# matvogel/P2P-Bridge

Measured on AMD Instinct MI355X. Metric: denoised points/sec (8192-pt patches, T=30), higher is better.
Workload: dtype f32; 1 GPU; PVDS_PUNet xyz-only, 8192-pt patches, T=30 bridge steps, batch 32 per GPU (BASELINE configs[1]); patches_per_gpu=32, points_per_patch=8192, bridge_steps=30, parallelism=patch-shard x1, process_group_world_size=1, hipgraph=True, weights=seeded random init (26.44 M params)

## Files before the change

include/p2pb_hip.h:

```cpp
#ifndef P2PB_HIP_H
#define P2PB_HIP_H

#include <stddef.h>

#ifdef __cplusplus
extern "C" {
#endif

#define P2PB_EINVAL (-22)

#define P2PB_ABI_VERSION 9

int p2pb_version(void);
const char *p2pb_target_arch(void);
int p2pb_set_split_terms(int terms);
int p2pb_set_split_terms_thread(int terms);
int p2pb_get_split_terms(void);
int p2pb_set_deterministic(int on);
int p2pb_get_deterministic(void);
int p2pb_debug_pointwise_form(int cin, int cout, int npos, unsigned long long *launches);

int p2pb_gn_finisher_arm(int groups, double count_per_channel, const float *gamma, const float *beta, const float *style,
                         int style_stride, float eps, float *scale, float *shift, float *chmean);
int p2pb_gn_finisher_armed(void);
void p2pb_gn_finisher_disarm(void);

int p2pb_voxel_coords(int b, int n, int r, int normalize, float eps, const float *coords, float *norm,
                      int *vox, void *stream);

size_t p2pb_avg_voxelize_ws_bytes(int b, int n, int r);
int p2pb_avg_voxelize_forward(int b, int c, int n, int r, const int *coords, const float *feat, int *ind,
                              int *cnt, float *out, void *ws, void *stream);
int p2pb_avg_voxelize_backward(int b, int c, int n, int r3, const int *ind, const int *cnt,
                               const float *grad_y, float *grad_x, void *stream);

int p2pb_trilinear_devoxelize_forward(int b, int c, int n, int r, int is_training, const float *coords,
                                      const float *feat, int *inds, float *wgts, float *outs, void *stream);
int p2pb_trilinear_devoxelize_backward(int b, int c, int n, int r3, const int *inds, const float *wgts,
                                       const float *grad_y, float *grad_x, void *stream);

int p2pb_ball_query(int b, int n, int m, float r2, int u, const float *centers, const float *points, int *idx,
                    void *stream);

int p2pb_grouping_forward(int b, int c, int n, int m, int u, const float *feat, const int *idx, float *out,
                          void *stream);
int p2pb_grouping_backward(int b, int c, int n, int m, int u, const float *grad_y, const int *idx,
                           float *grad_x, void *stream);
int p2pb_grouping_backward_pitched(int b, int c, int n, int m, int u, const float *grad_y, long gy_pitch, const int *idx,
                                   float *grad_x, void *stream);

int p2pb_group_concat(int b, int c, int n, int m, int u, const float *coords, const float *centers,
                      const float *feat, const int *idx, float *out, void *stream);

int p2pb_gather_features_forward(int b, int c, int n, int m, const float *feat, const int *idx, float *out,
                                 void *stream);
int p2pb_gather_features_backward(int b, int c, int n, int m, const float *grad_y, const int *idx,
                                  float *grad_x, void *stream);

int p2pb_furthest_point_sampling(int b, int n, int m, const float *coords, float *dist_ws, int *idx,
                                 void *stream);

size_t p2pb_fps_coop_ws_bytes(int b, int n);
int p2pb_furthest_point_sampling_coop(int b, int n, int m, const float *coords, void *ws, int *idx, void *stream);
size_t p2pb_fps_grid_ws_bytes(int b, int n);
int p2pb_furthest_point_sampling_grid(int b, int n, int m, const float *coords, void *ws, int *idx, void *stream);

int p2pb_point_face_dist(int np, int nt, const float *points, const float *tris, float min_triangle_area, float *dist,
                         int *idx, void *stream);
int p2pb_face_point_dist(int np, int nt, const float *points, const float *tris, float min_triangle_area, float *dist,
                         int *idx, void *stream);

size_t p2pb_knn_points_ws_bytes(int b, int s, int n);
int p2pb_knn_points(int b, int s, int n, int k, const float *query, const float *points, float *dist2, int *idx,
                    float *nn, void *ws, void *stream);

int p2pb_three_nn_interpolate_forward(int b, int c, int m, int n, const float *points, const float *centers,
                                      const float *cfeat, int *idx, float *w, float *out, void *stream);
int p2pb_three_nn(int b, int m, int n, const float *points, const float *centers, int *idx, float *w, void *stream);
int p2pb_three_interpolate(int b, int c, int m, int n, const float *cfeat, const int *idx, const float *w,
                           float *out, void *stream);
size_t p2pb_three_nn_cells_ws_bytes(int b, int m);
int p2pb_three_nn_cells(int b, int m, int n, const float *points, const float *centers, int *idx, float *w, void *ws,
                        void *stream);
int p2pb_three_nn_interpolate_backward(int b, int c, int n, int m, const float *grad_y, const int *idx,
                                       const float *w, float *grad_x, void *stream);
int p2pb_three_nn_interpolate_backward_pitched(int b, int c, int n, int m, const float *grad_y, long gy_pitch, const int *idx,
                                               const float *w, float *grad_x, void *stream);

int p2pb_chamfer_forward(int b, int n, int m, const float *xyz1, const float *xyz2, float *dist1, float *dist2,
                         int *idx1, int *idx2, void *stream);
size_t p2pb_chamfer_ws_bytes(int b, int n, int m);
int p2pb_chamfer_forward_ws(int b, int n, int m, const float *xyz1, const float *xyz2, float *dist1, float *dist2,
                            int *idx1, int *idx2, void *ws, void *stream);
int p2pb_chamfer_backward(int b, int n, int m, const float *xyz1, const float *xyz2, float *gradxyz1,
                          float *gradxyz2, const float *graddist1, const float *graddist2, const int *idx1,
                          const int *idx2, void *stream);

size_t p2pb_approxmatch_temp_floats(int b, int n, int m);
int p2pb_approxmatch_forward(int b, int n, int m, const float *xyz1, const float *xyz2, float *match,
                             float *temp, void *stream);
int p2pb_approxmatch_forward_ws(int b, int n, int m, const float *xyz1, const float *xyz2, float *match, float *temp,
                                size_t temp_floats, void *stream);
int p2pb_matchcost_forward(int b, int n, int m, const float *xyz1, const float *xyz2, const float *match,
                           float *cost, void *stream);
int p2pb_matchcost_backward(int b, int n, int m, const float *grad_cost, const float *xyz1, const float *xyz2,
                            const float *match, float *grad1, float *grad2, void *stream);

int p2pb_auction_forward(int b, int n, int m, const float *xyz1, const float *xyz2, float *dist, int *assignment,
                         float *price, int *assignment_inv, int *bid, float *bid_increments,
                         float *max_increments, int *unass_idx, int *unass_cnt, int *unass_cnt_sum, int *cnt_tmp,
                         int *max_idx, float eps, int iters, void *stream);
int p2pb_auction_backward(int b, int n, const float *xyz1, const float *xyz2, float *gradxyz,
                          const float *graddist, const int *idx, void *stream);


size_t p2pb_conv3d_k3_packed_floats(int cout, int cin);
int p2pb_conv3d_k3_pack_weights(int cout, int cin, const float *w, float *wt_packed, void *stream);
size_t p2pb_conv3d_k3_split_packed_bytes(int cout, int cin);
int p2pb_conv3d_k3_pack_weights_split(int cout, int cin, const float *w, void *wt_split, void *stream);
size_t p2pb_conv3d_k3_stats_floats(int b, int cout, int r);
int p2pb_conv3d_k3_forward(int b, int cin, int cout, int r, const float *in, const float *wt_packed,
                           const float *bias, const float *in_scale, const float *in_shift, int in_swish,
                           float *out, float *stats_part, void *stream);

int p2pb_conv3d_k3_forward_ex(int b, int cin, int cout, int r, const float *in, const void *wt_packed,
                              const float *bias, const float *out_class, const float *in_scale,
                              const float *in_shift, int in_swish, const float *in_sub, int flags, float *out,
                              float *stats_part, void *stream);
int p2pb_conv3d_brick_lists(int b, int r, const int *cnt, unsigned char *flags_ws, int *lists, int *counts,
                            void *stream);
int p2pb_conv3d_k3_forward_sparse(int b, int cin, int cout, int r, const float *in, const void *wt_packed,
                                  const float *bias, const float *out_class, const float *in_scale,
                                  const float *in_shift, int in_swish, const float *in_sub, int flags ,
                                  const int *active_list, const int *active_count, const int *inactive_list,
                                  const int *inactive_count, float *out, float *stats_part, void *stream);
int p2pb_conv3d_active_lists(int b, int r, const int *cnt, unsigned char *lists, int *counts, void *stream);
int p2pb_conv3d_k3_forward_compact(int b, int cin, int cout, int r, const float *in, const void *wt_split,
                                   const float *bias, const float *out_class, const float *in_scale,
                                   const float *in_shift, int in_swish, const float *in_sub,
                                   const unsigned char *alist, const int *acount, float *out, float *stats_part,
                                   int flags , void *stream);
int p2pb_conv3d_presplit(int b, int c, long nvox, const float *y, const float *in_scale, const float *in_shift,
                         int in_swish, const float *in_sub, void *out_split, void *stream);
int p2pb_conv3d_k3_forward_compact_pre(int b, int cin, int cout, int r, const void *in_split, const void *wt_split,
                                       const float *bias, const float *out_class, const unsigned char *alist,
                                       const int *acount, float *out, float *stats_part, int flags ,
                                       void *stream);
int p2pb_conv3d_k3_far_field(int b, int cin, int cout, const float *prev_bias, const float *in_scale,
                             const float *in_shift, int in_swish, const float *wt_packed, const float *bias,
                             float *a, float *k_out, float *tap_ws , void *stream);
int p2pb_conv3d_k3_far_field_gn(int b, int cin, int cout, const float *prev_bias, const float *part, int nslots,
                                double count_per_channel, int groups, const float *gamma, const float *beta,
                                const float *style, int style_stride, float eps, int in_swish, const float *wt_packed,
                                const float *bias, float *scale, float *shift, float *a, float *k_out, float *tap_ws,
                                void *stream);

int p2pb_gn_affine_params(int b, int c, int groups, int nslots, double count_per_channel, const float *part,
                          const float *gamma, const float *beta, const float *style, int style_stride, float eps,
                          float *scale, float *shift, float *chmean, void *stream);
int p2pb_gn_affine_params_ex(int b, int c, int groups, int nslots, double count_per_channel, const float *part,
                             const float *gamma, const float *beta, const float *style, int style_stride, float eps,
                             float *scale, float *shift, float *chmean, float *mean_rstd, void *stream);
int p2pb_norm_act_backward(int b, int c, int groups, int npos, const float *x, const float *gy, const float *scale,
                           const float *shift, const float *mean_rstd, const float *gamma, const float *beta,
                           const float *style, int style_stride, int swish, float *dx, float *dgamma, float *dbeta,
                           float *dstyle, float *ws, void *stream);
int p2pb_norm_act_backward_ex(int b, int c, int groups, int npos, const float *x, const float *gy, const float *scale,
                              const float *shift, const float *mean_rstd, const float *gamma, const float *beta,
                              const float *style, int style_stride, int swish, long gy_pitch, const float *gmean,
                              const float *residual, const float *rgate, float drop_p, const unsigned *seed, unsigned salt, float *dx, float *dgamma,
                              float *dbeta, float *dstyle, float *dres, float *drgate, float *ws, void *stream);
int p2pb_affine_act_train(int b, int c, int npos, const float *x, const float *scale, const float *shift, int swish,
                          const float *residual, const float *rgate, float drop_p, const unsigned *seed, unsigned salt,
                          float *y, void *stream);
int p2pb_se_gate_affine(int b, int c, int hidden, const float *chmean, const float *w1, const float *w2,
                        const float *scale, const float *shift, float *aff_a, float *aff_b, void *stream);
int p2pb_pvconv_tail(int b, int c, int hidden, const float *part2, int nslots2, double count2, int groups2,
                     const float *gamma2, const float *beta2, const float *style2, int style_stride2, float eps2,
                     const float *w1, const float *w2, float *aff_a, float *aff_b, int cp, const float *partp, int nslotsp,
                     double countp, int groupsp, const float *gammap, const float *betap, const float *stylep,
                     int style_stridep, float epsp, float *scale_p, float *shift_p, void *stream);

int p2pb_avg_voxelize_cl_forward(int b, int c, int n, int r, const int *coords, const float *feat, int *ind, int *cnt,
                                 float *out, float *feat_t, void *ws, void *stream);
int p2pb_voxel_sort(int b, int n, int r, const int *coords, int *ind, int *cnt, void *ws, void *stream);
int p2pb_avg_voxelize_cl_gather(int b, int c, int n, int r, const float *feat, const int *cnt, const void *ws,
                                float *out, float *feat_t, void *stream);
int p2pb_avg_voxelize_cl_gather_split(int b, int c, int n, int r, const float *feat, const int *cnt, const void *ws,
                                      void *out_split, float *feat_t, void *stream);
int p2pb_trilinear_devoxelize_cl_affine(int b, int c, int n, int r, const float *coords, const float *grid,
                                        const float *aff_a, const float *aff_b, const float *add ,
                                        const float *add_scale, const float *add_shift, float *outs, void *stream);
int p2pb_trilinear_devoxelize_affine(int b, int c, int n, int r, const float *coords, const float *feat,
                                     const float *aff_a, const float *aff_b, float *outs, void *stream);

int p2pb_three_interpolate_add(int b, int c, int m, int n, const float *cz, const int *idx, const float *w,
                               const float *add, const float *bias, float *out, float *stats_part,
                               float *ws , void *stream);
size_t p2pb_group_sub_stats_floats(int b, int c, int m, int u);
int p2pb_group_sub_stats_slots(int m, int u);
int p2pb_group_sub_stats(int b, int c, int n, int m, int u, const float *zt, const float *cxt, const int *idx,
                         float *stats_part, void *stream);
int p2pb_group_sub(int b, int c, int n, int m, int u, const float *z, const float *cx, const int *idx, float *out,
                   float *stats_part, float *ws , void *stream);

size_t p2pb_pointwise_packed_floats(int cout, int cin);
int p2pb_pointwise_pack_weights(int cout, int cin, const float *w , float *wp, void *stream);
size_t p2pb_pointwise_stats_floats(int b, int cout, int npos);
int p2pb_pointwise_conv_forward(int b, int cin, int cout, int npos, const float *in, const void *wp,
                                const float *bias, const float *bias_b, const float *in_scale,
                                const float *in_shift, int in_swish, int flags, float *out, float *stats_part,
                                void *stream);
size_t p2pb_pointwise_split_packed_bytes(int cout, int cin);
int p2pb_pointwise_pack_weights_split(int cout, int cin, const float *w , void *wp, void *stream);
int p2pb_pointwise_pool_supported(int npos, int pool_u);
size_t p2pb_pointwise_minmax_floats(int b, int cout, int npos, int pool_u, int flags);
int p2pb_pointwise_conv_pool_forward(int b, int cin, int cout, int npos, const float *in, const void *wp,
                                     const float *bias, const float *bias_b, const float *in_scale,
                                     const float *in_shift, int in_swish, int flags, float *out, float *stats_part,
                                     int pool_u, float *minmax, void *stream);
int p2pb_pointwise_conv_pool_gather(int b, int cin, int cout, int n, int m, int u, const float *zt, const float *cxt,
                                    const int *idx, const void *wp_split, const float *bias, const float *in_scale,
                                    const float *in_shift, int in_swish, float *stats_part, float *minmax, void *stream);
int p2pb_linear_rows(int b, int cin, int cout, const float *x, long x_stride, const float *w, long w_stride,
                     const float *bias, float *out, long out_stride, void *stream);
int p2pb_minmax_act(int b, int c, int m, int nslots, const float *minmax, const float *scale, const float *shift,
                    int swish, float *y, void *stream);
int p2pb_minmax_act_pool_gn(int b, int c, int nslots, const float *minmax, const float *part, int nslots_st,
                            double count_per_channel, int groups, const float *gamma, const float *beta, const float *style,
                            int style_stride, float eps, int swish, float *scale, float *shift, float *y, void *stream);
int p2pb_affine_act(int b, int c, int npos, const float *x, const float *scale, const float *shift, int swish,
                    const float *residual, float *y, void *stream);
int p2pb_affine_act_max(int b, int c, int m, int u, const float *x, const float *scale, const float *shift,
                        int swish, float *y, void *stream);

int p2pb_linear_attention_forward(int b, int heads, int dim_head, int n, const float *qkv, float *out, float *ctx,
                                  void *stream);
int p2pb_linear_attention_backward(int b, int heads, int dim_head, int n, const float *qkv, const float *ctx,
                                   const float *grad_out, float *grad_qkv, void *stream);

int p2pb_softmax_attention_forward(int b, int heads, int dim_head, int n, const float *q, const float *kv, float *out,
                                   float *lse, void *stream);
int p2pb_softmax_attention_backward(int b, int heads, int dim_head, int n, const float *q, const float *kv,
                                    const float *out, const float *lse, const float *grad_out, float *grad_q,
                                    float *grad_kv, void *stream);

int p2pb_se_gate_forward(int b, int c, int hidden, const float *mean, const float *w1, const float *w2, float *hid, float *gate,
                         void *stream);
int p2pb_se_gate_backward(int b, int c, int hidden, const float *mean, const float *w1, const float *w2, const float *hid,
                          const float *gate, const float *dgate, float *dmean, float *dw1, float *dw2, float *ws, void *stream);

int p2pb_row_max_forward(long rows, int u, const float *x, float *y, int *idx, void *stream);
int p2pb_row_max_backward(long rows, int u, const float *gy, const int *idx, float *gx, void *stream);

size_t p2pb_conv3d_k3_wgrad_ws_floats(int b, int cin, int cout, int r, int math);
int p2pb_conv3d_k3_wgrad(int b, int cin, int cout, int r, const float *x, const float *dy, float *dw, float *db,
                         float *ws, int math, void *stream);
size_t p2pb_conv3d_k3_wgrad_occ_ws_floats(int b, int cin, int cout, int r, int n);
int p2pb_conv3d_k3_wgrad_occ(int b, int cin, int cout, int r, int n, const float *x, const float *dy, const int *cnt, float *dw,
                             float *db, float *ws, void *stream);
size_t p2pb_pointwise_wgrad_ws_floats(int b, int cin, int cout, int npos, int math);
int p2pb_pointwise_wgrad(int b, int cin, int cout, int npos, const float *x, const float *dy, float *dw, float *db,
                         float *ws, int math, void *stream);

int p2pb_radius_count(int s, int n, const float *centers, const float *points, float radius, int *counts, void *stream);
int p2pb_radius_fill(int s, int n, const float *centers, const float *points, float radius, const long long *offsets,
                     int *out, void *stream);
int p2pb_merge_accumulate(int npatch, int k, const float *pred, const int *idx, const int *cuts, double *sums,
                          int *counts, void *stream);
int p2pb_merge_finish(int n, const double *sums, const int *counts, const float *original, float *out, void *stream);

int p2pb_conv3d_k3_pack_weights_split_adjoint(int cout, int cin, const float *w_forward, void *wt_split, void *stream);
int p2pb_pointwise_pack_weights_adjoint(int cout, int cin, const float *w_forward, float *wp, void *stream);
int p2pb_pointwise_pack_weights_split_adjoint(int cout, int cin, const float *w_forward, void *wp, void *stream);

size_t p2pb_optim_entry_bytes(void);
int p2pb_optim_chunk(void);
int p2pb_optim_clip_adam_step(int nchunks, const void *table, const int *chunks, double *partial, double *ctl, double max_norm,
                              double beta1, double beta2, double eps, double weight_decay, int decoupled, int skip_nonfinite,
                              unsigned *amax, int ntensors, void *stream);
int p2pb_conv3d_k3_pack_weights_split_amax(int cout, int cin, const float *w, void *wt_split, const unsigned *amax_bits,
                                           void *stream);
int p2pb_pointwise_pack_weights_split_amax(int cout, int cin, const float *w, void *wp, const unsigned *amax_bits, void *stream);

size_t p2pb_pairwise_chamfer_ws_bytes(int s, int r);
int p2pb_pairwise_chamfer(int s, int r, int n, int m, const float *A, const float *B, float *out, void *ws, void *stream);
size_t p2pb_pairwise_emd_ws_bytes(int s, int r, int n, int m);
int p2pb_pairwise_emd(int s, int r, int n, int m, const float *A, const float *B, float *out, void *ws, size_t ws_bytes,
                      void *stream);
int p2pb_occupancy_grid_cells(int resolution, int clip_sphere);
size_t p2pb_occupancy_ws_bytes(int resolution);
int p2pb_occupancy_counts(int clouds, int npts, int resolution, int clip_sphere, const float *pts, int *counters,
                          int *bernoulli, void *ws, void *stream);

#ifdef __cplusplus
}
#endif
#endif
```

p2p_bridge_amd/_lib.py:

```python
import ctypes
import os

import torch

_HERE = os.path.dirname(os.path.abspath(__file__))
LIB_PATH = os.environ.get("P2PB_LIB_PATH") or os.path.join(_HERE, "libp2pb_hip.so")

SYMBOLS = [
    "p2pb_version", "p2pb_target_arch", "p2pb_set_split_terms", "p2pb_set_split_terms_thread", "p2pb_get_split_terms", "p2pb_set_deterministic", "p2pb_get_deterministic", "p2pb_voxel_coords", "p2pb_avg_voxelize_ws_bytes",
    "p2pb_avg_voxelize_forward", "p2pb_avg_voxelize_backward", "p2pb_avg_voxelize_cl_gather_split", "p2pb_conv3d_presplit",
    "p2pb_conv3d_k3_forward_compact_pre", "p2pb_trilinear_devoxelize_forward",
    "p2pb_trilinear_devoxelize_backward", "p2pb_ball_query", "p2pb_grouping_forward", "p2pb_grouping_backward", "p2pb_group_concat", "p2pb_group_sub", "p2pb_three_interpolate_add", "p2pb_group_sub_stats_floats", "p2pb_group_sub_stats_slots", "p2pb_group_sub_stats",
    "p2pb_gather_features_forward", "p2pb_gather_features_backward", "p2pb_furthest_point_sampling",
    "p2pb_fps_coop_ws_bytes", "p2pb_furthest_point_sampling_coop", "p2pb_point_face_dist", "p2pb_face_point_dist", "p2pb_knn_points_ws_bytes", "p2pb_knn_points", "p2pb_three_nn_interpolate_forward", "p2pb_three_nn_interpolate_backward", "p2pb_three_nn", "p2pb_three_nn_cells", "p2pb_three_nn_cells_ws_bytes",
    "p2pb_three_interpolate", "p2pb_chamfer_forward",
    "p2pb_chamfer_backward", "p2pb_approxmatch_forward", "p2pb_matchcost_forward", "p2pb_matchcost_backward",
    "p2pb_auction_forward", "p2pb_auction_backward", "p2pb_conv3d_k3_packed_floats", "p2pb_conv3d_k3_pack_weights",
    "p2pb_conv3d_k3_split_packed_bytes", "p2pb_conv3d_k3_pack_weights_split",
    "p2pb_conv3d_k3_stats_floats", "p2pb_conv3d_k3_forward", "p2pb_conv3d_k3_forward_ex",
    "p2pb_conv3d_k3_far_field", "p2pb_conv3d_k3_far_field_gn", "p2pb_pvconv_tail", "p2pb_minmax_act_pool_gn", "p2pb_conv3d_active_lists", "p2pb_conv3d_k3_forward_compact", "p2pb_conv3d_brick_lists", "p2pb_conv3d_k3_forward_sparse", "p2pb_gn_affine_params", "p2pb_se_gate_affine",
    "p2pb_trilinear_devoxelize_affine", "p2pb_avg_voxelize_cl_forward", "p2pb_voxel_sort", "p2pb_avg_voxelize_cl_gather", "p2pb_trilinear_devoxelize_cl_affine", "p2pb_pointwise_packed_floats", "p2pb_pointwise_pack_weights",
    "p2pb_pointwise_stats_floats", "p2pb_pointwise_conv_forward", "p2pb_affine_act", "p2pb_affine_act_max",
    "p2pb_pointwise_split_packed_bytes", "p2pb_pointwise_pack_weights_split", "p2pb_pointwise_pool_supported", "p2pb_pointwise_minmax_floats", "p2pb_pointwise_conv_pool_forward",
    "p2pb_minmax_act", "p2pb_linear_attention_forward", "p2pb_linear_attention_backward", "p2pb_softmax_attention_forward", "p2pb_softmax_attention_backward",
    "p2pb_approxmatch_temp_floats", "p2pb_approxmatch_forward_ws", "p2pb_pointwise_conv_pool_gather", "p2pb_chamfer_ws_bytes", "p2pb_chamfer_forward_ws", "p2pb_radius_count", "p2pb_radius_fill", "p2pb_merge_accumulate", "p2pb_merge_finish", "p2pb_gn_affine_params_ex", "p2pb_norm_act_backward", "p2pb_norm_act_backward_ex", "p2pb_grouping_backward_pitched", "p2pb_three_nn_interpolate_backward_pitched", "p2pb_affine_act_train", "p2pb_conv3d_k3_wgrad_ws_floats", "p2pb_conv3d_k3_wgrad", "p2pb_conv3d_k3_wgrad_occ_ws_floats", "p2pb_conv3d_k3_wgrad_occ", "p2pb_pointwise_wgrad_ws_floats", "p2pb_pointwise_wgrad",
    "p2pb_debug_pointwise_form", "p2pb_linear_rows", "p2pb_gn_finisher_arm", "p2pb_gn_finisher_armed", "p2pb_gn_finisher_disarm", "p2pb_fps_grid_ws_bytes", "p2pb_furthest_point_sampling_grid",
    "p2pb_optim_entry_bytes", "p2pb_optim_chunk", "p2pb_optim_clip_adam_step",
    "p2pb_conv3d_k3_pack_weights_split_adjoint", "p2pb_pointwise_pack_weights_adjoint", "p2pb_pointwise_pack_weights_split_adjoint",
    "p2pb_conv3d_k3_pack_weights_split_amax", "p2pb_pointwise_pack_weights_split_amax",
    "p2pb_se_gate_forward", "p2pb_se_gate_backward", "p2pb_row_max_forward", "p2pb_row_max_backward",
    "p2pb_pairwise_chamfer_ws_bytes", "p2pb_pairwise_chamfer", "p2pb_pairwise_emd_ws_bytes", "p2pb_pairwise_emd",
    "p2pb_occupancy_grid_cells", "p2pb_occupancy_ws_bytes", "p2pb_occupancy_counts",
]

ABI_VERSION = 9

_lib = None


class P2PBError(RuntimeError):
    pass


def lib():
    global _lib
    if _lib is None:
        if not os.path.exists(LIB_PATH):
            raise P2PBError(
                f"{LIB_PATH} not found: build it with `python -m p2p_bridge_amd.build` "
                "(p2p_bridge_amd has no CPU / eager fallback)")
        _lib = ctypes.CDLL(LIB_PATH)
        _lib.p2pb_target_arch.restype = ctypes.c_char_p
        _lib.p2pb_avg_voxelize_ws_bytes.restype = ctypes.c_size_t
        _lib.p2pb_knn_points_ws_bytes.restype = ctypes.c_size_t
        _lib.p2pb_fps_grid_ws_bytes.restype = ctypes.c_size_t
        _lib.p2pb_three_nn_cells_ws_bytes.restype = ctypes.c_size_t
        _lib.p2pb_fps_coop_ws_bytes.restype = ctypes.c_size_t
        _lib.p2pb_conv3d_k3_packed_floats.restype = ctypes.c_size_t
        _lib.p2pb_conv3d_k3_split_packed_bytes.restype = ctypes.c_size_t
        _lib.p2pb_conv3d_k3_stats_floats.restype = ctypes.c_size_t
        _lib.p2pb_pointwise_packed_floats.restype = ctypes.c_size_t
        _lib.p2pb_pointwise_stats_floats.restype = ctypes.c_size_t
        _lib.p2pb_pointwise_minmax_floats.restype = ctypes.c_size_t
        _lib.p2pb_group_sub_stats_floats.restype = ctypes.c_size_t
        _lib.p2pb_pointwise_split_packed_bytes.restype = ctypes.c_size_t
        _lib.p2pb_conv3d_k3_wgrad_ws_floats.restype = ctypes.c_size_t
        _lib.p2pb_conv3d_k3_wgrad_occ_ws_floats.restype = ctypes.c_size_t
        _lib.p2pb_chamfer_ws_bytes.restype = ctypes.c_size_t
        _lib.p2pb_approxmatch_temp_floats.restype = ctypes.c_size_t
        _lib.p2pb_pointwise_wgrad_ws_floats.restype = ctypes.c_size_t
        _lib.p2pb_optim_entry_bytes.restype = ctypes.c_size_t
        _lib.p2pb_pairwise_chamfer_ws_bytes.restype = ctypes.c_size_t
        _lib.p2pb_pairwise_emd_ws_bytes.restype = ctypes.c_size_t
        _lib.p2pb_occupancy_ws_bytes.restype = ctypes.c_size_t
        have = _lib.p2pb_version() if hasattr(_lib, "p2pb_version") else None
        if have != ABI_VERSION:
            bad, _lib = _lib, None
            del bad
            raise P2PBError(f"{LIB_PATH} is ABI version {have}, this package binds version {ABI_VERSION} (include/p2pb_hip.h): "
                            "rebuild it with `python -m p2p_bridge_amd.build`")
        for s in SYMBOLS:
            getattr(_lib, s)
        _lib.p2pb_set_split_terms(6 if os.environ.get("P2PB_CONV_MATH") in ("bf16x6", "fp32") else 16)
    return _lib


def stream_ptr():
    return ctypes.c_void_p(torch.cuda.current_stream().cuda_stream)


def ptr(t):
    return ctypes.c_void_p(t.data_ptr()) if t is not None else ctypes.c_void_p(0)


def check(t, dtype, name):
    if not t.is_cuda:
        raise RuntimeError(f"{name} must be a CUDA tensor")
    if not t.is_contiguous():
        raise RuntimeError(f"{name} must be a contiguous tensor")
    if t.dtype != dtype:
        raise RuntimeError(f"{name} must be a {'float' if dtype == torch.float32 else 'int'} tensor")


def call(fn_name, *args):
    rc = getattr(lib(), fn_name)(*args)
    if rc != 0:
        raise P2PBError(f"{fn_name} failed with code {rc}")
```

p2p_bridge_amd/csrc/abi.hip:

```cpp
#include "common.h"

extern "C" int p2pb_version(void) { return P2PB_ABI_VERSION; }
extern "C" const char *p2pb_target_arch(void) { return "gfx950"; }

#include <atomic>
static std::atomic<int> g_split_terms{SPLIT_F16X3};
static thread_local int tl_split_terms = 0;
int p2pb_split_terms_now() { return tl_split_terms ? tl_split_terms : g_split_terms.load(std::memory_order_relaxed); }
extern "C" int p2pb_set_split_terms(int terms) {
  if (terms != SPLIT_BF16X6 && terms != SPLIT_F16X3) return P2PB_EINVAL;
  g_split_terms.store(terms, std::memory_order_relaxed);
  return 0;
}
extern "C" int p2pb_set_split_terms_thread(int terms) {
  if (terms != 0 && terms != SPLIT_BF16X6 && terms != SPLIT_F16X3 && terms != SPLIT_BF16X3) return P2PB_EINVAL;
  tl_split_terms = terms;
  return 0;
}
extern "C" int p2pb_get_split_terms(void) { return p2pb_split_terms_now(); }

static std::atomic<int> g_deterministic{0};
bool p2pb_deterministic() { return g_deterministic.load(std::memory_order_relaxed) != 0; }
extern "C" int p2pb_set_deterministic(int on) {
  g_deterministic.store(on ? 1 : 0, std::memory_order_relaxed);
  return 0;
}
extern "C" int p2pb_get_deterministic(void) { return p2pb_deterministic() ? 1 : 0; }

#include <mutex>
namespace {
struct FormRow {
  int cin, cout, npos, form;
  unsigned long long n;
};
std::mutex g_form_mu;
FormRow g_forms[128];
int g_nforms = 0;
}
void p2pb_note_pointwise_form(int cin, int cout, int npos, int form) {
  std::lock_guard<std::mutex> lk(g_form_mu);
  for (int i = 0; i < g_nforms; ++i)
    if (g_forms[i].cin == cin && g_forms[i].cout == cout && g_forms[i].npos == npos) {
      g_forms[i].form = form;
      ++g_forms[i].n;
      return;
    }
  if (g_nforms < 128) g_forms[g_nforms++] = {cin, cout, npos, form, 1ull};
}
extern "C" int p2pb_debug_pointwise_form(int cin, int cout, int npos, unsigned long long *launches) {
  std::lock_guard<std::mutex> lk(g_form_mu);
  if (launches) *launches = 0;
  if (cin < 0) {
    g_nforms = 0;
    return -1;
  }
  for (int i = 0; i < g_nforms; ++i)
    if (g_forms[i].cin == cin && g_forms[i].cout == cout && g_forms[i].npos == npos) {
      if (launches) *launches = g_forms[i].n;
      return g_forms[i].form;
    }
  return -1;
}

#include <cstdlib>
#include <cstring>
#include <cctype>
long p2pb_experiment_long(const char *key, long dflt) {
  const char *e = getenv("P2PB_EXPERIMENT");
  const size_t kl = strlen(key);
  while (e && *e) {
    while (*e == ';' || isspace((unsigned char)*e)) ++e;
    size_t i = 0;
    while (i < kl && e[i] && tolower((unsigned char)e[i]) == tolower((unsigned char)key[i])) ++i;
    if (i == kl) {
      const char *q = e + kl;
      while (*q == ' ' || *q == '\t') ++q;
      if (*q == '=') return atol(q + 1);
    }
    e = strchr(e, ';');
  }
  return dflt;
}

__global__ __launch_bounds__(256) void zero_words_kernel(unsigned *__restrict__ p, size_t nwords) {
  const size_t stride = (size_t)gridDim.x * 256;
  for (size_t i = (size_t)blockIdx.x * 256 + threadIdx.x; i < nwords; i += stride) p[i] = 0u;
}

__global__ __launch_bounds__(256) void zero_quads_kernel(uint4 *__restrict__ p, size_t nquads) {
  const size_t stride = (size_t)gridDim.x * 256;
  const uint4 z = make_uint4(0u, 0u, 0u, 0u);
  for (size_t i = (size_t)blockIdx.x * 256 + threadIdx.x; i < nquads; i += stride) p[i] = z;
}

int p2pb_zero_async(void *p, size_t nbytes, hipStream_t s) {
  if (nbytes == 0) return 0;
  if ((((size_t)p) & 15) == 0 && (nbytes & 15) == 0) {
    const size_t nq = nbytes / 16;
    const unsigned grid = (unsigned)((nq + 255) / 256 > 4096 ? 4096 : (nq + 255) / 256);
    hipLaunchKernelGGL(zero_quads_kernel, dim3(grid), dim3(256), 0, s, (uint4 *)p, nq);
    return (int)hipGetLastError();
  }
  const size_t nwords = (nbytes + 3) / 4;
  const unsigned grid = (unsigned)((nwords + 255) / 256 > 2048 ? 2048 : (nwords + 255) / 256);
  hipLaunchKernelGGL(zero_words_kernel, dim3(grid), dim3(256), 0, s, (unsigned *)p, nwords);
  return (int)hipGetLastError();
}

namespace {
thread_local bool tl_fin_armed = false;
thread_local GnFinish tl_fin;
}
extern "C" int p2pb_gn_finisher_arm(int groups, double count_per_channel, const float *gamma, const float *beta, const float *style,
                                    int style_stride, float eps, float *scale, float *shift, float *chmean) {
  if (groups <= 0 || !scale || !shift || !(count_per_channel > 0.0) || tl_fin_armed) return P2PB_EINVAL;
  tl_fin.gamma = gamma, tl_fin.beta = beta, tl_fin.style = style, tl_fin.scale = scale, tl_fin.shift = shift, tl_fin.chmean = chmean;
  tl_fin.count_per_channel = count_per_channel, tl_fin.style_stride = style_stride;
  tl_fin.groups = groups, tl_fin.eps = eps;
  tl_fin_armed = true;
  return 0;
}
extern "C" int p2pb_gn_finisher_armed(void) { return tl_fin_armed ? 1 : 0; }
extern "C" void p2pb_gn_finisher_disarm(void) { tl_fin_armed = false; }
bool p2pb_gn_finisher_take(GnFinish *out) {
  if (!tl_fin_armed) return false;
  *out = tl_fin;
  tl_fin_armed = false;
  return true;
}
```

p2p_bridge_amd/csrc/common.h:

```cpp
#pragma once
#include <hip/hip_runtime.h>
#include <stdint.h>

#include "../../include/p2pb_hip.h"

#define P2PB_WAVE 64

static inline int p2pb_launch_status() { return (int)hipGetLastError(); }
int p2pb_split_terms_now();
#define p2pb_g_split_terms (p2pb_split_terms_now())

static inline unsigned cdiv(long a, long b) { return (unsigned)((a + b - 1) / b); }

__device__ __forceinline__ float sqdist3(float dx, float dy, float dz) {
  return __fmaf_rn(dz, dz, __fmaf_rn(dy, dy, dx * dx));
}

__device__ __forceinline__ int lane_id() { return (int)(threadIdx.x & 63); }

__device__ __forceinline__ int mbcnt(unsigned long long mask) {
  return (int)__builtin_amdgcn_mbcnt_hi((unsigned)(mask >> 32), __builtin_amdgcn_mbcnt_lo((unsigned)mask, 0u));
}

template <int CTRL, int ROW_MASK>
__device__ __forceinline__ float dpp_add_step(float v) {
  const int o = __builtin_amdgcn_update_dpp(0, __builtin_bit_cast(int, v), CTRL, ROW_MASK, 0xf, false);
  return v + __builtin_bit_cast(float, o);
}
__device__ __forceinline__ float halfwave_sum_to_last(float v) {
  v = dpp_add_step<0x111, 0xf>(v);
  v = dpp_add_step<0x112, 0xf>(v);
  v = dpp_add_step<0x114, 0xf>(v);
  v = dpp_add_step<0x118, 0xf>(v);
  v = dpp_add_step<0x142, 0xa>(v);
  return v;
}

typedef __bf16 bf16x8 __attribute__((ext_vector_type(8)));
typedef __bf16 bf16x2 __attribute__((ext_vector_type(2)));
typedef float f32x2 __attribute__((ext_vector_type(2)));
typedef unsigned u32x4 __attribute__((ext_vector_type(4)));
typedef float f32x16 __attribute__((ext_vector_type(16)));

__device__ __forceinline__ void split3(float a, float b, unsigned &p0, unsigned &p1, unsigned &p2) {
  f32x2 v = {a, b};
  const bf16x2 q0 = __builtin_convertvector(v, bf16x2);
  v = v - __builtin_convertvector(q0, f32x2);
  const bf16x2 q1 = __builtin_convertvector(v, bf16x2);
  v = v - __builtin_convertvector(q1, f32x2);
  const bf16x2 q2 = __builtin_convertvector(v, bf16x2);
  p0 = __builtin_bit_cast(unsigned, q0);
  p1 = __builtin_bit_cast(unsigned, q1);
  p2 = __builtin_bit_cast(unsigned, q2);
}

#define SPLIT_BF16X6 6
#define SPLIT_BF16X3 3
#define SPLIT_F16X3 16
#define SPLIT_F16_SX 4.0f
typedef _Float16 f16x8 __attribute__((ext_vector_type(8)));
typedef _Float16 f16x2 __attribute__((ext_vector_type(2)));
__device__ __forceinline__ void split2h(float a, float b, unsigned &p0, unsigned &p1) {
  f32x2 v = {a, b};
  const f16x2 q0 = __builtin_convertvector(v, f16x2);
  v = v - __builtin_convertvector(q0, f32x2);
  const f16x2 q1 = __builtin_convertvector(v, f16x2);
  p0 = __builtin_bit_cast(unsigned, q0);
  p1 = __builtin_bit_cast(unsigned, q1);
}
template <int MODE>
__device__ __forceinline__ void split_pair(float a, float b, unsigned &p0, unsigned &p1, unsigned &p2) {
  if constexpr (MODE == SPLIT_F16X3) {
    split2h(a * SPLIT_F16_SX, b * SPLIT_F16_SX, p0, p1);
    p2 = 0u;
  } else {
    split3(a, b, p0, p1, p2);
  }
}
#define SPLIT_X2W_FLAG 0x100
#ifdef P2PB_X2W_TIMING
#define X2W_KEEP_LOW_WEIGHT_PRODUCT 0
#else
#define X2W_KEEP_LOW_WEIGHT_PRODUCT 1
#endif
constexpr __host__ __device__ int split_planes(int mode) { return mode == SPLIT_BF16X6 ? 3 : 2; }
template <int MODE>
__device__ __forceinline__ f32x16 split_mfma(const u32x4 &a, const u32x4 &b, const f32x16 &c) {
  if constexpr (MODE == SPLIT_F16X3)
    return __builtin_amdgcn_mfma_f32_32x32x16_f16(__builtin_bit_cast(f16x8, a), __builtin_bit_cast(f16x8, b), c, 0, 0, 0);
  else
    return __builtin_amdgcn_mfma_f32_32x32x16_bf16(__builtin_bit_cast(bf16x8, a), __builtin_bit_cast(bf16x8, b), c, 0, 0, 0);
}
__device__ __forceinline__ float f16_weight_scale(float wmax) {
  if (!(wmax > 0.0f) || wmax > 3.0e38f) return 1.0f;
  int e;
  (void)frexpf(wmax, &e);
  return ldexpf(1.0f, 14 - e);
}
struct GnFinish {
  const float *gamma, *beta, *style;
  float *scale, *shift, *chmean;
  double count_per_channel;
  int style_stride, groups;
  float eps;
};
static inline bool gn_shape_ok(int c, int groups, const float *style, int style_stride) {
  return groups > 0 && c % groups == 0 && c / groups <= 256 && !(style && style_stride < 2 * c);
}
typedef float gnf_f32x2 __attribute__((ext_vector_type(2)));
__device__ __forceinline__ void gn_finish_group_v(int c, int nslots, const float *__restrict__ part, const GnFinish &f, int b, int g,
                                                  double *lds, int vt, bool live, float *mean_rstd = nullptr,
                                                  float *tab_scale = nullptr, float *tab_shift = nullptr, float *tab_mean = nullptr) {
  double *rs = lds, *rq = lds + 256, *chs = lds + 512, *chq = lds + 768;
  const int t = vt;
  const int cg = c / f.groups, g0 = g * cg;
  const int nt = 256 / cg;
  const int k = t % cg, j = t / cg;
  float p_ga = 1.0f, p_be = 0.0f, p_fa = 1.0f, p_bi = 0.0f;
  if (live && t < cg) {
    const int ch = g0 + t;
    if (f.gamma) p_ga = f.gamma[ch];
    if (f.beta) p_be = f.beta[ch];
    if (f.style) {
      p_fa = f.style[(size_t)b * f.style_stride + ch];
      p_bi = f.style[(size_t)b * f.style_stride + c + ch];
    }
  }
  double s = 0.0, q = 0.0;
  if (live && j < nt) {
    const float *p0 = part + ((size_t)b * nslots * c + g0 + k) * 2;
    const size_t pitch = (size_t)c * 2;
    int sl = j;
    for (; sl + 7 * nt < nslots; sl += 8 * nt) {
      gnf_f32x2 v[8];
#pragma unroll
      for (int u = 0; u < 8; ++u) {
        const float *pp = p0 + (size_t)(sl + u * nt) * pitch;
        v[u] = *(const gnf_f32x2 *)pp;
      }
#pragma unroll
      for (int u = 0; u < 8; ++u) {
        s += (double)v[u][0];
        q += (double)v[u][1];
      }
    }
    for (; sl + 3 * nt < nslots; sl += 4 * nt) {
      gnf_f32x2 v[4];
#pragma unroll
      for (int u = 0; u < 4; ++u) {
        const float *pp = p0 + (size_t)(sl + u * nt) * pitch;
        v[u] = *(const gnf_f32x2 *)pp;
      }
#pragma unroll
      for (int u = 0; u < 4; ++u) {
        s += (double)v[u][0];
        q += (double)v[u][1];
      }
    }
    for (; sl < nslots; sl += nt) {
      const float *p = p0 + (size_t)sl * pitch;
      s += (double)p[0];
      q += (double)p[1];
    }
  }
  if (live) {
    rs[t] = s;
    rq[t] = q;
  }
  __syncthreads();
  if (live && t < cg) {
    double ts = 0.0, tq = 0.0;
    for (int jj = 0; jj < nt; ++jj) {
      ts += rs[jj * cg + t];
      tq += rq[jj * cg + t];
    }
    chs[t] = ts;
    chq[t] = tq;
  }
  __syncthreads();
  if (live && t < cg) {
    double gs = 0.0, gq = 0.0;
    for (int kk = 0; kk < cg; ++kk) {
      gs += chs[kk];
      gq += chq[kk];
    }
    const int ch = g0 + t;
    const double n = f.count_per_channel * cg;
    const double mean = gs / n;
    double var = gq / n - mean * mean;
    if (var < 0.0) var = 0.0;
    const double rstd = 1.0 / sqrt(var + (double)f.eps);
    const double ga = (double)p_ga, be = (double)p_be, fa = (double)p_fa, bi = (double)p_bi;
    const double sc = rstd * ga * fa;
    const double sh = (be - mean * rstd * ga) * fa + bi;
    const float cm = (float)(sc * (chs[t] / f.count_per_channel) + sh);
    if (f.scale) f.scale[(size_t)b * c + ch] = (float)sc;
    if (f.shift) f.shift[(size_t)b * c + ch] = (float)sh;
    if (f.chmean) f.chmean[(size_t)b * c + ch] = cm;
    if (tab_scale) tab_scale[ch] = (float)sc;
    if (tab_shift) tab_shift[ch] = (float)sh;
    if (tab_mean) tab_mean[ch] = cm;
    if (mean_rstd && t == 0) {
      mean_rstd[((size_t)b * f.groups + g) * 2] = (float)mean;
      mean_rstd[((size_t)b * f.groups + g) * 2 + 1] = (float)rstd;
    }
  }
  __syncthreads();
}
__device__ __forceinline__ void gn_finish_group(int c, int nslots, const float *__restrict__ part, const GnFinish &f, int b, int g,
                                                double *lds, float *mean_rstd = nullptr) {
  gn_finish_group_v(c, nslots, part, f, b, g, lds, (int)threadIdx.x, threadIdx.x < 256, mean_rstd);
}
template <int NS>
__device__ __forceinline__ void gn_finish_sample(int c, int nslots, const float *__restrict__ part, const GnFinish &f, int b, double *lds,
                                                 float *tab_scale = nullptr, float *tab_shift = nullptr, float *tab_mean = nullptr) {
  const int slice = (int)threadIdx.x >> 8, vt = (int)threadIdx.x & 255;
  for (int g0 = 0; g0 < f.groups; g0 += NS) {
    const int g = g0 + slice;
    gn_finish_group_v(c, nslots, part, f, b, g < f.groups ? g : 0, lds + slice * 1024, vt, slice < NS && g < f.groups, nullptr,
                      tab_scale, tab_shift, tab_mean);
  }
}
template <int CTRL>
__device__ __forceinline__ float dpp_full(float v) {
  const int i = __builtin_bit_cast(int, v);
  return __builtin_bit_cast(float, __builtin_amdgcn_update_dpp(i, i, CTRL, 0xf, 0xf, false));
}
__device__ __forceinline__ void permlane16_swap(float &a, float &b) {
  asm volatile("s_nop 1\n\tv_permlane16_swap_b32 %0, %1\n\ts_nop 1" : "+v"(a), "+v"(b));
}
struct RowAdd {
  __device__ static float f(float a, float b) { return a + b; }
};
__device__ __forceinline__ float vmin_raw(float a, float b) {
  float r;
  asm("v_min_f32 %0, %1, %2" : "=v"(r) : "v"(a), "v"(b));
  return r;
}
__device__ __forceinline__ float vmax_raw(float a, float b) {
  float r;
  asm("v_max_f32 %0, %1, %2" : "=v"(r) : "v"(a), "v"(b));
  return r;
}
struct RowMin {
  __device__ static float f(float a, float b) {
    float r;
    asm("v_min_f32 %0, %1, %2" : "=v"(r) : "v"(a), "v"(b));
    return r;
  }
};
struct RowMax {
  __device__ static float f(float a, float b) {
    float r;
    asm("v_max_f32 %0, %1, %2" : "=v"(r) : "v"(a), "v"(b));
    return r;
  }
};
template <class Op>
__device__ __forceinline__ float rowreduce32(float (&v)[32]) {
  const int lane = (int)(threadIdx.x & 63);
#pragma unroll
  for (int i = 0; i < 16; ++i) {
    float a = v[i], b = v[i + 16];
    permlane16_swap(a, b);
    v[i] = Op::f(a, b);
  }
#pragma unroll
  for (int i = 0; i < 8; ++i) {
    const float x = Op::f(v[i], dpp_full<0x128>(v[i])), y = Op::f(v[i + 8], dpp_full<0x128>(v[i + 8]));
    v[i] = (lane & 8) ? y : x;
  }
#pragma unroll
  for (int i = 0; i < 4; ++i) {
    const float x = Op::f(v[i], dpp_full<0x141>(v[i])), y = Op::f(v[i + 4], dpp_full<0x141>(v[i + 4]));
    v[i] = (lane & 4) ? y : x;
  }
#pragma unroll
  for (int i = 0; i < 2; ++i) {
    const float x = Op::f(v[i], dpp_full<0x4E>(v[i])), y = Op::f(v[i + 2], dpp_full<0x4E>(v[i + 2]));
    v[i] = (lane & 2) ? y : x;
  }
  const float x = Op::f(v[0], dpp_full<0xB1>(v[0])), y = Op::f(v[1], dpp_full<0xB1>(v[1]));
  return (lane & 1) ? y : x;
}

template <class Op>
__device__ __forceinline__ void groupreduce8(float (&v)[32]) {
  const int lane = (int)(threadIdx.x & 63);
#pragma unroll
  for (int i = 0; i < 16; ++i) {
    const float x = Op::f(v[i], dpp_full<0x141>(v[i])), y = Op::f(v[i + 16], dpp_full<0x141>(v[i + 16]));
    v[i] = (lane & 4) ? y : x;
  }
#pragma unroll
  for (int i = 0; i < 8; ++i) {
    const float x = Op::f(v[i], dpp_full<0x4E>(v[i])), y = Op::f(v[i + 8], dpp_full<0x4E>(v[i + 8]));
    v[i] = (lane & 2) ? y : x;
  }
#pragma unroll
  for (int i = 0; i < 4; ++i) {
    const float x = Op::f(v[i], dpp_full<0xB1>(v[i])), y = Op::f(v[i + 4], dpp_full<0xB1>(v[i + 4]));
    v[i] = (lane & 1) ? y : x;
  }
}

template <class Op>
__device__ __forceinline__ void groupreduce16(float (&v)[32]) {
  const int lane = (int)(threadIdx.x & 63);
#pragma unroll
  for (int i = 0; i < 16; ++i) {
    const float x = Op::f(v[i], dpp_full<0x140>(v[i])), y = Op::f(v[i + 16], dpp_full<0x140>(v[i + 16]));
    v[i] = (lane & 8) ? y : x;
  }
#pragma unroll
  for (int i = 0; i < 8; ++i) {
    const float x = Op::f(v[i], dpp_full<0x141>(v[i])), y = Op::f(v[i + 8], dpp_full<0x141>(v[i + 8]));
    v[i] = (lane & 4) ? y : x;
  }
#pragma unroll
  for (int i = 0; i < 4; ++i) {
    const float x = Op::f(v[i], dpp_full<0x4E>(v[i])), y = Op::f(v[i + 4], dpp_full<0x4E>(v[i + 4]));
    v[i] = (lane & 2) ? y : x;
  }
#pragma unroll
  for (int i = 0; i < 2; ++i) {
    const float x = Op::f(v[i], dpp_full<0xB1>(v[i])), y = Op::f(v[i + 2], dpp_full<0xB1>(v[i + 2]));
    v[i] = (lane & 1) ? y : x;
  }
}

enum {
  P2PB_FORM_PW_FP32 = 0,
  P2PB_FORM_PW_WIDE_FP32 = 1,
  P2PB_FORM_PW_WIDE_F16 = 2,
  P2PB_FORM_PW_SPLIT128 = 3,
  P2PB_FORM_PW_SPLIT256 = 4,
  P2PB_FORM_PW_PINGPONG = 5,
  P2PB_FORM_PW_GATHER = 6,
};
void p2pb_note_pointwise_form(int cin, int cout, int npos, int form);
bool p2pb_gn_finisher_take(GnFinish *out);
int p2pb_gn_affine_launch(int b, int c, int nslots, const float *part, const GnFinish &f, hipStream_t s);

long p2pb_experiment_long(const char *key, long dflt);

int p2pb_zero_async(void *p, size_t nbytes, hipStream_t s);

#define SCAT_THREADS 512
#define SCAT_LDS_MAX (128 * 1024)
bool p2pb_deterministic();
static inline int scat_threads() { return p2pb_deterministic() ? 64 : SCAT_THREADS; }
static inline int scat_rows(long L, int c, int cap) {
  if (L * 4 > SCAT_LDS_MAX) return 0;
  int ch = (int)((64 * 1024) / (L * 4));
  if (ch < 1) ch = 1;
  if (ch > cap) ch = cap;
  if (ch > c) ch = c;
  return ch;
}
__device__ __forceinline__ void scat_zero(float *rows, int count) {
  for (int i = threadIdx.x * 4; i < count; i += blockDim.x * 4) *(float4 *)(rows + i) = make_float4(0.f, 0.f, 0.f, 0.f);
  __syncthreads();
}
__device__ __forceinline__ void scat_store(const float *rows, int L, int Lp, int nch, float *gx_rows) {
  __syncthreads();
  for (int j = 0; j < nch; ++j)
    for (int i = threadIdx.x; i < L; i += blockDim.x) gx_rows[(size_t)j * L + i] = rows[j * Lp + i];
}
```

p2p_bridge_amd/csrc/pointwise.hip:

```cpp
#include "common.h"
#include "absmax.h"
#include <atomic>
#include <stdint.h>
#include <stdlib.h>

typedef float f32x4 __attribute__((ext_vector_type(4)));

#define PW_CK 16

__device__ __forceinline__ float swishf(float v) {
  return v * __builtin_amdgcn_rcpf(1.0f + __builtin_amdgcn_exp2f(v * -1.44269504088896340736f));
}

template <int MT, bool XF, bool STATS>
__global__ __launch_bounds__(256, 3) void pw_conv_kernel(int cin, int cout, int cout_pad, int P,
                                                      const float *__restrict__ in, const float *__restrict__ wp,
                                                      const float *__restrict__ bias,
                                                      const float *__restrict__ bias_b,
                                                      const float *__restrict__ in_scale,
                                                      const float *__restrict__ in_shift, int in_swish,
                                                      float *__restrict__ out, float *__restrict__ stats_part) {
  const int tid = threadIdx.x, lane = tid & 63, wave = tid >> 6;
  const int l31 = lane & 31, khalf = lane >> 5;
  const int p0 = blockIdx.x * 256, co0 = blockIdx.y * (32 * MT), b = blockIdx.z;
// ... 389 lines not shown
#pragma unroll
      for (int t = 0; t < 4; ++t) acc[m][t][r] += bv;
      if (co < cout && pok && outb)
        *(f32x4 *)(outb + (size_t)co * P + p) = f32x4{acc[m][0][r], acc[m][1][r], acc[m][2][r], acc[m][3][r]};
    }
  const int rrow = MT == 2 ? l31 : (l31 & 15);
  const int rco = co0 + (rrow >> 4) * 32 + (rrow & 3) + 8 * ((rrow & 15) >> 2) + 4 * khalf;
  auto rowval = [&](int kind, int m, int r) -> float {
    const int co = co0 + m * 32 + (r & 3) + 8 * (r >> 2) + 4 * khalf;
    const float v0 = acc[m][0][r], v1 = acc[m][1][r], v2 = acc[m][2][r], v3 = acc[m][3][r];
    const bool ok = co < cout && pok;
    if (kind == 0) return ok ? (v0 + v1) + (v2 + v3) : 0.0f;
    if (kind == 1) return ok ? (v0 * v0 + v1 * v1) + (v2 * v2 + v3 * v3) : 0.0f;
    if (kind == 2) return pok ? vmin_raw(vmin_raw(v0, v1), vmin_raw(v2, v3)) : INFINITY;
    return pok ? -vmax_raw(vmax_raw(v0, v1), vmax_raw(v2, v3)) : INFINITY;
  };
  if (STATS) {
    float s1, s2;
    float tv[32];
    if constexpr (MT == 2) {
#pragma unroll
      for (int i = 0; i < 32; ++i) tv[i] = rowval(0, i >> 4, i & 15);
      s1 = rowreduce32<RowAdd>(tv);
#pragma unroll
      for (int i = 0; i < 32; ++i) tv[i] = rowval(1, i >> 4, i & 15);
      s2 = rowreduce32<RowAdd>(tv);
    } else {
#pragma unroll
      for (int i = 0; i < 32; ++i) tv[i] = rowval(i >> 4, 0, i & 15);
      s1 = s2 = rowreduce32<RowAdd>(tv);
    }
    if (rco < cout) {
      if (slot < nslots) {
        float *q = stats_part + (((size_t)b * nslots + slot) * cout + rco) * 2;
        if constexpr (MT == 2) *(f32x2 *)q = f32x2{s1, s2};
        else q[l31 >> 4] = s1;
      }
      if (slot + 1 < nslots) {
        float *q = stats_part + (((size_t)b * nslots + slot + 1) * cout + rco) * 2;
        if constexpr (MT == 2) *(f32x2 *)q = f32x2{0.0f, 0.0f};
        else q[l31 >> 4] = 0.0f;
      }
    }
  }
  if constexpr (PG != 0) {
    float tv[32];
    if constexpr (PG == 32) {
      float mn, mx;
      if constexpr (MT == 2) {
#pragma unroll
        for (int i = 0; i < 32; ++i) tv[i] = rowval(2, i >> 4, i & 15);
        mn = rowreduce32<RowMin>(tv);
#pragma unroll
        for (int i = 0; i < 32; ++i) tv[i] = rowval(3, i >> 4, i & 15);
        mx = -rowreduce32<RowMin>(tv);
      } else {
#pragma unroll
        for (int i = 0; i < 32; ++i) tv[i] = rowval(2 + (i >> 4), 0, i & 15);
        mn = rowreduce32<RowMin>(tv);
        mx = -mn;
      }
      if (rco < cout) {
        float *q = mm_out + ((((size_t)b * gridDim.x + blockIdx.x) * 4 + wave) * cout + rco) * 2;
        if constexpr (MT == 2) *(f32x2 *)q = f32x2{mn, mx};
        else q[l31 >> 4] = (l31 >> 4) ? mx : mn;
      }
    } else if constexpr (PG == 8) {
      const int j = l31 & 7;
      const size_t ngrp = (size_t)(P / 32);
      if constexpr (MT == 2) {
        float tx[32];
#pragma unroll
        for (int i = 0; i < 32; ++i) {
          tv[i] = rowval(2, i >> 4, i & 15);
          tx[i] = rowval(3, i >> 4, i & 15);
        }
        groupreduce8<RowMin>(tv);
        groupreduce8<RowMin>(tx);
        const int cb = co0 + 32 * (j >> 2) + 8 * (j & 3) + 4 * khalf;
        if (pok) {
          float *q = mm_out + (((size_t)b * cout + cb) * ngrp + p / 32) * 2;
#pragma unroll
          for (int i = 0; i < 4; ++i)
            if (cb + i < cout) *(f32x2 *)(q + (size_t)i * ngrp * 2) = f32x2{tv[i], -tx[i]};
        }
      } else {
#pragma unroll
        for (int i = 0; i < 32; ++i) tv[i] = rowval(2 + (i >> 4), 0, i & 15);
        groupreduce8<RowMin>(tv);
        const int cb = co0 + 8 * (j & 3) + 4 * khalf;
        if (pok) {
          float *q = mm_out + (((size_t)b * cout + cb) * ngrp + p / 32) * 2 + (j >> 2);
#pragma unroll
          for (int i = 0; i < 4; ++i)
            if (cb + i < cout) q[(size_t)i * ngrp * 2] = (j >> 2) ? -tv[i] : tv[i];
        }
      }
    } else {
#pragma unroll
      for (int m = 0; m < MT; ++m)
#pragma unroll
        for (int r = 0; r < 16; ++r) {
          const int co = co0 + m * 32 + (r & 3) + 8 * (r >> 2) + 4 * khalf;
          float mn = rowval(2, m, r), mx = -rowval(3, m, r);
          group_minmax(mn, mx, pool_g);
          if (co < cout && (l31 & (pool_g - 1)) == 0 && pok) {
            const int u = 4 * pool_g;
            float *q = mm_out + (((size_t)b * cout + co) * (P / u) + p / u) * 2;
            q[0] = mn;
            q[1] = mx;
          }
        }
    }
  }
}

__global__ void pw_pack_kernel(int cout, int cin, int cin_pad, int cout_pad, const float *__restrict__ w,
                               float *__restrict__ wp, long s_co, long s_ci) {
  const size_t total = (size_t)cin_pad * cout_pad;
  for (size_t e = (size_t)blockIdx.x * 256 + threadIdx.x; e < total; e += (size_t)gridDim.x * 256) {
    const int kk = (int)(e & 3);
    const int co = (int)((e >> 2) % cout_pad);
    const int kh = (int)((e / ((size_t)4 * cout_pad)) & 1);
    const int chunk = (int)(e / ((size_t)8 * cout_pad));
    const int ci = chunk * 8 + 2 * kk + kh;
    wp[e] = (co < cout && ci < cin) ? w[(size_t)co * s_co + (size_t)ci * s_ci] : 0.0f;
  }
}

static inline int pw_cin_pad(int cin) { return (cin + 7) / 8 * 8; }
static inline int pw_cout_pad(int cout) { return (cout + 127) / 128 * 128; }

extern "C" size_t p2pb_pointwise_packed_floats(int cout, int cin) {
  return (size_t)pw_cin_pad(cin) * pw_cout_pad(cout);
}

static int pw_pack(int cout, int cin, const float *w, float *wp, bool adjoint, void *stream) {
  if (cout <= 0 || cin <= 0) return P2PB_EINVAL;
  const size_t total = p2pb_pointwise_packed_floats(cout, cin);
  hipLaunchKernelGGL(pw_pack_kernel, dim3((unsigned)((total + 255) / 256 > 2048 ? 2048 : (total + 255) / 256)), dim3(256),
                     0, (hipStream_t)stream, cout, cin, pw_cin_pad(cin), pw_cout_pad(cout), w, wp, adjoint ? 1L : (long)cin,
                     adjoint ? (long)cout : 1L);
  return p2pb_launch_status();
}
extern "C" int p2pb_pointwise_pack_weights(int cout, int cin, const float *w, float *wp, void *stream) {
  return pw_pack(cout, cin, w, wp, false, stream);
}
extern "C" int p2pb_pointwise_pack_weights_adjoint(int cout, int cin, const float *w_forward, float *wp, void *stream) {
  return pw_pack(cout, cin, w_forward, wp, true, stream);
}

extern "C" size_t p2pb_pointwise_stats_floats(int b, int cout, int npos) {
  return (size_t)b * ((npos + 255) / 256) * 4 * cout * 2;
}

#define PWS_CK 32

#define PWS_TILE (2 * 3 * 2 * 128)
#define PWS_LDS_BYTES (2 * PWS_TILE * 16)
#include "pw_pp512.h"

template <int PL, int WM, int NB>
__device__ __forceinline__ void pws_epilogue(f32x16 (&acc)[2][2 * NB], int b, int bx, int gx, int pblk, int co0,
                                             int wm, int wn, int l31, int khalf, int cout, int P, int nslots,
                                             const float *__restrict__ bias, const float *__restrict__ bias_b,
                                             float *__restrict__ out, float *__restrict__ stats_part,
                                             float *__restrict__ mm_out, int pool_u, int out_pm, const float *sb) {
#pragma unroll
  for (int pb = 0; pb < NB; ++pb) {
  const int p = pblk + 128 * pb + 2 * (wn * 32 + l31);
  const bool pok = p < P;
  if (WM == 2 && out_pm) {
    float *ob = out + (size_t)b * P * cout;
#pragma unroll
    for (int m = 0; m < 2; ++m)
#pragma unroll
      for (int g = 0; g < 4; ++g) {
        const int cq = co0 + wm * 64 + m * 32 + 8 * g + 4 * khalf;
        float bv[4];
#pragma unroll
        for (int i = 0; i < 4; ++i) bv[i] = sb[cq + i - co0];
        if (pok && cq < cout) {
#pragma unroll
          for (int n = 0; n < 2; ++n) {
            float *q = ob + (size_t)(p + n) * cout + cq;
            const f32x4 v = {acc[m][2 * pb + n][4 * g] + bv[0], acc[m][2 * pb + n][4 * g + 1] + bv[1],
                             acc[m][2 * pb + n][4 * g + 2] + bv[2], acc[m][2 * pb + n][4 * g + 3] + bv[3]};
            if (cq + 3 < cout && (cout & 3) == 0) *(f32x4 *)q = v;
            else
              for (int i = 0; i < 4; ++i)
                if (cq + i < cout) q[i] = v[i];
          }
        }
      }
    continue;
  }
  float *outb = out ? out + (size_t)b * cout * P : nullptr;
  const int slot = (bx * NB + pb) * 2 + wn;
  const int pool_g = pool_u ? pool_u / 2 : 32;
#pragma unroll
  for (int m = 0; m < 2; ++m) {
#pragma unroll
    for (int r = 0; r < 16; ++r) {
      const int co = co0 + wm * 64 + m * 32 + (r & 3) + 8 * (r >> 2) + 4 * khalf;
      const bool cok = co < cout;
      const float bv = sb[co - co0];
      acc[m][2 * pb][r] += bv;
      acc[m][2 * pb + 1][r] += bv;
      const f32x2 v = {acc[m][2 * pb][r], acc[m][2 * pb + 1][r]};
      if (cok && pok && outb) *(f32x2 *)(outb + (size_t)co * P + p) = v;
      if constexpr (PL == 2) {
        float mn = pok ? fminf(v[0], v[1]) : INFINITY, mx = pok ? fmaxf(v[0], v[1]) : -INFINITY;
        group_minmax(mn, mx, pool_g);
        if (cok && pok && (pool_g == 32 ? l31 == 31 : (l31 & (pool_g - 1)) == 0)) {
          float *q = mm_out + (((size_t)b * cout + co) * (P / pool_u) + p / pool_u) * 2;
          q[0] = mn;
          q[1] = mx;
        }
      }
    }
  }
  if constexpr (PL == 32) {
    float tn[32], tx[32];
#pragma unroll
    for (int m = 0; m < 2; ++m)
#pragma unroll
      for (int r = 0; r < 16; ++r) {
        const float v0 = acc[m][2 * pb][r], v1 = acc[m][2 * pb + 1][r];
        tn[m * 16 + r] = pok ? vmin_raw(v0, v1) : INFINITY;
        tx[m * 16 + r] = pok ? -vmax_raw(v0, v1) : INFINITY;
      }
    groupreduce16<RowMin>(tn);
    groupreduce16<RowMin>(tx);
    const int j = l31 & 15;
    const int cb = co0 + wm * 64 + 32 * (j >> 3) + 2 * (j & 1) + 8 * ((j & 7) >> 1) + 4 * khalf;
    if (pok) {
      const size_t ngrp = (size_t)(P / 32);
      float *q = mm_out + (((size_t)b * cout + cb) * ngrp + p / 32) * 2;
#pragma unroll
      for (int i = 0; i < 2; ++i)
        if (cb + i < cout) *(f32x2 *)(q + (size_t)i * ngrp * 2) = f32x2{tn[i], -tx[i]};
    }
  }
  const int rm = l31 >> 4, rr = l31 & 15;
  const int rco = co0 + wm * 64 + rm * 32 + (rr & 3) + 8 * (rr >> 2) + 4 * khalf;
  auto rowvals = [&](int kind, float (&v)[32]) {
#pragma unroll
    for (int m = 0; m < 2; ++m)
#pragma unroll
      for (int r = 0; r < 16; ++r) {
        const int co = co0 + wm * 64 + m * 32 + (r & 3) + 8 * (r >> 2) + 4 * khalf;
        const float v0 = acc[m][2 * pb][r], v1 = acc[m][2 * pb + 1][r];
        const bool ok = co < cout && pok;
        v[m * 16 + r] = kind == 0 ? (ok ? v0 + v1 : 0.0f)
                        : kind == 1 ? (ok ? v0 * v0 + v1 * v1 : 0.0f)
                        : kind == 2 ? (pok ? fminf(v0, v1) : INFINITY)
                                    : (pok ? fmaxf(v0, v1) : -INFINITY);
      }
  };
  if (stats_part) {
    float tv[32];
    rowvals(0, tv);
    const float s1 = rowreduce32<RowAdd>(tv);
    rowvals(1, tv);
    const float s2 = rowreduce32<RowAdd>(tv);
    if (rco < cout) {
      float *q = stats_part + (((size_t)b * nslots + slot) * cout + rco) * 2;
      q[0] = s1;
      q[1] = s2;
      if (bx == gx - 1 && pb == NB - 1 && wn == 1)
        for (int sl = slot + 1; sl < nslots; ++sl) {
          float *z = stats_part + (((size_t)b * nslots + sl) * cout + rco) * 2;
          z[0] = 0.0f;
          z[1] = 0.0f;
        }
    }
  }
  if constexpr (PL == 1) {
    float tv[32];
    rowvals(2, tv);
    const float mn = rowreduce32<RowMin>(tv);
    rowvals(3, tv);
    const float mx = rowreduce32<RowMax>(tv);
    if (rco < cout) {
      float *q = mm_out + ((((size_t)b * gx * NB + bx * NB + pb) * 2 + wn) * cout + rco) * 2;
      q[0] = mn;
      q[1] = mx;
    }
  }
  }
}

template <bool XF, int PL, int WM, int NB, int TERMS>
#ifndef PWS_WM4_WAVES
#define PWS_WM4_WAVES 4
#endif
__global__ __launch_bounds__(128 * WM, NB == 2 ? 2 : (WM == 2 ? 3 : PWS_WM4_WAVES)) void pw_split_kernel(int cin, int cout, int P, int nslots,
                                                       const float *__restrict__ in, const u32x4 *__restrict__ wp,
                                                       const float *__restrict__ bias,
                                                       const float *__restrict__ bias_b,
                                                       const float *__restrict__ in_scale,
                                                       const float *__restrict__ in_shift, int in_swish,
                                                       float *__restrict__ out, float *__restrict__ stats_part,
                                                       float *__restrict__ mm_out, int pool_u, int out_pm) {
  extern __shared__ u32x4 pws_lds[];
  constexpr int NT = 128 * WM;
  constexpr int BS = 128 * NB;
  u32x4 *lds_b = pws_lds + (WM / 2) * PWS_TILE;
  const u32x4 *lds_a = pws_lds;
  const int tid = threadIdx.x, lane = tid & 63;
  const int wave = __builtin_amdgcn_readfirstlane(tid >> 6);
  const int l31 = lane & 31, khalf = lane >> 5;
  const int wm = wave >> 1, wn = wave & 1;
  const int ncoblk = gridDim.y;
  const unsigned lin = blockIdx.x + gridDim.x * (blockIdx.y + gridDim.y * blockIdx.z);
  const unsigned nblk = gridDim.x * gridDim.y * gridDim.z;
  const unsigned vid = nblk % 8 == 0 ? (lin % 8) * (nblk / 8) + lin / 8 : lin;
  const int bx = (vid / ncoblk) % gridDim.x, by = vid % ncoblk;
  const int b = vid / (ncoblk * gridDim.x);
  const int pblk = bx * (128 * NB), co0 = by * (64 * WM);
  const float *inb = in + (size_t)b * cin * P;
  const bool mact = co0 + wm * 64 < cout;
  __shared__ float pws_bias[64 * WM];
  if (tid < 64 * WM) {
    const int co = co0 + tid;
    float v = 0.0f;
    if (co < cout) {
      v = bias ? bias[co] : 0.0f;
      if (bias_b) v += bias_b[(size_t)b * cout + co];
    }
    pws_bias[tid] = v;
  }

  f32x16 acc[2][2 * NB];
#pragma unroll
  for (int m = 0; m < 2; ++m)
#pragma unroll
    for (int n = 0; n < 2 * NB; ++n)
#pragma unroll
      for (int r = 0; r < 16; ++r) acc[m][n][r] = 0.0f;

  constexpr bool ONE = WM == 4 && NB == 1;
  constexpr int NBW = WM == 2 ? NB : 1;
  const int bgrp = WM == 2 ? wave : wave >> 1, bsel = WM == 2 ? 0 : (wave & 1);
  unsigned voff[NBW];
#pragma unroll
  for (int q = 0; q < NBW; ++q) {
    const int pl = ONE ? pblk + 64 * bsel + lane : pblk + 128 * (WM == 2 ? q : bsel) + 2 * lane;
    voff[q] = (unsigned)(pl < P ? pl : P - (ONE ? 1 : 2)) * 4u;
  }
  float braw[NBW][8][ONE ? 1 : 2];
  auto load_b = [&](int ci0) {
#pragma unroll
    for (int i = 0; i < 8; ++i) {
      const int row = min(ci0 + 8 * bgrp + i, cin - 1);
      auto rs = __builtin_amdgcn_make_buffer_rsrc((void *)(inb + (size_t)row * P), 0, P * 4, 0x00020000);
#pragma unroll
      for (int q = 0; q < NBW; ++q) {
        if constexpr (!ONE) {
          const f32x2 v = __builtin_bit_cast(f32x2, __builtin_amdgcn_raw_buffer_load_b64(rs, voff[q], 0, 0));
          braw[q][i][0] = v[0];
          braw[q][i][1] = v[1];
        } else {
          braw[q][i][0] = __builtin_bit_cast(float, __builtin_amdgcn_raw_buffer_load_b32(rs, voff[q], 0, 0));
        }
      }
    }
  };
  auto dma_a = [&](int chunk) {
    const int nblk128 = WM == 2 ? ncoblk : (cout + 127) / 128;
    const u32x4 *src = wp + ((size_t)chunk * nblk128 + by * (WM / 2)) * PWS_TILE;
    u32x4 *dst = pws_lds;
    const bool second_ok = WM == 2 || by * 2 + 1 < nblk128;
#pragma unroll
    for (int i = 0; i < 6; ++i)
      if ((second_ok || i * NT + tid < PWS_TILE) && (TERMS == 6 || (((i * NT + wave * 64) % PWS_TILE) / 256) % 3 != 2))
        __builtin_amdgcn_global_load_lds((const __attribute__((address_space(1))) void *)(src + i * NT + tid),
                                         (__attribute__((address_space(3))) void *)(dst + i * NT + wave * 64), 16, 0, 0);
  };
  load_b(0);

  for (int ci0 = 0; ci0 < cin; ci0 += PWS_CK) {
    __syncthreads();
    dma_a(ci0 / PWS_CK);
    {
      constexpr int NE = ONE ? 1 : 2;
      if (XF) {
#pragma unroll
        for (int i = 0; i < 8; ++i) {
          const int c = min(ci0 + 8 * bgrp + i, cin - 1);
          const float sc = in_scale[b * cin + c], sh = in_shift[b * cin + c];
#pragma unroll
          for (int q = 0; q < NBW; ++q)
#pragma unroll
            for (int e = 0; e < NE; ++e) {
              float v = braw[q][i][e] * sc + sh;
              if (in_swish) v = swishf(v);
              braw[q][i][e] = v;
            }
        }
      }
      const int kstep = bgrp >> 1, kh = bgrp & 1;
#pragma unroll
      for (int q = 0; q < NBW; ++q)
#pragma unroll
        for (int e = 0; e < NE; ++e) {
          u32x4 qq[3];
#pragma unroll
          for (int i = 0; i < 4; ++i) {
            unsigned p0, p1, p2;
            split_pair<TERMS>(braw[q][2 * i][e], braw[q][2 * i + 1][e], p0, p1, p2);
            qq[0][i] = p0;
            qq[1][i] = p1;
            qq[2][i] = p2;
          }
          const int blk = WM == 2 ? q : (NB == 2 ? bsel : 0);
          const int slot = blk * 128 + (ONE ? (lane & 1) * 64 + 32 * bsel + (lane >> 1) : e * 64 + lane);
#pragma unroll
          for (int s = 0; s < split_planes(TERMS); ++s) lds_b[((kstep * 3 + s) * 2 + kh) * BS + slot] = qq[s];
        }
    }
    __builtin_amdgcn_s_waitcnt(0x0F70);
    __syncthreads();
    if (ci0 + PWS_CK < cin) load_b(ci0 + PWS_CK);
    if (!mact) continue;
#pragma unroll
    for (int kstep = 0; kstep < 2; ++kstep) {
      u32x4 af[3][2];
#pragma unroll
      for (int s = 0; s < split_planes(TERMS); ++s)
#pragma unroll
        for (int m = 0; m < 2; ++m)
          af[s][m] = lds_a[(wm >> 1) * PWS_TILE + ((kstep * 3 + s) * 2 + khalf) * 128 + (wm & 1) * 64 + m * 32 + l31];
      constexpr int PA[6] = {2, 1, 0, 1, 0, 0}, PB[6] = {0, 1, 2, 0, 1, 0};
#pragma unroll
      for (int nb = 0; nb < NB; ++nb) {
        u32x4 bf[3][2];
#pragma unroll
        for (int s = 0; s < split_planes(TERMS); ++s)
#pragma unroll
          for (int n = 0; n < 2; ++n)
            bf[s][n] = lds_b[((kstep * 3 + s) * 2 + khalf) * BS + nb * 128 + n * 64 + wn * 32 + l31];
#pragma unroll
        for (int t = (TERMS == 6 ? 0 : 3); t < 6; ++t)
#pragma unroll
          for (int m = 0; m < 2; ++m)
#pragma unroll
            for (int n = 0; n < 2; ++n)
              if (X2W_KEEP_LOW_WEIGHT_PRODUCT || TERMS != SPLIT_F16X3 || PA[t] != 1)
                acc[m][2 * nb + n] = split_mfma<TERMS>(af[PA[t]][m], bf[PB[t]][n], acc[m][2 * nb + n]);
      }
    }
  }
  if (!mact) return;
  {
    if constexpr (TERMS == SPLIT_F16X3) {
      const int nblk128 = WM == 2 ? ncoblk : (cout + 127) / 128;
      const float oscale = ((const float *)(wp + (size_t)((cin + PWS_CK - 1) / PWS_CK) * nblk128 * PWS_TILE))[1];
  #pragma unroll
      for (int m = 0; m < 2; ++m)
  #pragma unroll
        for (int n = 0; n < 2 * NB; ++n)
  #pragma unroll
          for (int r = 0; r < 16; ++r) acc[m][n][r] *= oscale;
    }
  pws_epilogue<PL, WM, NB>(acc, b, bx, (int)gridDim.x, pblk, co0, wm, wn, l31, khalf, cout, P, nslots, bias, bias_b, out,
                             stats_part, mm_out, pool_u, out_pm, pws_bias);
  }
}

__global__ void pw_pack_split_kernel(int cout, int cin, int nchunk, int ncoblk, const float *__restrict__ w,
                                     unsigned short *__restrict__ wp, int mode, float *__restrict__ trailer, long s_co, long s_ci,
                                     const unsigned *__restrict__ amax) {
  const size_t total = (size_t)nchunk * ncoblk * 2 * 2 * 128 * 8;
  const bool x2w = (mode & SPLIT_X2W_FLAG) != 0;
  mode &= 0xff;
  const float wmax = amax ? __builtin_bit_cast(float, *amax) : trailer[0];
  const float sw = mode == SPLIT_F16X3 ? f16_weight_scale(wmax) : 1.0f;
  if (blockIdx.x == 0 && threadIdx.x == 0) {
    trailer[1] = mode == SPLIT_F16X3 ? 1.0f / (SPLIT_F16_SX * sw) : 1.0f;
    if (amax) trailer[0] = wmax, trailer[2] = trailer[3] = 0.0f;
  }
  for (size_t e = (size_t)blockIdx.x * 256 + threadIdx.x; e < total; e += (size_t)gridDim.x * 256) {
    const int idx = (int)(e & 7);
    size_t q = e >> 3;
    const int col = (int)(q & 127);
    q >>= 7;
    const int kh = (int)(q & 1);
    q >>= 1;
    const int ks = (int)(q & 1);
    q >>= 1;
    const int cb = (int)(q % ncoblk), chunk = (int)(q / ncoblk);
    const int co = cb * 128 + col, ci = chunk * PWS_CK + ks * 16 + kh * 8 + idx;
    const float x = (co < cout && ci < cin) ? w[(size_t)co * s_co + (size_t)ci * s_ci] : 0.0f;
    unsigned p0, p1, p2;
    if (mode == SPLIT_F16X3) {
      split2h(x * sw, 0.0f, p0, p1);
      if (x2w) p1 = 0u;
      p2 = 0u;
    } else {
      split3(x, 0.0f, p0, p1, p2);
    }
    const unsigned pp[3] = {p0, p1, p2};
    for (int s = 0; s < 3; ++s)
      wp[((((((size_t)chunk * ncoblk + cb) * 2 + ks) * 3 + s) * 2 + kh) * 128 + col) * 8 + idx] = (unsigned short)(pp[s] & 0xffff);
  }
}

extern "C" size_t p2pb_pointwise_split_packed_bytes(int cout, int cin) {
  const size_t nchunk = (cin + PWS_CK - 1) / PWS_CK, ncoblk = (cout + 127) / 128;
  return nchunk * ncoblk * (2 * 3 * 2 * 128) * 16 + 16;
}

static int pw_pack_split(int cout, int cin, const float *w, void *wp, bool adjoint, void *stream, const unsigned *amax = nullptr) {
  if (cout <= 0 || cin <= 0) return P2PB_EINVAL;
  const int nchunk = (cin + PWS_CK - 1) / PWS_CK, ncoblk = (cout + 127) / 128;
  const size_t total = (size_t)nchunk * ncoblk * 2 * 2 * 128 * 8;
  float *trailer = (float *)((char *)wp + (size_t)nchunk * ncoblk * PWS_TILE * 16);
  static const long x2w = p2pb_experiment_long("x2w", 0);
  const int mode = p2pb_g_split_terms;
  if (mode == SPLIT_F16X3 && !amax) {
    const int rc = p2pb_zero_async(trailer, 16, (hipStream_t)stream);
    if (rc) return rc;
    hipLaunchKernelGGL(absmax_bits_kernel, dim3(absmax_blocks((size_t)cout * cin)), dim3(256), 0, (hipStream_t)stream, w, (size_t)cout * cin,
                       (unsigned *)trailer);
  }
  hipLaunchKernelGGL(pw_pack_split_kernel, dim3((unsigned)((total + 255) / 256 > 2048 ? 2048 : (total + 255) / 256)),
                     dim3(256), 0, (hipStream_t)stream, cout, cin, nchunk, ncoblk, w, (unsigned short *)wp,
                     mode | ((x2w && mode == SPLIT_F16X3 && !adjoint) ? SPLIT_X2W_FLAG : 0), trailer,
                     adjoint ? 1L : (long)cin, adjoint ? (long)cout : 1L, mode == SPLIT_F16X3 ? amax : nullptr);
  return p2pb_launch_status();
}
extern "C" int p2pb_pointwise_pack_weights_split(int cout, int cin, const float *w, void *wp, void *stream) {
  return pw_pack_split(cout, cin, w, wp, false, stream);
}
extern "C" int p2pb_pointwise_pack_weights_split_adjoint(int cout, int cin, const float *w_forward, void *wp, void *stream) {
  return pw_pack_split(cout, cin, w_forward, wp, true, stream);
}
extern "C" int p2pb_pointwise_pack_weights_split_amax(int cout, int cin, const float *w, void *wp, const unsigned *amax_bits,
                                                      void *stream) {
  return amax_bits ? pw_pack_split(cout, cin, w, wp, false, stream, amax_bits) : P2PB_EINVAL;
}

static thread_local GnFinish tl_pw_fin;
static thread_local bool tl_pw_fin_pending = false;
static int pw_finish_behind(int rc, int b, int cout, int P, const float *stats_part, hipStream_t s) {
  if (!tl_pw_fin_pending) return rc;
  tl_pw_fin_pending = false;
  if (rc != 0) return rc;
  if (!stats_part) return P2PB_EINVAL;
  const GnFinish &f = tl_pw_fin;
  if (f.groups <= 0 || cout % f.groups != 0 || cout / f.groups > 256 || (f.style && f.style_stride < 2 * cout)) return P2PB_EINVAL;
  return p2pb_gn_affine_launch(b, cout, (P + 255) / 256 * 4, stats_part, tl_pw_fin, s);
}

static int pw_launch_split(int b, int cin, int cout, int P, const float *in, const void *wp, const float *bias,
                           const float *bias_b, const float *in_scale, const float *in_shift, int in_swish,
                           float *out, float *stats_part, float *minmax, int pool_u, int out_pm, hipStream_t s) {
  const bool xf = in_scale != nullptr;
  const int mode = p2pb_g_split_terms;
  static const int wm_env = (int)p2pb_experiment_long("pw_wm", 0);
  const bool wm4 = !out_pm && (wm_env ? wm_env == 4
                                       : (cout >= 512 && (long)((P + 127) / 128) * ((cout + 255) / 256) * b >= 1024));
  dim3 grid((P + 127) / 128, wm4 ? (cout + 255) / 256 : (cout + 127) / 128, b);
  const int nslots = (P + 255) / 256 * 4;
  const u32x4 *w = (const u32x4 *)wp;
#define LAUNCHW(XF, PL, WM, NB, TM)                                                                                  \
  do {                                                                                                               \
    static bool once = false;                                                                                        \
    const int lds = (WM / 2 + NB) * PWS_TILE * 16;                                                                   \
    if (!once) {                                                                                                     \
      (void)hipFuncSetAttribute((const void *)pw_split_kernel<XF, PL, WM, NB, TM>,                                   \
                                hipFuncAttributeMaxDynamicSharedMemorySize, lds);                                    \
      once = true;                                                                                                   \
    }                                                                                                                \
    hipLaunchKernelGGL((pw_split_kernel<XF, PL, WM, NB, TM>), grid, dim3(128 * WM), lds, s, cin, cout, P, nslots, in, \
                       w, bias, bias_b, in_scale, in_shift, in_swish, out, stats_part, minmax, pool_u, out_pm);       \
  } while (0)
#define LAUNCHF(XF, PL, WM, NB)                                       \
  do {                                                                \
    if (mode == SPLIT_F16X3) LAUNCHW(XF, PL, WM, NB, SPLIT_F16X3);     \
    else LAUNCHW(XF, PL, WM, NB, 6);                                   \
  } while (0)
  if (mode == SPLIT_BF16X3) {
    if (xf || minmax || out_pm) return P2PB_EINVAL;
    p2pb_note_pointwise_form(cin, cout, P, wm4 ? P2PB_FORM_PW_SPLIT256 : P2PB_FORM_PW_SPLIT128);
    if (wm4) LAUNCHW(false, 0, 4, 1, SPLIT_BF16X3);
    else LAUNCHW(false, 0, 2, 1, SPLIT_BF16X3);
    return p2pb_launch_status();
  }
#define LAUNCH(XF, PL)                    \
  do {                                    \
    if (wm4) LAUNCHF(XF, PL, 4, 1);        \
    else LAUNCHF(XF, PL, 2, 1);            \
  } while (0)
  static const int pp_env = (int)p2pb_experiment_long("pw_pp", 1);
  if (pp_env && wm4 && mode == SPLIT_F16X3 && cin % 64 == 0 && cout % 512 == 0 && (!minmax || pool_u == 0) &&
      (size_t)cin * P * 4 < (1ull << 31)) {
    dim3 pgrid((P + 127) / 128, cout / 512, b);
#define LAUNCHP5(XF, PL)                                                                                              \
  do {                                                                                                                \
    static bool once = false;                                                                                         \
    if (!once) {                                                                                                      \
      (void)hipFuncSetAttribute((const void *)pw_pp512_kernel<XF, PL>, hipFuncAttributeMaxDynamicSharedMemorySize,    \
                                P5_LDS_BYTES);                                                                        \
      once = true;                                                                                                    \
    }                                                                                                                 \
    hipLaunchKernelGGL((pw_pp512_kernel<XF, PL>), pgrid, dim3(512), P5_LDS_BYTES, s, cin, cout, P, nslots, in, w, bias, \
                       bias_b, in_scale, in_shift, in_swish, out, stats_part, minmax, pool_u);                        \
  } while (0)
    if (xf && minmax) LAUNCHP5(true, true);
    else if (xf) LAUNCHP5(true, false);
    else if (minmax) LAUNCHP5(false, true);
    else LAUNCHP5(false, false);
#undef LAUNCHP5
    p2pb_note_pointwise_form(cin, cout, P, P2PB_FORM_PW_PINGPONG);
    return p2pb_launch_status();
  }
  p2pb_note_pointwise_form(cin, cout, P, wm4 ? P2PB_FORM_PW_SPLIT256 : P2PB_FORM_PW_SPLIT128);
  const int pl = !minmax ? 0 : pool_u == 0 ? 1 : pool_u == 32 ? 32 : 2;
  if (xf) {
    if (pl == 0) LAUNCH(true, 0);
    else if (pl == 1) LAUNCH(true, 1);
    else if (pl == 32) LAUNCH(true, 32);
    else LAUNCH(true, 2);
  } else {
    if (pl == 0) LAUNCH(false, 0);
    else if (pl == 1) LAUNCH(false, 1);
    else if (pl == 32) LAUNCH(false, 32);
    else LAUNCH(false, 2);
  }
#undef LAUNCH
#undef LAUNCHF
#undef LAUNCHW
  return p2pb_launch_status();
}

static bool pw_wide_ok(int P, const float *in, const float *out) {
  return P % 4 == 0 && (((uintptr_t)in | (uintptr_t)out) & 15) == 0;
}

template <int MT>
static int pw_launch(int b, int cin, int cout, int P, const float *in, const float *wp, const float *bias,
                     const float *bias_b, const float *in_scale, const float *in_shift, int in_swish, float *out,
                     float *stats_part, float *minmax, int pool_g, int out_pm, hipStream_t s, bool split_pack = false) {
  const bool xf = in_scale != nullptr, st = stats_part != nullptr;
  if (split_pack && (!pw_wide_ok(P, in, out) || p2pb_g_split_terms != SPLIT_F16X3)) return P2PB_EINVAL;
  if (pw_wide_ok(P, in, out)) {
    dim3 grid((P + 511) / 512, (cout + 32 * MT - 1) / (32 * MT), b);
    const int nslots = (P + 255) / 256 * 4;
#define LAUNCHX(XF, ST, PL, TM)                                                                                       \
  hipLaunchKernelGGL((pw_wide_kernel<MT, XF, ST, PL, TM>), grid, dim3(256), 0, s, cin, cout, pw_cout_pad(cout), P,       \
                     nslots, in, wp, bias, bias_b, in_scale, in_shift, in_swish, out, stats_part, minmax, pool_g, out_pm,  \
                     PwGather())
#define LAUNCH(XF, ST, PL)                                 \
  do {                                                     \
    if (split_pack) LAUNCHX(XF, ST, PL, SPLIT_F16X3);       \
    else LAUNCHX(XF, ST, PL, 0);                            \
  } while (0)
    p2pb_note_pointwise_form(cin, cout, P, split_pack ? P2PB_FORM_PW_WIDE_F16 : P2PB_FORM_PW_WIDE_FP32);
    if (minmax) {
      const int pg = pool_g == 8 || pool_g == 32 ? pool_g : 1;
      if (xf) {
        if (pg == 8) LAUNCH(true, true, 8);
        else if (pg == 32) LAUNCH(true, true, 32);
        else LAUNCH(true, true, 1);
      } else {
        if (pg == 8) LAUNCH(false, true, 8);
        else if (pg == 32) LAUNCH(false, true, 32);
        else LAUNCH(false, true, 1);
      }
    } else if (xf && st) LAUNCH(true, true, 0);
    else if (xf) LAUNCH(true, false, 0);
    else if (st) LAUNCH(false, true, 0);
    else LAUNCH(false, false, 0);
#undef LAUNCH
#undef LAUNCHX
    return p2pb_launch_status();
  }
  if (minmax || out_pm) return P2PB_EINVAL;
  p2pb_note_pointwise_form(cin, cout, P, P2PB_FORM_PW_FP32);
  dim3 grid((P + 255) / 256, (cout + 32 * MT - 1) / (32 * MT), b);
#define LAUNCH(XF, ST)                                                                                            \
  hipLaunchKernelGGL((pw_conv_kernel<MT, XF, ST>), grid, dim3(256), 0, s, cin, cout, pw_cout_pad(cout), P, in, wp, bias, \
                     bias_b, in_scale, in_shift, in_swish, out, stats_part)
  if (xf && st) LAUNCH(true, true);
  else if (xf) LAUNCH(true, false);
  else if (st) LAUNCH(false, true);
  else LAUNCH(false, false);
#undef LAUNCH
  return p2pb_launch_status();
}

static int pw_conv_forward_impl(int b, int cin, int cout, int npos, const float *in, const void *wp_any,
                                           const float *bias, const float *bias_b, const float *in_scale,
                                           const float *in_shift, int in_swish, int flags, float *out,
                                           float *stats_part, void *stream) {
  if (b <= 0 || cin <= 0 || cout <= 0 || npos <= 0 || !out) return P2PB_EINVAL;
  hipStream_t s = (hipStream_t)stream;
  const int out_pm = (flags & 32) != 0;
  if (out_pm && stats_part) return P2PB_EINVAL;
  if ((flags & 4) && (flags & 128)) {
    const float *wsp = (const float *)wp_any;
    return cout > 32 ? pw_launch<2>(b, cin, cout, npos, in, wsp, bias, bias_b, in_scale, in_shift, in_swish, out,
                                    stats_part, nullptr, 0, out_pm, s, true)
                     : pw_launch<1>(b, cin, cout, npos, in, wsp, bias, bias_b, in_scale, in_shift, in_swish, out,
                                    stats_part, nullptr, 0, out_pm, s, true);
  }
  if (flags & 4) {
    if (!pw_wide_ok(npos, in, out)) return P2PB_EINVAL;
    return pw_launch_split(b, cin, cout, npos, in, wp_any, bias, bias_b, in_scale, in_shift, in_swish, out, stats_part,
                           nullptr, 0, out_pm, s);
  }
  const float *wp = (const float *)wp_any;
  return cout > 32 ? pw_launch<2>(b, cin, cout, npos, in, wp, bias, bias_b, in_scale, in_shift, in_swish, out,
                                  stats_part, nullptr, 0, out_pm, s)
                   : pw_launch<1>(b, cin, cout, npos, in, wp, bias, bias_b, in_scale, in_shift, in_swish, out,
                                  stats_part, nullptr, 0, out_pm, s);
}

extern "C" int p2pb_pointwise_conv_forward(int b, int cin, int cout, int npos, const float *in, const void *wp_any,
                                           const float *bias, const float *bias_b, const float *in_scale,
                                           const float *in_shift, int in_swish, int flags, float *out,
                                           float *stats_part, void *stream) {
  tl_pw_fin_pending = p2pb_gn_finisher_take(&tl_pw_fin);
  const int rc = pw_conv_forward_impl(b, cin, cout, npos, in, wp_any, bias, bias_b, in_scale, in_shift, in_swish, flags, out,
                                      stats_part, stream);
  return pw_finish_behind(rc, b, cout, npos, stats_part, (hipStream_t)stream);
}

static int pool_lanes(int pool_u) { return pool_u == 0 ? 32 : pool_u / 4; }

extern "C" int p2pb_pointwise_pool_supported(int npos, int pool_u) {
  const bool uok = pool_u == 0 || pool_u == 4 || pool_u == 8 || pool_u == 16 || pool_u == 32 || pool_u == 64;
  return npos > 0 && npos % 4 == 0 && uok && (pool_u == 0 || npos % pool_u == 0);
}

extern "C" size_t p2pb_pointwise_minmax_floats(int b, int cout, int npos, int pool_u, int flags) {
  const bool split_tiling = (flags & 4) && !(flags & 128);
  if (pool_u == 0) return (size_t)b * (split_tiling ? (npos + 127) / 128 * 2 : (npos + 511) / 512 * 4) * cout * 2;
  return (size_t)b * cout * (npos / pool_u) * 2;
}

static int pw_conv_pool_forward_impl(int b, int cin, int cout, int npos, const float *in,
                                                const void *wp_any, const float *bias, const float *bias_b,
                                                const float *in_scale, const float *in_shift, int in_swish, int flags,
                                                float *out, float *stats_part, int pool_u, float *minmax,
                                                void *stream) {
  if (b <= 0 || cin <= 0 || cout <= 0 || npos <= 0 || !minmax || !stats_part) return P2PB_EINVAL;
  if (!p2pb_pointwise_pool_supported(npos, pool_u) || !pw_wide_ok(npos, in, out)) return P2PB_EINVAL;
  hipStream_t s = (hipStream_t)stream;
  if ((flags & 4) && (flags & 128)) {
    const float *wsp = (const float *)wp_any;
    const int gl = pool_lanes(pool_u);
    return cout > 32 ? pw_launch<2>(b, cin, cout, npos, in, wsp, bias, bias_b, in_scale, in_shift, in_swish, out,
                                    stats_part, minmax, gl, 0, s, true)
                     : pw_launch<1>(b, cin, cout, npos, in, wsp, bias, bias_b, in_scale, in_shift, in_swish, out,
                                    stats_part, minmax, gl, 0, s, true);
  }
  if (flags & 4)
    return pw_launch_split(b, cin, cout, npos, in, wp_any, bias, bias_b, in_scale, in_shift, in_swish, out, stats_part,
                           minmax, pool_u, 0, s);
  const float *wp = (const float *)wp_any;
  const int g = pool_lanes(pool_u);
  return cout > 32 ? pw_launch<2>(b, cin, cout, npos, in, wp, bias, bias_b, in_scale, in_shift, in_swish, out,
                                  stats_part, minmax, g, 0, s)
                   : pw_launch<1>(b, cin, cout, npos, in, wp, bias, bias_b, in_scale, in_shift, in_swish, out,
                                  stats_part, minmax, g, 0, s);
}

extern "C" int p2pb_pointwise_conv_pool_forward(int b, int cin, int cout, int npos, const float *in,
                                                const void *wp_any, const float *bias, const float *bias_b,
                                                const float *in_scale, const float *in_shift, int in_swish, int flags,
                                                float *out, float *stats_part, int pool_u, float *minmax,
                                                void *stream) {
  tl_pw_fin_pending = p2pb_gn_finisher_take(&tl_pw_fin);
  const int rc = pw_conv_pool_forward_impl(b, cin, cout, npos, in, wp_any, bias, bias_b, in_scale, in_shift, in_swish, flags, out,
                                           stats_part, pool_u, minmax, stream);
  return pw_finish_behind(rc, b, cout, npos, stats_part, (hipStream_t)stream);
}

static int pw_conv_pool_gather_impl(int b, int cin, int cout, int n, int m, int u, const float *zt,
                                               const float *cxt, const int *idx, const void *wp_split, const float *bias,
                                               const float *in_scale, const float *in_shift, int in_swish,
                                               float *stats_part, float *minmax, void *stream) {
  const long npos = (long)m * u;
  if (b <= 0 || cin <= 0 || cout <= 0 || n <= 0 || m <= 0 || !zt || !idx || !wp_split || !in_scale || !in_shift ||
      !stats_part || !minmax || (cin & 7) || npos > 0x7fffffffL || !p2pb_pointwise_pool_supported((int)npos, u) || u == 0 ||
      p2pb_g_split_terms != SPLIT_F16X3 || (((uintptr_t)zt | (uintptr_t)cxt) & 15))
    return P2PB_EINVAL;
  hipStream_t s = (hipStream_t)stream;
  const int P = (int)npos, nslots = (P + 255) / 256 * 4, gl = pool_lanes(u);
  const PwGather gat = {cxt, idx, n, u};
  const float *wsp = (const float *)wp_split;
#define LAUNCHG(MTV, PGV)                                                                                                 \
  hipLaunchKernelGGL((pw_wide_kernel<MTV, true, true, PGV, SPLIT_F16X3, true>),                                    \
                     dim3((P + 511) / 512, (cout + 32 * MTV - 1) / (32 * MTV), b), dim3(256), 0, s, cin, cout,             \
                     pw_cout_pad(cout), P, nslots, zt, wsp, bias, (const float *)nullptr, in_scale, in_shift, in_swish,    \
                     (float *)nullptr, stats_part, minmax, gl, 0, gat)
  if (gl == 8) {
    if (cout > 32) LAUNCHG(2, 8);
    else LAUNCHG(1, 8);
  } else {
    if (cout > 32) LAUNCHG(2, 1);
    else LAUNCHG(1, 1);
  }
#undef LAUNCHG
  p2pb_note_pointwise_form(cin, cout, P, P2PB_FORM_PW_GATHER);
  return p2pb_launch_status();
}

extern "C" int p2pb_pointwise_conv_pool_gather(int b, int cin, int cout, int n, int m, int u, const float *zt,
                                               const float *cxt, const int *idx, const void *wp_split, const float *bias,
                                               const float *in_scale, const float *in_shift, int in_swish,
                                               float *stats_part, float *minmax, void *stream) {
  tl_pw_fin_pending = p2pb_gn_finisher_take(&tl_pw_fin);
  const int rc = pw_conv_pool_gather_impl(b, cin, cout, n, m, u, zt, cxt, idx, wp_split, bias, in_scale, in_shift, in_swish,
                                          stats_part, minmax, stream);
  return pw_finish_behind(rc, b, cout, (int)((long)m * u), stats_part, (hipStream_t)stream);
}


__global__ __launch_bounds__(256) void minmax_act_kernel(int c, int m, int nslots, const float *__restrict__ mm,
                                                         const float *__restrict__ scale,
                                                         const float *__restrict__ shift, int swish,
                                                         float *__restrict__ y, size_t total) {
  for (size_t e = (size_t)blockIdx.x * 256 + threadIdx.x; e < total; e += (size_t)gridDim.x * 256) {
    float mn, mx;
    size_t bc;
    if (nslots == 0) {
      bc = e / m;
      const float2 v = *(const float2 *)(mm + e * 2);
      mn = v.x;
      mx = v.y;
    } else {
      bc = e;
      const size_t b = e / c, ch = e % c;
      mn = INFINITY;
      mx = -INFINITY;
      for (int sl = 0; sl < nslots; ++sl) {
        const float2 v = *(const float2 *)(mm + ((b * nslots + sl) * c + ch) * 2);
        mn = fminf(mn, v.x);
        mx = fmaxf(mx, v.y);
      }
    }
    const float sc = scale[bc], sh = shift[bc];
    float lo = mn * sc + sh, hi = mx * sc + sh;
    if (swish) {
      lo = swishf(lo);
      hi = swishf(hi);
    }
    y[e] = fmaxf(lo, hi);
  }
}

__global__ __launch_bounds__(256) void minmax_act_pool_kernel(int c, int nslots, const float *__restrict__ mm,
                                                              const float *__restrict__ scale,
                                                              const float *__restrict__ shift, int swish,
                                                              float *__restrict__ y, const float *__restrict__ part, int nslots_st,
                                                              GnFinish fin) {
  __shared__ float smn[8][32], smx[8][32];
  __shared__ double gl[4 * 256];
  extern __shared__ float mmp_tab[];
  const int b = blockIdx.y, ch = blockIdx.x * 32 + (threadIdx.x & 31), part_i = threadIdx.x >> 5;
  float mn = INFINITY, mx = -INFINITY;
  if (ch < c)
    for (int sl = part_i; sl < nslots; sl += 8) {
      const float2 v = *(const float2 *)(mm + (((size_t)b * nslots + sl) * c + ch) * 2);
      mn = fminf(mn, v.x);
      mx = fmaxf(mx, v.y);
    }
  smn[part_i][threadIdx.x & 31] = mn;
  smx[part_i][threadIdx.x & 31] = mx;
  if (part != nullptr) {
    const int cg = c / fin.groups, c0 = blockIdx.x * 32, c1 = min(c0 + 32, c) - 1;
    for (int g = c0 / cg; g <= c1 / cg; ++g)
      gn_finish_group_v(c, nslots_st, part, fin, b, g, gl, (int)threadIdx.x, true, nullptr, mmp_tab, mmp_tab + c);
  }
  __syncthreads();
  if (part_i != 0 || ch >= c) return;
#pragma unroll
  for (int p = 1; p < 8; ++p) {
    mn = fminf(mn, smn[p][threadIdx.x]);
    mx = fmaxf(mx, smx[p][threadIdx.x]);
  }
  const float sc = part ? mmp_tab[ch] : scale[(size_t)b * c + ch], sh = part ? mmp_tab[c + ch] : shift[(size_t)b * c + ch];
  float lo = mn * sc + sh, hi = mx * sc + sh;
  if (swish) {
    lo = swishf(lo);
    hi = swishf(hi);
  }
  y[(size_t)b * c + ch] = fmaxf(lo, hi);
}

extern "C" int p2pb_minmax_act(int b, int c, int m, int nslots, const float *minmax, const float *scale,
                               const float *shift, int swish, float *y, void *stream) {
  if (b <= 0 || c <= 0 || m <= 0 || nslots < 0) return P2PB_EINVAL;
  if (nslots >= 16) {
    hipLaunchKernelGGL(minmax_act_pool_kernel, dim3((c + 31) / 32, b), dim3(256), 0, (hipStream_t)stream, c, nslots, minmax,
                       scale, shift, swish, y, (const float *)nullptr, 0, GnFinish());
    return p2pb_launch_status();
  }
  const size_t total = nslots == 0 ? (size_t)b * c * m : (size_t)b * c;
  const unsigned blocks = (unsigned)((total + 255) / 256 > 4096 ? 4096 : (total + 255) / 256);
  hipLaunchKernelGGL(minmax_act_kernel, dim3(blocks), dim3(256), 0, (hipStream_t)stream, c, m, nslots, minmax, scale,
                     shift, swish, y, total);
  return p2pb_launch_status();
}
extern "C" int p2pb_minmax_act_pool_gn(int b, int c, int nslots, const float *minmax, const float *part, int nslots_st,
                                       double count_per_channel, int groups, const float *gamma, const float *beta,
                                       const float *style, int style_stride, float eps, int swish, float *scale, float *shift,
                                       float *y, void *stream) {
  if (b <= 0 || c <= 0 || nslots <= 0 || !minmax || !part || nslots_st <= 0 || !scale || !shift || !y || groups <= 0 ||
      c % groups != 0 || c / groups > 256 || (style && style_stride < 2 * c) || (size_t)c * 8 > 32 * 1024)
    return P2PB_EINVAL;
  GnFinish f = {};
  f.gamma = gamma, f.beta = beta, f.style = style, f.scale = scale, f.shift = shift, f.style_stride = style_stride, f.groups = groups;
  f.eps = eps, f.count_per_channel = count_per_channel;
  hipLaunchKernelGGL(minmax_act_pool_kernel, dim3((c + 31) / 32, b), dim3(256), (size_t)c * 8, (hipStream_t)stream, c, nslots, minmax,
                     (const float *)nullptr, (const float *)nullptr, swish, y, part, nslots_st, f);
  return p2pb_launch_status();
}

#define LR_BC 16
__global__ __launch_bounds__(256) void linear_rows_kernel(int B, int cin, int cout, const float *__restrict__ x, long xs,
                                                          const float *__restrict__ w, long ws,
                                                          const float *__restrict__ bias, float *__restrict__ out, long os,
                                                          int bc) {
  extern __shared__ float lr_x[];
  const int tid = threadIdx.x, lane = tid & 63, wave = tid >> 6, l31 = lane & 31, h = lane >> 5;
  const int row0 = blockIdx.x * 32;
  const int xp = cin + 4;
  const int wrow = min(row0 + l31, cout - 1);
  const int nk8 = (cin + 7) / 8;
  for (int b0 = 0; b0 < B; b0 += bc) {
    const int nb = min(bc, B - b0);
    __syncthreads();
    for (int e = tid * 4; e < nb * cin; e += 1024) {
      const int bb = e / cin, c = e - bb * cin;
      *(f32x4 *)(lr_x + bb * xp + c) = *(const f32x4 *)(x + (size_t)(b0 + bb) * xs + c);
    }
    __syncthreads();
    f32x16 acc;
#pragma unroll
    for (int r = 0; r < 16; ++r) acc[r] = 0.0f;
    const float *wp_ = w + (size_t)wrow * ws + 4 * h;
    const float *xq = lr_x + min(l31, nb - 1) * xp + 4 * h;
    const int nit = (nk8 - wave + 3) / 4;
    for (int it0 = 0; it0 < nit; it0 += 8) {
      f32x4 wv[8], xv[8];
#pragma unroll
      for (int u = 0; u < 8; ++u) {
        const int k = (wave + 4 * (it0 + u)) * 8;
        wv[u] = f32x4{0.0f, 0.0f, 0.0f, 0.0f};
        if (it0 + u < nit && k + 4 * h < cin) wv[u] = *(const f32x4 *)(wp_ + k);
      }
#pragma unroll
      for (int u = 0; u < 8; ++u) {
        const int k = (wave + 4 * (it0 + u)) * 8;
        xv[u] = f32x4{0.0f, 0.0f, 0.0f, 0.0f};
        if (it0 + u < nit && k + 4 * h < cin) xv[u] = *(const f32x4 *)(xq + k);
      }
#pragma unroll
      for (int u = 0; u < 8; ++u)
#pragma unroll
        for (int i = 0; i < 4; ++i) acc = __builtin_amdgcn_mfma_f32_32x32x2f32(wv[u][i], xv[u][i], acc, 0, 0, 0);
    }
    __syncthreads();
    float *red = lr_x;
    if (l31 < nb) {
#pragma unroll
      for (int r = 0; r < 16; ++r) red[(wave * 32 + (r & 3) + 8 * (r >> 2) + 4 * h) * 17 + l31] = acc[r];
    }
    __syncthreads();
    for (int e = tid; e < 32 * nb; e += 256) {
      const int r = e / nb, bb = e - r * nb;
      if (row0 + r < cout) {
        const float v = (red[(0 * 32 + r) * 17 + bb] + red[(1 * 32 + r) * 17 + bb]) + (red[(2 * 32 + r) * 17 + bb] + red[(3 * 32 + r) * 17 + bb]);
        out[(size_t)(b0 + bb) * os + row0 + r] = v + (bias ? bias[row0 + r] : 0.0f);
      }
    }
  }
}

extern "C" int p2pb_linear_rows(int b, int cin, int cout, const float *x, long x_stride, const float *w, long w_stride,
                                const float *bias, float *out, long out_stride, void *stream) {
  if (b <= 0 || cin <= 0 || cout <= 0 || !x || !w || !out || (cin & 3) || (x_stride & 3) || (w_stride & 3) ||
      (((uintptr_t)x | (uintptr_t)w) & 15) || x_stride < cin || w_stride < cin || out_stride < cout)
    return P2PB_EINVAL;
  int bc = (int)(65536 / ((long)(cin + 4) * 4));
  if (bc < 1) return P2PB_EINVAL;
  if (bc > LR_BC) bc = LR_BC;
  if (bc > b) bc = b;
  size_t lr_lds = (size_t)bc * (cin + 4) * 4;
  if (lr_lds < 4 * 32 * 17 * 4) lr_lds = 4 * 32 * 17 * 4;
  hipLaunchKernelGGL(linear_rows_kernel, dim3(cdiv(cout, 32)), dim3(256), lr_lds, (hipStream_t)stream, b, cin,
                     cout, x, x_stride, w, w_stride, bias, out, out_stride, bc);
  return p2pb_launch_status();
}

__global__ __launch_bounds__(256) void affine_act_kernel(int c, int P, const float *__restrict__ x,
                                                         const float *__restrict__ scale,
                                                         const float *__restrict__ shift, int swish,
                                                         const float *__restrict__ residual, float *__restrict__ y) {
  const int bc = blockIdx.y;
  const float sc = scale[bc], sh = shift[bc];
  const float *xr = x + (size_t)bc * P;
  const float *rr = residual ? residual + (size_t)bc * P : nullptr;
  float *yr = y + (size_t)bc * P;
  for (int p = blockIdx.x * 256 + threadIdx.x; p < P; p += gridDim.x * 256) {
    float v = xr[p] * sc + sh;
    if (swish) v = swishf(v);
    if (rr) v = rr[p] + v;
    yr[p] = v;
  }
}

__global__ __launch_bounds__(256) void affine_act4_kernel(int c, int P4, const f32x4 *__restrict__ x,
                                                          const float *__restrict__ scale,
                                                          const float *__restrict__ shift, int swish,
                                                          const f32x4 *__restrict__ residual, f32x4 *__restrict__ y) {
  const int bc = blockIdx.y;
  const float sc = scale[bc], sh = shift[bc];
  const f32x4 *xr = x + (size_t)bc * P4;
  const f32x4 *rr = residual ? residual + (size_t)bc * P4 : nullptr;
  f32x4 *yr = y + (size_t)bc * P4;
  for (int p = blockIdx.x * 256 + threadIdx.x; p < P4; p += gridDim.x * 256) {
    f32x4 v = xr[p];
#pragma unroll
    for (int i = 0; i < 4; ++i) {
      float t = v[i] * sc + sh;
      if (swish) t = swishf(t);
      v[i] = t;
    }
    if (rr) v += rr[p];
    yr[p] = v;
  }
}

extern "C" int p2pb_affine_act(int b, int c, int npos, const float *x, const float *scale, const float *shift,
                               int swish, const float *residual, float *y, void *stream) {
  if (b <= 0 || c <= 0 || npos <= 0) return P2PB_EINVAL;
  if (npos % 4 == 0 && (((uintptr_t)x | (uintptr_t)y | (uintptr_t)residual) & 15) == 0) {
    const int p4 = npos / 4;
    const unsigned gx = (unsigned)((p4 + 255) / 256 > 64 ? 64 : (p4 + 255) / 256);
    hipLaunchKernelGGL(affine_act4_kernel, dim3(gx, b * c), dim3(256), 0, (hipStream_t)stream, c, p4, (const f32x4 *)x,
                       scale, shift, swish, (const f32x4 *)residual, (f32x4 *)y);
    return p2pb_launch_status();
  }
  const unsigned gx = (unsigned)((npos + 255) / 256 > 64 ? 64 : (npos + 255) / 256);
  hipLaunchKernelGGL(affine_act_kernel, dim3(gx, b * c), dim3(256), 0, (hipStream_t)stream, c, npos, x, scale, shift,
                     swish, residual, y);
  return p2pb_launch_status();
}

__global__ __launch_bounds__(256) void affine_act_max_kernel(int M, int U, const float *__restrict__ x,
                                                             const float *__restrict__ scale,
                                                             const float *__restrict__ shift, int swish,
                                                             float *__restrict__ y) {
  const int bc = blockIdx.y;
  const float sc = scale[bc], sh = shift[bc];
  const float *xr = x + (size_t)bc * M * U;
  float *yr = y + (size_t)bc * M;
  const int total = M * U;
  for (int e = blockIdx.x * 256 + threadIdx.x; e < total; e += gridDim.x * 256) {
    float v = xr[e] * sc + sh;
    if (swish) v = swishf(v);
    for (int off = U >> 1; off > 0; off >>= 1) v = fmaxf(v, __shfl_xor(v, off));
    if ((e & (U - 1)) == 0) yr[e / U] = v;
  }
}

__global__ __launch_bounds__(256) void affine_act_rowmax_kernel(int P, const float *__restrict__ x,
                                                                const float *__restrict__ scale,
                                                                const float *__restrict__ shift, int swish,
                                                                float *__restrict__ y) {
  __shared__ float red[256];
  const int bc = blockIdx.x;
  const float sc = scale[bc], sh = shift[bc];
  const float *xr = x + (size_t)bc * P;
  float mx = -INFINITY;
// ... 30 lines not shown
```

p2p_bridge_amd/fused.py:

```python
import ctypes
import os

from . import _experiment
import threading

import torch

from ._lib import call, check, lib, ptr, stream_ptr

_i, _f, _d = ctypes.c_int, ctypes.c_float, ctypes.c_double
F32 = torch.float32


CONV_MATHS = ("f16x3", "bf16x6", "fp32")
SPLIT_MATHS = ("f16x3", "bf16x6")
CONV_MATH_DEFAULT = "f16x3"
_SPLIT_TERMS = {"f16x3": 16, "bf16x6": 6, "fp32": 6, "bf16x3": 3}
_conv_math_override = None


def conv_math() -> str:
    m = _conv_math_override or os.environ.get("P2PB_CONV_MATH", CONV_MATH_DEFAULT)
    if m not in CONV_MATHS:
        raise ValueError(f"P2PB_CONV_MATH must be one of {CONV_MATHS}, got {m!r}")
# ... 126 lines not shown

@_honours_pin(1)
def conv3d_k3(x, conv, in_scale=None, in_shift=None, swish=False, stats=True, in_sub=None, out_class=None,
              skip_zero=False, compact=False, math=None, force_split=False, channels_last=False, pre=False):
    check(x, F32, "x")
    b, ci, r = (x.shape[0], x.shape[4], x.shape[1]) if channels_last else (x.shape[0], x.shape[1], x.shape[2])
    co = conv.out_channels
    split = force_split or use_split(co, math)
    if pre:
        assert split and channels_last and in_scale is None and in_sub is None and x.shape[4] == (conv.in_channels + 15) // 16 * 16
        ci = conv.in_channels
    wt = pack_conv3d_weight(conv, split)
    y = torch.empty((b, r, r, r, co) if channels_last else (b, co, r, r, r), dtype=F32, device=x.device)
    st = None
    if stats:
        nfl = lib().p2pb_conv3d_k3_stats_floats(_i(b), _i(co), _i(r))
        st = torch.empty(b, nfl // (b * co * 2), co, 2, dtype=F32, device=x.device)
    flags = (1 if skip_zero else 0) | (2 if compact else 0) | (4 if split else 0) | (8 if channels_last else 0) | (16 if pre else 0)
    call("p2pb_conv3d_k3_forward_ex", _i(b), _i(ci), _i(co), _i(r), ptr(x), ptr(wt), ptr(conv.bias), ptr(out_class),
         ptr(in_scale), ptr(in_shift), _i(int(swish)), ptr(in_sub), _i(flags), ptr(y), ptr(st), stream_ptr())
    return y, st


def brick_lists(cnt, r):
    b = cnt.shape[0]
    nb = {32: 128, 16: 16}[r]
    lists = torch.empty(4, b * nb, dtype=torch.int32, device=cnt.device)
    counts = torch.empty(4, dtype=torch.int32, device=cnt.device)
    flags = torch.empty(b * nb * 2, dtype=torch.uint8, device=cnt.device)
    call("p2pb_conv3d_brick_lists", _i(b), _i(r), ptr(cnt), ptr(flags), ptr(lists), ptr(counts), stream_ptr())
    return lists, counts


@_honours_pin(1)
def conv3d_k3_sparse(x, conv, lists, counts, which, in_scale=None, in_shift=None, swish=False, in_sub=None,
                     out_class=None, math=None, channels_last=False, pre=False, active_only=False):
    check(x, F32, "x")
    b, ci, r = (x.shape[0], x.shape[4], x.shape[1]) if channels_last else (x.shape[0], x.shape[1], x.shape[2])
    co = conv.out_channels
    split = use_split(co, math)
    if pre:
        assert split and channels_last and in_scale is None and in_sub is None and x.shape[4] == (conv.in_channels + 15) // 16 * 16
        ci = conv.in_channels
    wt = pack_conv3d_weight(conv, split)
    y = torch.empty((b, r, r, r, co) if channels_last else (b, co, r, r, r), dtype=F32, device=x.device)
    nfl = lib().p2pb_conv3d_k3_stats_floats(_i(b), _i(co), _i(r))
    st = torch.empty(b, nfl // (b * co * 2), co, 2, dtype=F32, device=x.device)
    act, ina = lists[2 * which], lists[2 * which + 1]
    ca, ci_ = counts[2 * which:], counts[2 * which + 1:]
    flags = (4 if split else 0) | (8 if channels_last else 0) | (16 if pre else 0) | (32 if active_only else 0)
    call("p2pb_conv3d_k3_forward_sparse", _i(b), _i(ci), _i(co), _i(r), ptr(x), ptr(wt), ptr(conv.bias),
         ptr(out_class), ptr(in_scale), ptr(in_shift), _i(int(swish)), ptr(in_sub), _i(flags), ptr(act), ptr(ca),
         ptr(ina), ptr(ci_), ptr(y), ptr(st), stream_ptr())
    return y, st


def active_lists(cnt, r):
    b = cnt.shape[0]
    nb = {32: 128, 16: 16, 8: 2}[int(r)]
    lists = torch.empty(2, b, nb, 256, dtype=torch.uint8, device=cnt.device)
    counts = torch.empty(2, b, nb, dtype=torch.int32, device=cnt.device)
    call("p2pb_conv3d_active_lists", _i(b), _i(int(r)), ptr(cnt), ptr(lists), ptr(counts), stream_ptr())
    return lists, counts


@_honours_pin(1)
def conv3d_k3_compact(x, conv, lists, counts, which, in_scale=None, in_shift=None, swish=False, in_sub=None,
                      out_class=None, pre=False, listed_only=False):
    check(x, F32, "x")
    b, r, ci = x.shape[0], x.shape[1], x.shape[4]
    co = conv.out_channels
    wt = pack_conv3d_weight(conv, True)
    y = torch.empty(b, r, r, r, co, dtype=F32, device=x.device)
    nfl = lib().p2pb_conv3d_k3_stats_floats(_i(b), _i(co), _i(r))
    st = torch.empty(b, nfl // (b * co * 2), co, 2, dtype=F32, device=x.device)
    al, ac = lists[which], counts[which]
    if pre:
        assert in_scale is None and in_sub is None and x.shape[4] == (conv.in_channels + 15) // 16 * 16
        call("p2pb_conv3d_k3_forward_compact_pre", _i(b), _i(conv.in_channels), _i(co), _i(r), ptr(x), ptr(wt), ptr(conv.bias),
             ptr(out_class), ptr(al), ptr(ac), ptr(y), ptr(st), _i(32 if listed_only else 0), stream_ptr())
        return y, st
    call("p2pb_conv3d_k3_forward_compact", _i(b), _i(ci), _i(co), _i(r), ptr(x), ptr(wt), ptr(conv.bias),
         ptr(out_class), ptr(in_scale), ptr(in_shift), _i(int(swish)), ptr(in_sub), ptr(al), ptr(ac), ptr(y), ptr(st),
         _i(32 if listed_only else 0), stream_ptr())
    return y, st


def conv3d_far_field(prev_bias, conv, in_scale, in_shift, swish=True):
    b, ci = in_scale.shape
    co = conv.out_channels
    wt = pack_conv3d_weight(conv)
    dev = prev_bias.device
    a = torch.empty(b, ci, dtype=F32, device=dev)
    k = torch.empty(b, 27, co, dtype=F32, device=dev)
    ws = torch.empty(b, 27, co, dtype=F32, device=dev)
    call("p2pb_conv3d_k3_far_field", _i(b), _i(ci), _i(co), ptr(prev_bias), ptr(in_scale), ptr(in_shift),
         _i(int(swish)), ptr(wt), ptr(conv.bias), ptr(a), ptr(k), ptr(ws), stream_ptr())
    return a, k


def _style_arg(style, c):
    if style is None:
        return None, 0
    if style.stride(1) != 1 or style.shape[1] != 2 * c:
        style = style.contiguous()
    return style, style.stride(0)


def conv3d_far_field_gn(prev_bias, conv, part, fin, swish=True):
    count, groups, gamma, beta, style, eps, _ = fin
    b, nslots, ci, _ = part.shape
    co = conv.out_channels
    wt = pack_conv3d_weight(conv)
    dev = part.device
    scale = torch.empty(b, ci, dtype=F32, device=dev)
    shift, a = torch.empty_like(scale), torch.empty_like(scale)
    k = torch.empty(b, 27, co, dtype=F32, device=dev)
    ws = torch.empty(b, 27, co, dtype=F32, device=dev)
    style, stride = _style_arg(style, ci)
    call("p2pb_conv3d_k3_far_field_gn", _i(b), _i(ci), _i(co), ptr(prev_bias), ptr(part), _i(nslots), _d(float(count)), _i(int(groups)),
         ptr(gamma), ptr(beta), ptr(style), _i(stride), _f(eps), _i(int(swish)), ptr(wt), ptr(conv.bias), ptr(scale), ptr(shift),
         ptr(a), ptr(k), ptr(ws), stream_ptr())
    return scale, shift, a, k


def pvconv_tail(part2, fin2, se=None, point=None):
    count2, groups2, gamma2, beta2, style2, eps2, _ = fin2
    b, ns2, c, _ = part2.shape
    dev = part2.device
    aff_a = torch.empty(b, c, dtype=F32, device=dev)
    aff_b = torch.empty_like(aff_a)
    style2, stride2 = _style_arg(style2, c)
    w1, w2 = se if se is not None else (None, None)
    hidden = 0 if se is None else w1.shape[0]
    scp = shp = partp = gammap = betap = stylep = None
    cp = nsp = groupsp = stridep = 0
    countp, epsp = 1.0, 1e-5
    if point is not None:
        partp, (countp, groupsp, gammap, betap, stylep, epsp, _) = point
        nsp, cp = partp.shape[1], partp.shape[2]
        stylep, stridep = _style_arg(stylep, cp)
        scp = torch.empty(b, cp, dtype=F32, device=dev)
        shp = torch.empty_like(scp)
    call("p2pb_pvconv_tail", _i(b), _i(c), _i(hidden), ptr(part2), _i(ns2), _d(float(count2)), _i(int(groups2)), ptr(gamma2), ptr(beta2),
         ptr(style2), _i(stride2), _f(eps2), ptr(w1), ptr(w2), ptr(aff_a), ptr(aff_b), _i(cp), ptr(partp), _i(nsp), _d(float(countp)),
         _i(int(groupsp)), ptr(gammap), ptr(betap), ptr(stylep), _i(stridep), _f(epsp), ptr(scp), ptr(shp), stream_ptr())
    return aff_a, aff_b, scp, shp


def minmax_act_pool_gn(mm, part, fin, swish=True):
    count, groups, gamma, beta, style, eps, _ = fin
    b, nslots, c, _ = mm.shape
    dev = mm.device
    y = torch.empty(b, c, dtype=F32, device=dev)
    scale, shift = torch.empty_like(y), torch.empty_like(y)
    style, stride = _style_arg(style, c)
    call("p2pb_minmax_act_pool_gn", _i(b), _i(c), _i(nslots), ptr(mm), ptr(part), _i(part.shape[1]), _d(float(count)), _i(int(groups)),
         ptr(gamma), ptr(beta), ptr(style), _i(stride), _f(eps), _i(int(swish)), ptr(scale), ptr(shift), ptr(y), stream_ptr())
    return y, scale, shift


def gn_affine_params(part, count_per_channel, groups, gamma, beta, style=None, eps=1e-5, want_mean=False):
    b, nslots, c, _ = part.shape
    scale = torch.empty(b, c, dtype=F32, device=part.device)
    shift = torch.empty_like(scale)
    chmean = torch.empty_like(scale) if want_mean else None
    stride = 0
    if style is not None:
        if style.stride(1) != 1 or style.shape[1] != 2 * c:
            style = style.contiguous()
        stride = style.stride(0)
    call("p2pb_gn_affine_params", _i(b), _i(c), _i(groups), _i(nslots), _d(float(count_per_channel)), ptr(part),
         ptr(gamma), ptr(beta), ptr(style), _i(stride), _f(eps), ptr(scale), ptr(shift), ptr(chmean), stream_ptr())
    return scale, shift, chmean


def se_gate_affine(chmean, fc1_weight, fc2_weight, scale, shift):
    b, c = chmean.shape
    a, bb = torch.empty_like(scale), torch.empty_like(shift)
    call("p2pb_se_gate_affine", _i(b), _i(c), _i(fc1_weight.shape[0]), ptr(chmean), ptr(fc1_weight), ptr(fc2_weight),
         ptr(scale), ptr(shift), ptr(a), ptr(bb), stream_ptr())
    return a, bb


def devoxelize_affine(grid, vcoords, r, aff_a, aff_b, channels_last=False, add=None):
    check(grid, F32, "grid"), check(vcoords, F32, "coords")
    b, c = (grid.shape[0], grid.shape[4]) if channels_last else grid.shape[:2]
    n = vcoords.shape[2]
    out = torch.empty(b, c, n, dtype=F32, device=grid.device)
    aff_a, aff_b = aff_a.contiguous(), aff_b.contiguous()
    if channels_last:
        h, hs, hb = add if add is not None else (None, None, None)
        call("p2pb_trilinear_devoxelize_cl_affine", _i(b), _i(c), _i(n), _i(int(r)), ptr(vcoords), ptr(grid),
             ptr(aff_a), ptr(aff_b), ptr(h), ptr(hs), ptr(hb), ptr(out), stream_ptr())
    else:
        assert add is None
        call("p2pb_trilinear_devoxelize_affine", _i(b), _i(c), _i(n), _i(int(r)), ptr(vcoords), ptr(grid),
             ptr(aff_a), ptr(aff_b), ptr(out), stream_ptr())
    return out


def voxel_sort(vox, r):
    b, _, n = vox.shape
    r = int(r)
    dev = vox.device
    ind = torch.empty(b, n, dtype=torch.int32, device=dev)
    cnt = torch.empty(b, r * r * r, dtype=torch.int32, device=dev)
    ws = torch.empty(lib().p2pb_avg_voxelize_ws_bytes(_i(b), _i(n), _i(r)), dtype=torch.uint8, device=dev)
    call("p2pb_voxel_sort", _i(b), _i(n), _i(r), ptr(vox), ptr(ind), ptr(cnt), ptr(ws), stream_ptr())
    return cnt, ws


def voxelize_cl_gather(features, cnt, ws, r, split=False):
    check(features, F32, "features")
    b, c, n = features.shape
    r = int(r)
    feat_t = torch.empty(b, n, c, dtype=F32, device=features.device)
    if split:
        out = torch.empty(b, r, r, r, (c + 15) // 16 * 16, dtype=F32, device=features.device)
        call("p2pb_avg_voxelize_cl_gather_split", _i(b), _i(c), _i(n), _i(r), ptr(features), ptr(cnt), ptr(ws), ptr(out),
             ptr(feat_t), stream_ptr())
        return out
    out = torch.empty(b, r, r, r, c, dtype=F32, device=features.device)
    call("p2pb_avg_voxelize_cl_gather", _i(b), _i(c), _i(n), _i(r), ptr(features), ptr(cnt), ptr(ws), ptr(out),
         ptr(feat_t), stream_ptr())
    return out


def voxelize_cl(features, vox, r):
    check(features, F32, "features")
    b, c, n = features.shape
    r = int(r)
    dev = features.device
    out = torch.empty(b, r, r, r, c, dtype=F32, device=dev)
    ind = torch.empty(b, n, dtype=torch.int32, device=dev)
    cnt = torch.empty(b, r * r * r, dtype=torch.int32, device=dev)
    feat_t = torch.empty(b, n, c, dtype=F32, device=dev)
    ws = torch.empty(lib().p2pb_avg_voxelize_ws_bytes(_i(b), _i(n), _i(r)), dtype=torch.uint8, device=dev)
    call("p2pb_avg_voxelize_cl_forward", _i(b), _i(c), _i(n), _i(r), ptr(vox), ptr(features), ptr(ind), ptr(cnt),
         ptr(out), ptr(feat_t), ptr(ws), stream_ptr())
    return out, cnt




def enabled(module: torch.nn.Module, x: torch.Tensor) -> bool:
    return x.is_cuda and not module.training and not torch.is_grad_enabled()


def pack_pointwise_weight(conv, ci_lo=0, ci_hi=None, split=False) -> torch.Tensor:
    w = conv.weight
    adjoint = bool(getattr(conv, "adjoint", False))
    if adjoint:
        assert ci_lo == 0 and ci_hi in (None, w.shape[0])
        ci_hi = w.shape[0]
    ci_hi = w.shape[1] if ci_hi is None else ci_hi
    key = (w.data_ptr(), w._version, w.device)
    cache = getattr(conv, "_p2pb_packed_pw", None)
    if cache is None or cache[0] != key:
        cache = conv._p2pb_packed_pw = (key, {})
    packs = cache[1]
    if split:
        split = "f16" if lib().p2pb_get_split_terms() == 16 else "bf16"
    k = (ci_lo, ci_hi, split)
    if k not in packs:
        if adjoint:
            w2 = w.detach().reshape(w.shape[0], -1).contiguous()
            co = w2.shape[1]
        else:
            co = w.shape[0]
            w2 = w.detach().reshape(co, -1)[:, ci_lo:ci_hi].contiguous()
        sfx = "_adjoint" if adjoint else ""
        if split:
            wp = torch.empty(lib().p2pb_pointwise_split_packed_bytes(_i(co), _i(ci_hi - ci_lo)), dtype=torch.uint8,
                             device=w.device)
            amax = _amax_slot(w) if (split == "f16" and not adjoint and ci_lo == 0 and ci_hi == w2.shape[1] == w[0].numel()) else None
            if amax is not None:
                call("p2pb_pointwise_pack_weights_split_amax", _i(co), _i(ci_hi), ptr(w2), ptr(wp), ptr(amax), stream_ptr())
            else:
                call("p2pb_pointwise_pack_weights_split" + sfx, _i(co), _i(ci_hi - ci_lo), ptr(w2), ptr(wp), stream_ptr())
        else:
            wp = torch.empty(lib().p2pb_pointwise_packed_floats(_i(co), _i(ci_hi - ci_lo)), dtype=F32, device=w.device)
            call("p2pb_pointwise_pack_weights" + sfx, _i(co), _i(ci_hi - ci_lo), ptr(w2), ptr(wp), stream_ptr())
        packs[k] = wp
    return packs[k]


def pool_supported(npos: int, pool_u: int) -> bool:
    return bool(lib().p2pb_pointwise_pool_supported(_i(npos), _i(pool_u)))


PW_SPLIT_MIN_CIN, PW_SPLIT_MIN_COUT = 128, 128


def use_wide_f16(ci: int, co: int) -> bool:
    return ci >= _experiment.get_int("wide_f16_min_cin", 16)


def use_split_pw(ci: int, co: int, npos: int, math=None) -> bool:
    return ((math or conv_math()) in SPLIT_MATHS and ci >= PW_SPLIT_MIN_CIN and co >= PW_SPLIT_MIN_COUT
            and npos % 4 == 0)


def arm_finisher(fin, b, c, device):
    count, groups, gamma, beta, style, eps, want_mean = fin
    scale = torch.empty(b, c, dtype=F32, device=device)
    shift = torch.empty_like(scale)
    chmean = torch.empty_like(scale) if want_mean else None
    stride = 0
    if style is not None:
        if style.stride(1) != 1 or style.shape[1] != 2 * c:
            style = style.contiguous()
        stride = style.stride(0)
    call("p2pb_gn_finisher_arm", _i(int(groups)), _d(float(count)), ptr(gamma), ptr(beta), ptr(style), _i(stride), _f(eps),
         ptr(scale), ptr(shift), ptr(chmean))
    return (scale, shift, chmean), style


@_honours_pin(1)
def pw_conv(x, conv, in_scale=None, in_shift=None, swish=False, stats=True, bias_b=None, ci_lo=0, ci_hi=None,
            use_bias=True, pool_u=None, store=True, math=None, point_major=False, fin=None):
    check(x, F32, "x")
    b, ci, p = x.shape
    co = conv.out_channels if getattr(conv, "adjoint", False) else conv.weight.shape[0]
    split = use_split_pw(ci, co, p, math)
    if in_scale is not None and (co + (127 if split else 63)) // (128 if split else 64) >= _experiment.get_int("prepass_blocks", 9):
        x = affine_act(x, in_scale, in_shift, swish)
        in_scale = in_shift = None
        swish = False
    point_major = point_major and not stats and pool_u is None and p % 4 == 0
    wide_h = (not split and math is None and conv_math() == "f16x3" and lib().p2pb_get_split_terms() == 16 and p % 4 == 0
              and x.data_ptr() % 16 == 0 and use_wide_f16(ci, co))
    wp = pack_pointwise_weight(conv, ci_lo, ci_hi, split or wide_h)
    pre = 128 if wide_h else 0
    flags = _i((4 if (split or wide_h) else 0) | (32 if point_major else 0) | pre)
    if point_major:
        y = torch.empty(b, p, co, dtype=F32, device=x.device)
    else:
        y = torch.empty(b, co, p, dtype=F32, device=x.device) if (store or pool_u is None) else None
    st = None
    if stats or pool_u is not None:
        nfl = lib().p2pb_pointwise_stats_floats(_i(b), _i(co), _i(p))
        st = torch.empty(b, nfl // (b * co * 2), co, 2, dtype=F32, device=x.device)
    bias = conv.bias if use_bias else None
    aff = keep = None
    if fin is not None:
        assert st is not None
        aff, keep = arm_finisher(fin, b, co, x.device)
    try:
        if pool_u is None:
            call("p2pb_pointwise_conv_forward", _i(b), _i(ci), _i(co), _i(p), ptr(x), ptr(wp), ptr(bias), ptr(bias_b),
                 ptr(in_scale), ptr(in_shift), _i(int(swish)), flags, ptr(y), ptr(st), stream_ptr())
            return (y, st) if fin is None else (y, st, aff)
        return _pw_conv_pool(x, wp, bias, bias_b, in_scale, in_shift, swish, flags, y, st, pool_u, b, ci, co, p, fin, aff)
    finally:
        if fin is not None:
            lib().p2pb_gn_finisher_disarm()


def _pw_conv_pool(x, wp, bias, bias_b, in_scale, in_shift, swish, flags, y, st, pool_u, b, ci, co, p, fin, aff):
    nmm = lib().p2pb_pointwise_minmax_floats(_i(b), _i(co), _i(p), _i(pool_u), flags)
    mm = torch.empty((b, nmm // (b * co * 2), co, 2) if pool_u == 0 else (b, co, p // pool_u, 2), dtype=F32,
                     device=x.device)
    call("p2pb_pointwise_conv_pool_forward", _i(b), _i(ci), _i(co), _i(p), ptr(x), ptr(wp), ptr(bias), ptr(bias_b),
         ptr(in_scale), ptr(in_shift), _i(int(swish)), flags, ptr(y), ptr(st), _i(pool_u), ptr(mm), stream_ptr())
    return (y, st, mm) if fin is None else (y, st, mm, aff)


def linear_rows(x, weight, bias=None):
    if x.stride(-1) != 1 or x.data_ptr() % 16 or x.stride(0) % 4:
        x = x.contiguous()
    if weight.stride(-1) != 1 or weight.data_ptr() % 16 or weight.stride(0) % 4:
        weight = weight.contiguous()
    b, ci = x.shape
    co = weight.shape[0]
    assert weight.shape[1] == ci and x.dtype == F32 and weight.dtype == F32 and x.is_cuda
    out = torch.empty(b, co, dtype=F32, device=x.device)
    call("p2pb_linear_rows", _i(b), _i(ci), _i(co), ptr(x), ctypes.c_long(x.stride(0)), ptr(weight), ctypes.c_long(weight.stride(0)),
         ptr(bias), ptr(out), ctypes.c_long(co), stream_ptr())
    return out


def minmax_act(mm, scale, shift, swish=True, global_pool=False):
    if global_pool:
        b, nslots, c, _ = mm.shape
        y = torch.empty(b, c, dtype=F32, device=mm.device)
        m = 1
    else:
        b, c, m, _ = mm.shape
        nslots = 0
        y = torch.empty(b, c, m, dtype=F32, device=mm.device)
    call("p2pb_minmax_act", _i(b), _i(c), _i(m), _i(nslots), ptr(mm), ptr(scale), ptr(shift), _i(int(swish)), ptr(y),
         stream_ptr())
    return y


def gather_pool_supported(ci: int, co: int, m: int, u: int) -> bool:
    return (conv_math() == "f16x3" and lib().p2pb_get_split_terms() == 16 and ci % 8 == 0
            and not use_split_pw(ci, co, m * u) and use_wide_f16(ci, co) and pool_supported(m * u, u) and u > 0
            and _experiment.get("sa_gather", "1") != "0")


@_honours_pin(3)
def pw_conv_pool_gather(zt, cxt, idx, conv, in_scale, in_shift, swish=True, fin=None):
    check(zt, F32, "zt")
    b, n, ci = zt.shape
    m, u = idx.shape[1], idx.shape[2]
    co = conv.weight.shape[0]
    p = m * u
    wp = pack_pointwise_weight(conv, 0, None, True)
    nfl = lib().p2pb_pointwise_stats_floats(_i(b), _i(co), _i(p))
    st = torch.empty(b, nfl // (b * co * 2), co, 2, dtype=F32, device=zt.device)
    mm = torch.empty(b, co, m, 2, dtype=F32, device=zt.device)
    aff = keep = None
    if fin is not None:
        aff, keep = arm_finisher(fin, b, co, zt.device)
    try:
        call("p2pb_pointwise_conv_pool_gather", _i(b), _i(ci), _i(co), _i(n), _i(m), _i(u), ptr(zt), ptr(cxt), ptr(idx), ptr(wp),
             ptr(conv.bias), ptr(in_scale), ptr(in_shift), _i(int(swish)), ptr(st), ptr(mm), stream_ptr())
    finally:
        if fin is not None:
            lib().p2pb_gn_finisher_disarm()
    return (st, mm) if fin is None else (st, mm, aff)


def group_sub(z, cx, idx, point_major=False, stats_only=False):
    check(z, F32, "z")
    if point_major:
        b, n, c = z.shape
    else:
        b, c, n = z.shape
    m, u = idx.shape[1], idx.shape[2]
    if stats_only and point_major:
        st = torch.empty(b, lib().p2pb_group_sub_stats_slots(_i(m), _i(u)), c, 2, dtype=F32, device=z.device)
        call("p2pb_group_sub_stats", _i(b), _i(c), _i(n), _i(m), _i(u), ptr(z), ptr(cx), ptr(idx), ptr(st), stream_ptr())
        return None, st
    y = None if stats_only else torch.empty(b, c, m * u, dtype=F32, device=z.device)
    nfl = lib().p2pb_group_sub_stats_floats(_i(b), _i(c), _i(m), _i(u))
    st = torch.empty(b, nfl // (b * c * 2), c, 2, dtype=F32, device=z.device)
    ws = None if point_major else torch.empty(b * (n + m) * c, dtype=F32, device=z.device)
    call("p2pb_group_sub", _i(b), _i(c), _i(n), _i(m), _i(u), ptr(z), ptr(cx), ptr(idx), ptr(y), ptr(st), ptr(ws),
         stream_ptr())
    return y, st


def interp_add(cz, idx, w, add=None, bias=None, point_major=False):
    check(cz, F32, "cz")
    if point_major:
        b, m, c = cz.shape
    else:
        b, c, m = cz.shape
    n = idx.shape[2]
    y = torch.empty(b, c, n, dtype=F32, device=cz.device)
    nfl = lib().p2pb_group_sub_stats_floats(_i(b), _i(c), _i(n), _i(1))
    st = torch.empty(b, nfl // (b * c * 2), c, 2, dtype=F32, device=cz.device)
    ws = None if point_major else torch.empty(b * m * c, dtype=F32, device=cz.device)
    call("p2pb_three_interpolate_add", _i(b), _i(c), _i(m), _i(n), ptr(cz), ptr(idx), ptr(w), ptr(add), ptr(bias),
         ptr(y), ptr(st), ptr(ws), stream_ptr())
    return y, st


def affine_act(x, scale, shift, swish=True, residual=None):
    b, c, p = x.shape
    y = torch.empty_like(x)
    if residual is not None:
        residual = residual.contiguous()
    call("p2pb_affine_act", _i(b), _i(c), _i(p), ptr(x), ptr(scale), ptr(shift), _i(int(swish)), ptr(residual), ptr(y),
         stream_ptr())
    return y


def affine_act_max(x, scale, shift, m, u, swish=True):
    b, c = x.shape[:2]
    y = torch.empty((b, c, m) if u else (b, c), dtype=F32, device=x.device)
    call("p2pb_affine_act_max", _i(b), _i(c), _i(m), _i(u), ptr(x), ptr(scale), ptr(shift), _i(int(swish)), ptr(y),
         stream_ptr())
    return y


class operand_audit:
    LIMIT = 16376.0

    def __enter__(self):
        import sys
        self._pre = os.environ.get("P2PB_EXPERIMENT")
        os.environ["P2PB_EXPERIMENT"] = _experiment.setting(conv_pre=":")
        self.rows, self.layers, self._mod = [], [], sys.modules[__name__]
        self._orig = {k: getattr(self._mod, k) for k in ("pw_conv", "conv3d_k3", "conv3d_k3_sparse", "conv3d_k3_compact")}
        names = {"pw_conv": ("in_scale", "in_shift", "swish"), "conv3d_k3": ("in_scale", "in_shift", "swish"),
                 "conv3d_k3_sparse": (None, None, None, "in_scale", "in_shift", "swish"),
                 "conv3d_k3_compact": (None, None, None, "in_scale", "in_shift", "swish")}

        def wrap(kind, orig):
            def f(x, conv, *a, **k):
                kw = dict(k)
                for n, v in zip(names[kind], a):
                    if n:
                        kw[n] = v
                sc, sh = kw.get("in_scale"), kw.get("in_shift")
                cl = kw.get("channels_last", kind == "conv3d_k3_compact")
                v = x
                if sc is not None:
                    shape = [x.shape[0]] + ([1] * (x.dim() - 2) + [-1] if cl else [-1] + [1] * (x.dim() - 2))
                    v = x * sc.view(shape) + sh.view(shape)
                    if kw.get("swish"):
                        v = v * torch.sigmoid(v)
                self.rows.append((kind, tuple(x.shape), float(v.abs().max()), float(conv.weight.abs().max())))
                self.layers.append(conv)
                return orig(x, conv, *a, **k)
            return f

        for k, o in self._orig.items():
            setattr(self._mod, k, wrap(k, o))
        return self

    def __exit__(self, *exc):
        for k, o in self._orig.items():
            setattr(self._mod, k, o)
        if self._pre is None:
            os.environ.pop("P2PB_EXPERIMENT", None)
        else:
            os.environ["P2PB_EXPERIMENT"] = self._pre

    @property
    def worst(self):
        return max((r[2] for r in self.rows), default=0.0)

    @property
    def ok(self):
        return self.worst < self.LIMIT / 4
```

p2p_bridge_amd/pvcnn_unet.py:

```python
from dataclasses import dataclass
from typing import Any, List, Optional

import numpy as np
import os

import torch

from . import _experiment
import torch.nn as nn
import torch.nn.functional as F

from . import layers as L


def _get(cfg, key, default=None):
    if cfg is None:
        return default
    if isinstance(cfg, dict):
        v = cfg.get(key, None)
    else:
        v = getattr(cfg, key, None)
        if v is None and hasattr(cfg, "get"):
            v = cfg.get(key, None)
    return default if v is None else v
# ... 85 lines not shown
    def forward(ctx, qkv, heads):
        from ._lib import call, check, ptr, stream_ptr
        import ctypes

        qkv = qkv.contiguous()
        check(qkv, torch.float32, "qkv")
        b, c3, n = qkv.shape
        dh = c3 // (3 * heads)
        out = torch.empty(b, heads * dh, n, dtype=qkv.dtype, device=qkv.device)
        need = ctx.needs_input_grad[0]
        ctxm = torch.empty(b, heads, dh, dh, dtype=qkv.dtype, device=qkv.device) if need else None
        call("p2pb_linear_attention_forward", ctypes.c_int(b), ctypes.c_int(heads), ctypes.c_int(dh), ctypes.c_int(n),
             ptr(qkv), ptr(out), ptr(ctxm), stream_ptr())
        if need:
            ctx.save_for_backward(qkv, ctxm)
            ctx.heads = heads
        return out

    @staticmethod
    def backward(ctx, g):
        from ._lib import call, ptr, stream_ptr
        import ctypes

        qkv, ctxm = ctx.saved_tensors
        b, c3, n = qkv.shape
        heads = ctx.heads
        dq = torch.empty_like(qkv)
        g = g.contiguous()
        from ._lib import check

        check(g, torch.float32, "grad_out")
        call("p2pb_linear_attention_backward", ctypes.c_int(b), ctypes.c_int(heads), ctypes.c_int(c3 // (3 * heads)),
             ctypes.c_int(n), ptr(qkv), ptr(ctxm), ptr(g), ptr(dq), stream_ptr())
        return dq, None


class LinearAttention(nn.Module):

    def __init__(self, dim, heads=4, dim_head=32):
        super().__init__()
        self.heads = heads
        hidden = dim_head * heads
        self.to_qkv = nn.Conv2d(dim, hidden * 3, 1, bias=False)
        self.to_out = nn.Conv2d(hidden, dim, 1)

    def forward(self, x):
        from . import fused

        b, c, n = x.shape
        if fused.enabled(self, x):
            qkv, _ = fused.pw_conv(x.contiguous(), self.to_qkv, stats=False, use_bias=False)
            out = _LinearAttentionCore.apply(qkv, self.heads)
            return fused.pw_conv(out, self.to_out, stats=False)[0]
        from . import dense

        qkv = dense.pointwise(x.unsqueeze(-1), self.to_qkv).view(b, -1, n)
        out = _LinearAttentionCore.apply(qkv, self.heads)
        return dense.pointwise(out.unsqueeze(-1), self.to_out).squeeze(-1)


class _SoftmaxAttentionCore(torch.autograd.Function):

    @staticmethod
    def forward(ctx, q, kv, heads):
        from ._lib import call, check, ptr, stream_ptr
        import ctypes

        q, kv = q.contiguous(), kv.contiguous()
        check(q, torch.float32, "q")
        check(kv, torch.float32, "kv")
        b, c, n = q.shape
        if c % heads or tuple(kv.shape) != (b, 2 * c, n) or kv.device != q.device:
            raise RuntimeError(f"q {tuple(q.shape)} / kv {tuple(kv.shape)}: expected [B, heads*32, n] and [B, 2*heads*32, n] "
                               f"with heads = {heads}")
        need = any(ctx.needs_input_grad[:2])
        out = torch.empty_like(q)
        lse = torch.empty(b, heads, n, dtype=q.dtype, device=q.device) if need else None
        call("p2pb_softmax_attention_forward", ctypes.c_int(b), ctypes.c_int(heads), ctypes.c_int(c // heads), ctypes.c_int(n),
             ptr(q), ptr(kv), ptr(out), ptr(lse), stream_ptr())
        if need:
            ctx.save_for_backward(q, kv, out, lse)
            ctx.heads = heads
        return out

    @staticmethod
    def backward(ctx, g):
        from ._lib import call, check, ptr, stream_ptr
        import ctypes

        q, kv, out, lse = ctx.saved_tensors
        b, c, n = q.shape
        heads = ctx.heads
        g = g.contiguous()
        check(g, torch.float32, "grad_out")
        dq, dkv = torch.empty_like(q), torch.empty_like(kv)
        call("p2pb_softmax_attention_backward", ctypes.c_int(b), ctypes.c_int(heads), ctypes.c_int(c // heads), ctypes.c_int(n),
             ptr(q), ptr(kv), ptr(out), ptr(lse), ptr(g), ptr(dq), ptr(dkv), stream_ptr())
        return dq, dkv, None


class Attention(nn.Module):

    def __init__(self, dim, heads=4, dim_head=32):
        super().__init__()
        self.heads = heads
        hidden = dim_head * heads
        self.to_q = nn.Linear(dim, hidden, bias=False)
        self.to_kv = nn.Linear(dim, hidden * 2, bias=False)
        self.to_out = nn.Linear(hidden, dim, bias=False)

    def forward(self, x):
        from . import fused
        from ._lib import check

        x = x.contiguous()
        check(x, torch.float32, "x")
        if fused.enabled(self, x):
            q, _ = fused.pw_conv(x, self.to_q, stats=False, use_bias=False)
            kv, _ = fused.pw_conv(x, self.to_kv, stats=False, use_bias=False)
            out = _SoftmaxAttentionCore.apply(q, kv, self.heads)
            return fused.pw_conv(out, self.to_out, stats=False, use_bias=False)[0]
        from . import dense

        if not dense.enabled(x):
            raise RuntimeError("Attention: the HIP training kernels are switched off and there is no eager form")
        out = _SoftmaxAttentionCore.apply(dense.pointwise(x, self.to_q), dense.pointwise(x, self.to_kv), self.heads)
        return dense.pointwise(out, self.to_out)


class StyleBank:

    def __init__(self, net: nn.Module):
        self.mods = [m for m in net.modules() if isinstance(m, AdaGN)]
        self.key = None
        self.weight = self.bias = None
        self.slices = {}

    def _ensure_slices(self):
        if not self.slices:
            off = 0
            for m in self.mods:
                n2 = m.emd.weight.shape[0]
                self.slices[id(m)] = (off, off + n2)
                off += n2

    def _refresh(self):
        self._ensure_slices()
        key = tuple((m.emd.weight.data_ptr(), m.emd.weight._version, m.emd.bias._version) for m in self.mods)
        if key != self.key:
            self.weight = torch.cat([m.emd.weight.detach() for m in self.mods], dim=0).contiguous()
            self.bias = torch.cat([m.emd.bias.detach() for m in self.mods], dim=0).contiguous()
            self.key = key

    def evaluate(self, cond):
        self._refresh()
        from . import fused

        return _Styles(cond, fused.linear_rows(cond, self.weight, self.bias), self.slices)

    def evaluate_train(self, cond, decoder_ids=None):
        self._ensure_slices()
        parts, cut = {}, []
        groups = [(self.mods, cond)]
        if decoder_ids:
            alias = cond.view_as(cond) if cond.requires_grad else cond
            cut = [alias]
            groups = [([m for m in self.mods if id(m) not in decoder_ids], cond),
                      ([m for m in self.mods if id(m) in decoder_ids], alias)]
        styles = None
        for mods, vec in groups:
            if not mods:
                continue
            w = torch.cat([m.emd.weight for m in mods], dim=0)
            b = torch.cat([m.emd.bias for m in mods], dim=0)
            styles = F.linear(vec, w, b)
            bounds, off = [], 0
            for m in mods:
                bounds.append((off, off + m.emd.weight.shape[0]))
                off = bounds[-1][1]
            parts.update({id(m): t for m, t in zip(mods, _SplitColumns.apply(styles, tuple(bounds)))})
        out = _Styles(cond, styles if len(groups) == 1 else None, self.slices, parts)
        out.cut = cut
        return out


class _SplitColumns(torch.autograd.Function):

    @staticmethod
    def forward(ctx, x, bounds):
        ctx.bounds, ctx.rows = bounds, x.shape[0]
        ctx.set_materialize_grads(False)
        return tuple(x[:, lo:hi] for lo, hi in bounds)

    @staticmethod
    def backward(ctx, *grads):
        ref = next((g for g in grads if g is not None), None)
        if ref is None:
            return None, None
        parts = [g if g is not None else ref.new_zeros(ctx.rows, hi - lo) for g, (lo, hi) in zip(grads, ctx.bounds)]
        return torch.cat(parts, dim=1), None


class _Styles:

    def __init__(self, vector, styles, slices, parts=None):
        self.vector, self.styles, self.slices, self.parts = vector, styles, slices, parts
        self.cut = []

    def style(self, adagn):
        if self.parts is not None:
            return self.parts[id(adagn)]
        lo, hi = self.slices[id(adagn)]
        return self.styles[:, lo:hi]


def _group_norm_of(norm):
    return norm.norm if isinstance(norm, AdaGN) else (norm.group_norm if isinstance(norm, MyGroupNorm) else norm)


def norm_affine(norm, part, count, cond, want_mean=False):
    from . import fused

    style = None
    if isinstance(norm, AdaGN):
        if cond is None:
            raise RuntimeError("AdaGN needs the global embedding")
        style = cond.style(norm) if isinstance(cond, _Styles) else norm.emd(cond)
    gn = _group_norm_of(norm)
    out = fused.gn_affine_params(part, count, gn.num_groups, gn.weight, gn.bias, style, gn.eps, want_mean)
    return out if want_mean else out[:2]


def norm_fin(norm, count, cond, want_mean=False):
    style = None
    if isinstance(norm, AdaGN):
        if cond is None:
            raise RuntimeError("AdaGN needs the global embedding")
        style = cond.style(norm) if isinstance(cond, _Styles) else norm.emd(cond)
    gn = _group_norm_of(norm)
    return (count, gn.num_groups, gn.weight, gn.bias, style, gn.eps, want_mean)


class SharedMLP(nn.Module):

    def __init__(self, in_channels, out_channels, dim=1, gn_groups=8, cond_dim=0, affine=True):
        super().__init__()
        conv = nn.Conv1d if dim == 1 else nn.Conv2d
        if not isinstance(out_channels, (list, tuple)):
            out_channels = [out_channels]
        mods = []
        for oc in out_channels:
            mods.append(conv(in_channels, oc, 1))
            mods.append(AdaGN(oc, cond_dim, dim, gn_groups) if cond_dim > 0 else nn.GroupNorm(gn_groups, oc,
                                                                                             affine=affine))
            mods.append(Swish())
            in_channels = oc
        self.layers = nn.ModuleList(mods)

    def run(self, x, cond, reduce_max=False, residual=None, rgate=None, dropout=None):
        from . import fused

        if fused.enabled(self, x):
            if rgate is not None:
                residual = residual * rgate.unsqueeze(-1)
            return self._run_fused(x, cond, reduce_max, residual)
        from . import dense

        n = len(self.layers) // 3
        fold = residual is not None and not reduce_max and n > 0
        for i in range(n):
            last = fold and i == n - 1
            x = dense.conv_norm_act(x, self.layers[3 * i], self.layers[3 * i + 1], cond, swish=True,
                                    residual=residual if last else None, rgate=rgate if last else None, dropout=dropout if i == n - 1 else None)
        if reduce_max:
            x = dense.row_max(x)
        if residual is None or fold:
            return x
        return (residual if rgate is None else residual * rgate.unsqueeze(-1)) + x

    def _run_fused(self, x, cond, reduce_max, residual, first=None):
        from . import fused

        shape = x.shape
        B, P = shape[0], int(np.prod(shape[2:]))
        h = x.reshape(B, shape[1], P)
        if not h.is_contiguous():
            h = h.contiguous()
        sc = sh = None
        nl = len(self.layers) // 3
        if first is not None:
            sc, sh = norm_affine(self.layers[1], first, P, cond)
            if nl == 1:
                C = h.shape[1]
                if reduce_max:
                    return fused.affine_act_max(h, sc, sh, int(np.prod(shape[2:-1])), shape[-1]).view(B, C, *shape[2:-1])
                return fused.affine_act(h, sc, sh, True, None).view(B, C, *shape[2:])
        pool = reduce_max and fused.pool_supported(P, shape[-1])
        for i in range(1 if first is not None else 0, nl):
            conv, norm = self.layers[3 * i], self.layers[3 * i + 1]
            if pool and i == nl - 1:
                _, st, mm, (sc, sh, _) = fused.pw_conv(h, conv, sc, sh, swish=sc is not None, pool_u=shape[-1], store=False,
                                                       fin=norm_fin(norm, P, cond))
                return fused.minmax_act(mm, sc, sh).view(B, conv.weight.shape[0], *shape[2:-1])
            h, st, (sc, sh, _) = fused.pw_conv(h, conv, sc, sh, swish=sc is not None, fin=norm_fin(norm, P, cond))
        C = h.shape[1]
        if reduce_max:
            return fused.affine_act_max(h, sc, sh, int(np.prod(shape[2:-1])), shape[-1]).view(B, C, *shape[2:-1])
        res = None if residual is None else residual.reshape(B, C, P)
        return fused.affine_act(h, sc, sh, True, res).view(B, C, *shape[2:])

    def forward(self, data: PVCData) -> PVCData:
        data.features = self.run(data.features, data.cond)
        return data


class Voxelization(nn.Module):

    def __init__(self, resolution, normalize=True, eps=0.0):
        super().__init__()
        self.r, self.normalize, self.eps = int(resolution), normalize, eps

    def forward(self, features, coords):
        norm, vox = L.voxel_coords(coords.detach().contiguous(), self.r, self.normalize, self.eps)
        if features is None:
            return features, norm
        return L.avg_voxelize(features, vox, self.r), norm


class PVConv(nn.Module):

    def __init__(self, in_channels, out_channels, resolution, with_se=True, dropout=0.1, gn_groups=8, cond_dim=0,
                 normalize=True, eps=0.0, attention=None):
        super().__init__()
        self.resolution = int(resolution)
        self.voxelization = Voxelization(resolution, normalize, eps)
        norm = (lambda c: AdaGN(c, cond_dim, 3, gn_groups)) if cond_dim > 0 else (lambda c: nn.GroupNorm(gn_groups, c))
        mods = [nn.Conv3d(in_channels, out_channels, 3, stride=1, padding=1), norm(out_channels), Swish(),
                nn.Dropout(dropout), nn.Conv3d(out_channels, out_channels, 3, stride=1, padding=1), norm(out_channels)]
        if with_se:
            mods.append(SE3d(out_channels))
        self.voxel_layers = nn.ModuleList(mods)
        self.attn = attention(out_channels) if attention is not None else None
        self.sparse_conv = True
        self.level = -1
        self.point_features = SharedMLP(in_channels, out_channels, gn_groups=gn_groups, cond_dim=cond_dim)
        self._pass, self.drop_salt = None, 0

    def _voxel_branch_fused(self, features, coords, cond, point=None, geo=None):
        from . import fused

        vl, r = self.voxel_layers, self.resolution
        geo_v = geo.take_voxel(self.level, r) if (geo is not None and self.level >= 0) else None
        lists = counts = None
        pre1 = pre2 = False
        if geo_v is not None:
            vcoords, cnt, ws, lists, counts = geo_v
            pre1, pre2 = fused.conv_pre_plan(r)
            pre1, pre2 = pre1 and fused.pinned_math(vl[0]) is None, pre2 and fused.pinned_math(vl[4]) is None
            v = fused.voxelize_cl_gather(features.contiguous(), cnt, ws, r, split=pre1)
        else:
            vcoords, vox = L.voxel_coords(coords.detach().contiguous(), r, self.voxelization.normalize,
                                          self.voxelization.eps)
            v, cnt = fused.voxelize_cl(features.contiguous(), vox, r)
        r3 = float(r ** 3)
        c1, c2 = compact_plan()
        if self.sparse_conv and (r in c1 or r in c2):
            if lists is None:
                lists, counts = fused.active_lists(cnt, r)
            if r in c1:
                y1, st1 = fused.conv3d_k3_compact(v, vl[0], lists, counts, 0, pre=pre1)
            else:
                y1, st1 = fused.conv3d_k3(v, vl[0], compact=True, channels_last=True, pre=pre1)
            if r in c2:
                sc1, sh1, a, k = fused.conv3d_far_field_gn(vl[0].bias, vl[4], st1, norm_fin(vl[1], r3, cond), True)
                if pre2:
                    y2, st2 = fused.conv3d_k3_compact(fused.conv3d_presplit(y1, sc1, sh1, True, a), vl[4], lists, counts, 1,
                                                      out_class=k, pre=True, listed_only=True)
                else:
                    y2, st2 = fused.conv3d_k3_compact(y1, vl[4], lists, counts, 1, sc1, sh1, True, in_sub=a, out_class=k,
                                                      listed_only=True)
            else:
                sc1, sh1 = norm_affine(vl[1], st1, r3, cond)
                if pre2:
                    y2, st2 = fused.conv3d_k3(fused.conv3d_presplit(y1, sc1, sh1, True), vl[4], compact=True, channels_last=True, pre=True)
                else:
                    y2, st2 = fused.conv3d_k3(y1, vl[4], sc1, sh1, swish=True, compact=True, channels_last=True)
        elif r >= 32 and self.sparse_conv:
            if lists is None:
                lists, counts = fused.brick_lists(cnt, r)
            y1, st1 = fused.conv3d_k3_sparse(v, vl[0], lists, counts, 0, channels_last=True, pre=pre1)
            sc1, sh1, a, k = fused.conv3d_far_field_gn(vl[0].bias, vl[4], st1, norm_fin(vl[1], r3, cond), True)
            if pre2:
                y2, st2 = fused.conv3d_k3_sparse(fused.conv3d_presplit(y1, sc1, sh1, True, a), vl[4], lists, counts, 1,
                                                 out_class=k, channels_last=True, pre=True, active_only=True)
            else:
                y2, st2 = fused.conv3d_k3_sparse(y1, vl[4], lists, counts, 1, sc1, sh1, True, in_sub=a, out_class=k,
                                                 channels_last=True, active_only=True)
        else:
            y1, st1 = fused.conv3d_k3(v, vl[0], compact=True, channels_last=True, pre=pre1)
            sc1, sh1 = norm_affine(vl[1], st1, r3, cond)
            if pre2:
                y2, st2 = fused.conv3d_k3(fused.conv3d_presplit(y1, sc1, sh1, True), vl[4], compact=True, channels_last=True, pre=True)
            else:
                y2, st2 = fused.conv3d_k3(y1, vl[4], sc1, sh1, swish=True, compact=True, channels_last=True)
        se = vl[6] if len(vl) > 6 else None
        aff_a, aff_b, scp, shp = fused.pvconv_tail(st2, norm_fin(vl[5], r3, cond), None if se is None else (se.fc[0].weight, se.fc[2].weight),
                                                   None if point is None else (point[1], point[2]))
        return fused.devoxelize_affine(y2, vcoords, r, aff_a, aff_b, channels_last=True,
                                       add=None if point is None else (point[0], scp, shp))

    def forward(self, data: PVCData) -> PVCData:
        coords, features, cond = data.coords, data.features, data.cond
        assert features.shape[0] == coords.shape[0] and features.shape[2] == coords.shape[2] and coords.shape[1] == 3
        if not self.training and not torch.is_grad_enabled() and self.resolution in FUSED_RESOLUTIONS:
            pf = self.point_features.layers
            if len(pf) == 3 and features.is_cuda:
                from . import fused as F_

                feats = features.contiguous()
                h, st = F_.pw_conv(feats, pf[0])
                data.features = self._voxel_branch_fused(feats, coords, cond, point=(h, st, norm_fin(pf[1], feats.shape[2], cond)),
                                                         geo=data.geo)
                if self.attn is not None:
                    data.features = self.attn(data.features)
                return data
            fused = self._voxel_branch_fused(features, coords, cond, geo=data.geo)
        else:
            from . import dense

            v, vcoords = self.voxelization(features, coords)
            vl = self.voxel_layers
            seed = self._pass.get("drop_seed") if (self._pass is not None and self.training and vl[3].p > 0 and v.is_cuda) else None
            v = dense.conv_norm_act(v, vl[0], vl[1], cond, swish=True, occ=L.occupancy_of(v),
                                    dropout=None if seed is None else (float(vl[3].p), seed, self.drop_salt))
            if seed is None:
                v = vl[3](v)
            if len(vl) > 6 and v.is_cuda:
                v, vmean = dense.conv_norm_act(v, vl[4], vl[5], cond, swish=False, want_mean=True)
                gate = dense.se_gate(vmean, vl[6].fc)
                dv = L.trilinear_devoxelize(v, vcoords, self.resolution, self.training)
                data.features = self.point_features.run(features, cond, residual=dv, rgate=gate)
                if self.attn is not None:
                    data.features = self.attn(data.features)
                return data
            v = dense.conv_norm_act(v, vl[4], vl[5], cond, swish=False)
            if len(vl) > 6:
                v = vl[6](v)
            fused = L.trilinear_devoxelize(v, vcoords, self.resolution, self.training)
        data.features = self.point_features.run(features, cond, residual=fused)
        if self.attn is not None:
            data.features = self.attn(data.features)
        return data


FUSED_RESOLUTIONS = (4, 8, 16, 32)


def compact_plan():
    import os

    from . import fused

    if fused.conv_math() not in fused.SPLIT_MATHS:
        return set(), set()
    spec = _experiment.get("compact", "16:16")
    parts = (spec.split(":") + [""])[:2]
    return tuple({int(t) for t in p.split(",") if t.strip()} for p in parts)


class BallQuery(nn.Module):

    def __init__(self, radius, num_neighbors, include_coordinates=True):
        super().__init__()
        self.radius, self.num_neighbors, self.include_coordinates = radius, num_neighbors, include_coordinates

    def forward(self, points_coords, centers_coords, points_features=None):
        points_coords = points_coords.contiguous()
        centers_coords = centers_coords.contiguous()
        idx = L.ball_query(centers_coords, points_coords, self.radius, self.num_neighbors)
        if (points_features is not None and self.include_coordinates and points_features.is_cuda and points_features.dtype == torch.float32
                and not points_coords.requires_grad and not centers_coords.requires_grad and _experiment.get_int("group_concat", 1)):
            return L.GroupConcat.apply(points_coords, centers_coords, points_features, idx)
        rel = L.pvcnn_grouping(points_coords, idx) - centers_coords.unsqueeze(-1)
        if points_features is None:
            return rel
        feats = L.pvcnn_grouping(points_features, idx)
        return torch.cat([rel, feats], dim=1) if self.include_coordinates else feats


class PointNetSAModule(nn.Module):

    def __init__(self, num_centers, radius, num_neighbors, in_channels, out_channels, gn_groups=8, cond_dim=0):
        super().__init__()
        self.num_centers = num_centers
        self.level = -1
        self.out_channels = out_channels[-1]
        self.groupers = nn.ModuleList([BallQuery(radius, num_neighbors, True)])
        self.mlps = nn.ModuleList([SharedMLP(in_channels + 3, out_channels, dim=2, gn_groups=gn_groups,
                                             cond_dim=cond_dim)])

    def forward(self, data: PVCData) -> PVCData:
        coords = data.coords[:, :3]
        if data.geo is not None:
            centers, nidx = data.geo.take_sa(self.level)
            if data.time_emb is not None:
                data.time_emb = data.time_emb[:, :, : centers.shape[-1]]
            mlp = self.mlps[0]
            from . import fused

            if fused.enabled(mlp, coords) and data.features is not None:
                conv0 = mlp.layers[0]
                xin = torch.cat([coords, data.features], dim=1)
                cen = centers.contiguous()
                pm = xin.shape[2] % 4 == 0 and cen.shape[2] % 4 == 0
                z, _ = fused.pw_conv(xin, conv0, stats=False, point_major=pm)
                cx, _ = fused.pw_conv(cen, conv0, stats=False, ci_lo=0, ci_hi=3, use_bias=False, point_major=pm)
                M, U = nidx.shape[1], nidx.shape[2]
                c1 = conv0.weight.shape[0]
                if pm and len(mlp.layers) == 6 and fused.gather_pool_supported(c1, mlp.layers[3].weight.shape[0], M, U):
                    _, st = fused.group_sub(z, cx, nidx, point_major=True, stats_only=True)
                    sc, sh = norm_affine(mlp.layers[1], st, M * U, data.cond)
                    st2, mm, (sc2, sh2, _) = fused.pw_conv_pool_gather(z, cx, nidx, mlp.layers[3], sc, sh, True,
                                                                       fin=norm_fin(mlp.layers[4], M * U, data.cond))
                    data.features = fused.minmax_act(mm, sc2, sh2)
                else:
                    y, st = fused.group_sub(z, cx, nidx, point_major=pm)
                    data.features = mlp._run_fused(y.view(y.shape[0], y.shape[1], M, U), data.cond, True, None, first=st)
            else:
                grouped = L._ext.group_concat(coords.contiguous(), centers, data.features.contiguous(), nidx)
                data.features = mlp.run(grouped, data.cond, reduce_max=True)
            data.coords = centers
            return data
        centers = L.furthest_point_sample_pvcnn(coords, self.num_centers)
        if data.time_emb is not None:
            data.time_emb = temb_at(data.time_emb, centers.shape[-1])
        grouped = self.groupers[0](coords, centers, data.features)
        data.features = self.mlps[0].run(grouped, data.cond, reduce_max=True)
        data.coords = centers
        return data


class PointNetFPModule(nn.Module):

    def __init__(self, in_channels, out_channels, gn_groups=8, cond_dim=0):
        super().__init__()
        self.level = -1
        self.mlp = SharedMLP(in_channels, list(out_channels), dim=1, gn_groups=gn_groups, cond_dim=cond_dim)

    def forward(self, data: PVCData) -> PVCData:
        if data.geo is not None:
            idx, w = data.geo.take_fp(self.level)
            from . import fused

            if fused.enabled(self.mlp, data.lower_features):
                conv0 = self.mlp.layers[0]
                g = data.lower_features.contiguous()
                cg = g.shape[1]
                pm = g.shape[2] % 4 == 0
                tb = None
                if data.lower_temb is not None:
                    e = data.lower_temb.shape[1]
                    tb = fused.linear_rows(data.lower_temb, conv0.weight.reshape(conv0.weight.shape[0], -1)[:, cg:cg + e])
                cz, _ = fused.pw_conv(g, conv0, stats=False, ci_lo=0, ci_hi=cg, use_bias=False, point_major=pm, bias_b=tb)
                if tb is not None:
                    cg += data.lower_temb.shape[1]
                skip = data.features
                if skip is not None:
                    ys, _ = fused.pw_conv(skip.contiguous(), conv0, stats=False, ci_lo=cg, ci_hi=cg + skip.shape[1])
                    y, st = fused.interp_add(cz, idx, w, add=ys, point_major=pm)
                else:
                    y, st = fused.interp_add(cz, idx, w, bias=conv0.bias, point_major=pm)
                if data.time_emb is not None:
                    data.time_emb = data.time_emb[:, :, 0:1].expand(-1, -1, data.coords.shape[-1])
                data.features = self.mlp._run_fused(y, data.cond, False, None, first=st)
                return data
            x = L.three_interpolate(data.lower_features.contiguous(), idx, w)
        else:
            x = L.nearest_neighbor_interpolate(data.coords, data.lower_coords, data.lower_features)
        if data.features is not None:
            x = torch.cat([x, data.features], dim=1)
        if data.time_emb is not None:
            data.time_emb = temb_at(data.time_emb, data.coords.shape[-1])
        data.features = self.mlp.run(x, data.cond)
        return data


class MyGroupNorm(nn.Module):

    def __init__(self, num_groups, num_channels):
        super().__init__()
        self.num_channels = num_channels - num_channels % num_groups
        self.group_norm = nn.GroupNorm(num_groups, self.num_channels)

    def forward(self, x):
        if x.shape[1] == self.num_channels:
            return self.group_norm(x)
        return torch.cat([self.group_norm(x[:, : self.num_channels]), x[:, self.num_channels:]], dim=1)


class _PnetMLP(nn.Module):

    def __init__(self, cin, cout):
        super().__init__()
        self.mlp = nn.Sequential(nn.Conv2d(cin, cout, kernel_size=1, bias=True), MyGroupNorm(32, cout), Swish())

    def forward(self, x):
        from . import dense

        return dense.conv_norm_act(x, self.mlp[0], self.mlp[1], None, swish=True)


class ConditionedSharedMLPLayer(nn.Module):

    def __init__(self, channels):
        super().__init__()
        assert len(channels) > 2
        self.shared_mlp_0 = _PnetMLP(channels[0], channels[1])
        self.shared_mlp_1 = _PnetMLP(channels[1], channels[2])
        self.last_mlp_layers = nn.ModuleList([_PnetMLP(a, b) for a, b in zip(channels[2:-1], channels[3:])])

    def forward(self, x):
        x = self.shared_mlp_1(self.shared_mlp_0(x))
        for m in self.last_mlp_layers:
            x = m(x)
        return x


class Pnet2Stage(nn.Module):

    def __init__(self, mlp1, mlp2):
        super().__init__()
        self.mlp1 = ConditionedSharedMLPLayer(mlp1)
        self.mlp2 = ConditionedSharedMLPLayer([2 * mlp1[-1]] + mlp2)

    def forward(self, coords):
        from . import fused

        if fused.enabled(self, coords) and self._fusable():
            return self._forward_fused(coords)
        from . import dense

        f = self.mlp1(coords.unsqueeze(-1))
        g = dense.row_max(f.squeeze(-1))[:, :, None, None].expand(-1, -1, f.size(2), -1)
        f = self.mlp2(torch.cat([f, g], dim=1))
        return dense.row_max(f.squeeze(-1))

    def _fusable(self):
        ok = len(self.mlp1.last_mlp_layers) == 0 and len(self.mlp2.last_mlp_layers) == 0
        for blk in (self.mlp1.shared_mlp_0, self.mlp1.shared_mlp_1, self.mlp2.shared_mlp_0, self.mlp2.shared_mlp_1):
            ok = ok and blk.mlp[1].num_channels == blk.mlp[0].out_channels
        return ok

    def _forward_fused(self, coords):
        from . import fused

        N = coords.shape[2]
        a0, a1 = self.mlp1.shared_mlp_0.mlp, self.mlp1.shared_mlp_1.mlp
        b0, b1 = self.mlp2.shared_mlp_0.mlp, self.mlp2.shared_mlp_1.mlp
        h, st, (sc, sh, _) = fused.pw_conv(coords.contiguous(), a0[0], fin=norm_fin(a0[1], N, None))
        pool = fused.pool_supported(N, 0)
        if pool:
            h, st, mm = fused.pw_conv(h, a1[0], sc, sh, swish=True, pool_u=0)
            g, sc, sh = fused.minmax_act_pool_gn(mm, st, norm_fin(a1[1], N, None))
        else:
            h, st, (sc, sh, _) = fused.pw_conv(h, a1[0], sc, sh, swish=True, fin=norm_fin(a1[1], N, None))
            g = fused.affine_act_max(h, sc, sh, N, 0)
        c1 = h.shape[1]
        w = b0[0].weight.reshape(b0[0].out_channels, -1)
        bias_b = fused.linear_rows(g, w[:, c1:])
        h, st, (sc, sh, _) = fused.pw_conv(h, b0[0], sc, sh, swish=True, bias_b=bias_b, ci_lo=0, ci_hi=c1, fin=norm_fin(b0[1], N, None))
        if pool:
            _, st, mm = fused.pw_conv(h, b1[0], sc, sh, swish=True, pool_u=0, store=False)
            return fused.minmax_act_pool_gn(mm, st, norm_fin(b1[1], N, None))[0]
        h, st, (sc, sh, _) = fused.pw_conv(h, b1[0], sc, sh, swish=True, fin=norm_fin(b1[1], N, None))
        return fused.affine_act_max(h, sc, sh, N, 0)




def stage_plan(npoints: int, channels: List[int], n_sa_blocks: List[int], n_fp_blocks: List[int],
               radius: List[float], voxel_resolutions: List[int], feat_dim: int, input_dim: int = 3,
               embed_dim: int = 64, centers: Optional[List[int]] = None, attentions: Optional[List[int]] = None):
    nlev = len(channels) - 1
    sa, sa_in = [], []
    cin = feat_dim + input_dim
    for i in range(nlev):
        sa_in.append(cin)
        ncen = npoints // 4 ** (i + 1) if centers is None else centers[i]
        convs = []
        last = i == nlev - 1
        if not last:
            for p in range(n_sa_blocks[i] if i == 0 else min(1, n_sa_blocks[i])):
                convs.append(dict(cin=cin + (embed_dim if (i > 0 and p == 0) else 0), cout=channels[i],
                                  r=int(voxel_resolutions[i]),
                                  attn=bool(attentions[i]) and p == 0 if attentions is not None else False))
                cin = channels[i]
        mlp_in = cin + (embed_dim if (i > 0 and not convs) else 0)
        mlp_out = [channels[i], channels[i], channels[i + 1]] if last else [channels[i], channels[i + 1]]
        sa.append(dict(convs=convs, centers=ncen, radius=radius[i], neighbors=32, mlp_in=mlp_in, mlp_out=mlp_out))
        cin = mlp_out[-1]
    sa_in[0] = feat_dim + input_dim
    fp_mlps = [[channels[3], channels[3]], [channels[3], channels[3]], [channels[3], channels[2]],
               [channels[2], channels[2], channels[1]]]
    fp_conv = [(channels[3], n_fp_blocks[3], voxel_resolutions[3]), (channels[3], n_fp_blocks[2], voxel_resolutions[2]),
               (channels[2], n_fp_blocks[1], voxel_resolutions[1]), (channels[1], n_fp_blocks[0], voxel_resolutions[0])]
    fp = []
    for j in range(4):
        mlp_in = cin + sa_in[-1 - j] + embed_dim
        convs = []
        c = fp_mlps[j][-1]
        for _ in range(fp_conv[j][1]):
            convs.append(dict(cin=c, cout=fp_conv[j][0], r=int(fp_conv[j][2])))
            c = fp_conv[j][0]
        fp.append(dict(mlp_in=mlp_in, mlp_out=fp_mlps[j], convs=convs))
        cin = c
    return dict(sa=sa, fp=fp, bottleneck=sa[-1]["mlp_out"][-1], out=cin)


class Geometry:

    def __init__(self, plan, coords, side):
        main = torch.cuda.current_stream()
        self.main = main
        c0 = coords.contiguous()
        side.wait_stream(main)
        self.sa, self.fp = [], []
        from . import fused

        self.voxel = {}
        vox_plan = {}
        for (lev, r, normalize, eps) in plan.get("voxel", ()):
            vox_plan.setdefault(lev, []).append((r, normalize, eps))

        def voxel_prep(i, c, stream):
            for (r, normalize, eps) in vox_plan.get(i, ()):
                if r not in FUSED_RESOLUTIONS:
                    continue
                vcoords, vox = L.voxel_coords(c, r, normalize, eps)
                cnt, ws = fused.voxel_sort(vox, r)
                lists = counts = None
                c1, c2 = compact_plan()
                if r in c1 or r in c2:
                    lists, counts = fused.active_lists(cnt, r)
                elif r == 32:
                    lists, counts = fused.brick_lists(cnt, r)
                ev = torch.cuda.Event()
                ev.record(stream)
                self.voxel[(i, r)] = (vcoords, cnt, ws, lists, counts, ev)

        voxel_prep(0, c0, main)
        with torch.cuda.stream(side):
            level_coords = []
            c = c0
            for i, st in enumerate(plan["sa"]):
                level_coords.append(c)
                if i > 0:
                    voxel_prep(i, c, side)
                idx = L._ext.furthest_point_sampling_forward(c, st["centers"])
                cen = L._ext.gather_features_forward(c, idx)
                nidx = L._ext.ball_query(cen, c, st["radius"], st["neighbors"])
                ev = torch.cuda.Event()
                ev.record(side)
                self.sa.append((cen, nidx, ev))
                c = cen
            lower = c
            for j in range(len(plan["fp"])):
                pts = level_coords[-1 - j]
                idx, w = L._ext.three_nn(pts, lower)
                ev = torch.cuda.Event()
                ev.record(side)
                self.fp.append((idx, w, ev))
                lower = pts
        self.join = torch.cuda.Event()
        self.join.record(side)

    def _take(self, items, level):
        *vals, ev = items[level]
        self.main.wait_event(ev)
        for v in vals:
            v.record_stream(self.main)
        return vals

    def take_voxel(self, level, r):
        item = self.voxel.get((level, r))
        if item is None:
            return None
        *vals, ev = item
        self.main.wait_event(ev)
        for v in vals:
            if v is not None:
                v.record_stream(self.main)
        return vals

    def take_sa(self, level):
        return self._take(self.sa, level)

    def take_fp(self, level):
        return self._take(self.fp, level)

    def finish(self):
        self.main.wait_event(self.join)


class _Stage(nn.Sequential):

    def forward(self, data):
        for m in self:
            data = m(data)
        return data


class PVCNN2Unet(nn.Module):
    def __init__(self, cfg, return_layers: bool = False):
        super().__init__()
        m = _get(cfg, "model")
        pvd = _get(m, "PVD")
        self.input_dim = _get(m, "in_dim", 3)
        extra = _get(pvd, "extra_feature_channels", None)
        self.extra_feature_channels = extra if extra is not None else _get(m, "extra_feature_channels", 0)
        self.embed_dim = _get(m, "time_embed_dim", 64)
        out_dim = _get(m, "out_dim", 3)
        dropout = _get(m, "dropout", None)
        dropout = 0.1 if dropout is None else dropout
        heads = _get(pvd, "attention_heads", 4)
        with_se = _get(pvd, "use_se", True)
        E = self.embed_dim

        self.embedf = nn.Sequential(nn.Linear(E, E), nn.LeakyReLU(0.1, inplace=True), nn.Linear(E, E))
        if _get(pvd, "use_global_embedding", False):
            c = self.cond_emb_dim = _get(pvd, "global_embedding_dim")
            self.global_pnet = Pnet2Stage([self.input_dim, c // 8, c // 4], [c // 2, c])
        else:
            self.global_pnet, self.cond_emb_dim = None, 0
        self.f_embed_dim = _get(pvd, "feat_embed_dim", self.extra_feature_channels)
        self.embed_feats = None
        if self.f_embed_dim != self.extra_feature_channels:
            fin = self.extra_feature_channels or self.input_dim
            self.embed_feats = nn.Sequential(nn.Conv1d(fin, self.f_embed_dim, 1), nn.GroupNorm(8, self.f_embed_dim),
                                             Swish(), nn.Conv1d(self.f_embed_dim, self.f_embed_dim, 1))

        plan = stage_plan(_get(_get(cfg, "data"), "npoints"), list(_get(pvd, "channels")), list(_get(pvd, "n_sa_blocks")),
                          list(_get(pvd, "n_fp_blocks")), list(_get(pvd, "radius")),
                          list(_get(pvd, "voxel_resolutions")), self.f_embed_dim, self.input_dim, E,
                          _get(pvd, "centers", None), _get(pvd, "attentions", None))
        self.plan = plan
        cd = self.cond_emb_dim
        attn_type = str(_get(pvd, "attention_type", "linear")).lower()
        if attn_type == "linear":
            attn_fn = lambda dim: LinearAttention(dim, heads=heads)
        elif attn_type == "flash":
            attn_fn = lambda dim: Attention(dim, heads=heads)
        else:
            attn_fn = None
        if attn_type != "linear" and any(s.get("attn") for st in plan["sa"] for s in st["convs"]):
            raise ValueError(f"attention_type={attn_type!r} with model.PVD.attentions={list(_get(pvd, 'attentions'))}: a PVConv-"
                             "level attention (a flag on a stage that has a PVConv) exists for attention_type 'linear' only; "
                             "flag only the last stage (the stock [0, 0, 0, 1])")
        pv = lambda s: PVConv(s["cin"], s["cout"], s["r"], with_se=with_se, dropout=dropout, cond_dim=cd,
                              attention=attn_fn if s.get("attn") else None)
        sa_layers = []
        for st in plan["sa"]:
            blocks = [pv(s) for s in st["convs"]]
            blocks.append(PointNetSAModule(st["centers"], st["radius"], st["neighbors"], st["mlp_in"], st["mlp_out"],
                                           cond_dim=cd))
            sa_layers.append(blocks[0] if len(blocks) == 1 else _Stage(*blocks))
        self.sa_layers = nn.ModuleList(sa_layers)
        nlev = len(plan["sa"])
        for i, stage in enumerate(self.sa_layers):
            (stage[-1] if isinstance(stage, _Stage) else stage).level = i
            for blk in (stage if isinstance(stage, _Stage) else [stage]):
                if isinstance(blk, PVConv):
                    blk.level = i
        self.global_att = attn_fn(plan["bottleneck"]) if attn_fn is not None else None
        fp_layers = []
        for st in plan["fp"]:
            blocks = [PointNetFPModule(st["mlp_in"], st["mlp_out"], cond_dim=cd)] + [pv(s) for s in st["convs"]]
            fp_layers.append(blocks[0] if len(blocks) == 1 else _Stage(*blocks))
        self.fp_layers = nn.ModuleList(fp_layers)
        for j, stage in enumerate(self.fp_layers):
            (stage[0] if isinstance(stage, _Stage) else stage).level = j
            for blk in (stage if isinstance(stage, _Stage) else [stage]):
                if isinstance(blk, PVConv):
                    blk.level = nlev - 1 - j
        self.plan["voxel"] = sorted({(m.level, m.resolution, bool(m.voxelization.normalize), float(m.voxelization.eps))
                                     for m in self.modules() if isinstance(m, PVConv)})
        self._side_streams = {}
        out_mlp = _get(pvd, "out_mlp", 128)
        self.classifier = nn.ModuleList([SharedMLP(plan["out"], out_mlp, cond_dim=0), nn.Dropout(dropout),
                                         nn.Conv1d(out_mlp, out_dim, 1)])
        half = E // 2
        freq = torch.from_numpy(np.exp(np.arange(0, half) * -(np.log(10000) / (half - 1)))).float()
        self.register_buffer("_temb_freq", freq, persistent=False)
        self._style_bank = None
        self.overlap_geometry = True
        self.collect_cut, self.cut = False, None
        self._dec_adagn = None
        self._pass = {"drop_seed": None}
        for k, m in enumerate(m for m in self.modules() if isinstance(m, PVConv)):
            m._pass, m.drop_salt = self._pass, k + 1

    def get_timestep_embedding(self, timesteps, device=None):
        if timesteps.dim() == 2 and timesteps.shape[1] == 1:
            timesteps = timesteps[:, 0]
        assert timesteps.dim() == 1, f"get shape: {timesteps.shape}"
        e = timesteps[:, None] * self._temb_freq[None, :]
        e = torch.cat([torch.sin(e), torch.cos(e)], dim=1)
        if self.embed_dim % 2 == 1:
            e = F.pad(e, (0, 1), "constant", 0)
        return e

    def _decoder_adagns(self):
        if self._dec_adagn is None:
            self._dec_adagn = {id(m) for part in (self.global_att, self.fp_layers, self.classifier) if part is not None
                               for m in part.modules() if isinstance(m, AdaGN)}
        return self._dec_adagn

    def forward(self, x, t, x_cond=None):
        if x_cond is not None:
            x = torch.cat([x, x_cond], dim=1)
        B, C, N = x.shape
        assert C == self.input_dim + self.extra_feature_channels, \
            f"input dim: {C}, expected: {self.input_dim + self.extra_feature_channels}"
        coords = x[:, : self.input_dim].contiguous()
        feats = x[:, self.input_dim:].contiguous()
        from . import fused

        use_fused = fused.enabled(self, x)
        geo = None
        if use_fused and self.overlap_geometry:
            dev = x.device
            if dev not in self._side_streams:
                self._side_streams[dev] = torch.cuda.Stream(device=dev)
            geo = Geometry(self.plan, coords, self._side_streams[dev])
        if self.embed_feats is not None:
            src = coords if self.extra_feature_channels == 0 else feats
            if use_fused:
                h, st, (sc, sh, _) = fused.pw_conv(src, self.embed_feats[0], fin=norm_fin(self.embed_feats[1], N, None))
                feats, _ = fused.pw_conv(h, self.embed_feats[3], sc, sh, swish=True, stats=False)
            else:
                from . import dense

                e = self.embed_feats
                feats = dense.pointwise(dense.conv_norm_act(src, e[0], e[1], None, swish=True), e[3])
        cond = self.global_pnet(coords) if self.global_pnet is not None else None
        if cond is not None and x.is_cuda:
            if self._style_bank is None:
                self._style_bank = StyleBank(self)
            if use_fused:
                cond = self._style_bank.evaluate(cond)
            else:
                cond = self._style_bank.evaluate_train(cond, self._decoder_adagns() if self.collect_cut else None)
        feats = torch.cat([coords, feats], dim=1)
        self._pass["drop_seed"] = None
        if not use_fused and self.training and x.is_cuda and self.classifier[1].p > 0:
            from . import dense

            if dense.fold_step_neighbours():
                self._pass["drop_seed"] = dense.dropout_seed(x.device)
        time_emb = None
        if t is not None:
            if t.dim() == 0:
                t = t.view(1).expand(B)
            te = self.get_timestep_embedding(t)
            if use_fused:
                te = fused.linear_rows(te, self.embedf[0].weight, self.embedf[0].bias)
                te = fused.linear_rows(F.leaky_relu(te, self.embedf[1].negative_slope), self.embedf[2].weight, self.embedf[2].bias)
            else:
                te = self.embedf(te)
            time_emb = temb_broadcast(te, N)
        data = PVCData(features=feats, coords=coords, time_emb=time_emb, cond=cond, geo=geo)

        skips, level_coords = [feats], []
        for i, stage in enumerate(self.sa_layers):
            if i > 0:
                skips.append(data.features)
            level_coords.append(data.coords)
            if i > 0 and data.time_emb is not None:
                data.features = torch.cat([data.features, data.time_emb], dim=1)
            data = stage(data)

        if self.collect_cut and torch.is_grad_enabled():
            def alias(x):
                return x.view_as(x) if x.requires_grad else x

            data.features = alias(data.features)
            skips = [alias(x) for x in skips]
            cut = [data.features] + skips
            if data.time_emb is not None and te.requires_grad:
                te_c = alias(te)
                data.time_emb = temb_broadcast(te_c, data.coords.shape[-1])
                cut.append(te_c)
            if isinstance(cond, _Styles):
                cut += cond.cut
            self.cut = [x for x in cut if x.requires_grad]

        if self.global_att is not None:
            data.features = self.global_att(data.features)

        for j, stage in enumerate(self.fp_layers):
            ltemb = None
            if data.time_emb is None:
                lower = data.features
            elif use_fused and geo is not None and data.time_emb.shape[1] % 4 == 0 and data.features.shape[1] % 4 == 0:
                lower, ltemb = data.features, data.time_emb[:, :, 0]
            else:
                lower = torch.cat([data.features, data.time_emb], dim=1)
            data = stage(PVCData(features=skips[-1 - j], coords=level_coords[-1 - j], lower_coords=data.coords,
                                 lower_features=lower, time_emb=data.time_emb, cond=data.cond, geo=geo, lower_temb=ltemb))
        if geo is not None:
            geo.finish()

        if use_fused:
            c0 = self.classifier[0]
            xin = data.features.contiguous()
            h, st, (sc, sh, _) = fused.pw_conv(xin, c0.layers[0], fin=norm_fin(c0.layers[1], xin.shape[2], None))
            return fused.pw_conv(h, self.classifier[2], sc, sh, swish=True, stats=False)[0]
        from . import dense

        seed = self._pass["drop_seed"]
        if seed is not None:
            h = self.classifier[0].run(data.features, None, dropout=(float(self.classifier[1].p), seed, 0))
        else:
            h = self.classifier[1](self.classifier[0].run(data.features, None))
        return dense.pointwise(h, self.classifier[2])
```

Measured before the change: 1.152 million points/s.

## Fold GroupNorm finisher into consumer pointwise conv prologue

Adds a lazy NormFold path. The GroupNorm statistics reduction and affine computation that used to run as a separate finisher kernel after a pointwise conv are deferred, then computed inside the next pointwise split kernel's prologue in LDS, as long as the slot count and channel count are small enough. This removes one kernel launch and one global round trip of the scale and shift per folded layer. In exchange, every block of the consumer kernel repeats the stats reduction, and consumers that cannot fold fall back to a separate launch.

```diff
diff --git a/include/p2pb_hip.h b/include/p2pb_hip.h
--- a/include/p2pb_hip.h
+++ b/include/p2pb_hip.h
@@ -9,7 +9,7 @@
 
 #define P2PB_EINVAL (-22)
 
-#define P2PB_ABI_VERSION 9
+#define P2PB_ABI_VERSION 10
 
 int p2pb_version(void);
 const char *p2pb_target_arch(void);
@@ -24,6 +24,10 @@
                          int style_stride, float eps, float *scale, float *shift, float *chmean);
 int p2pb_gn_finisher_armed(void);
 void p2pb_gn_finisher_disarm(void);
+int p2pb_gn_fold_arm(int c, int groups, int nslots, double count_per_channel, const float *part, const float *gamma,
+                     const float *beta, const float *style, int style_stride, float eps, float *scale, float *shift);
+void p2pb_gn_fold_disarm(void);
+void p2pb_debug_fold_counts(unsigned long long *in_kernel, unsigned long long *launched);
 
 int p2pb_voxel_coords(int b, int n, int r, int normalize, float eps, const float *coords, float *norm,
                       int *vox, void *stream);
diff --git a/p2p_bridge_amd/_lib.py b/p2p_bridge_amd/_lib.py
--- a/p2p_bridge_amd/_lib.py
+++ b/p2p_bridge_amd/_lib.py
@@ -24,7 +24,7 @@
     "p2pb_pointwise_split_packed_bytes", "p2pb_pointwise_pack_weights_split", "p2pb_pointwise_pool_supported", "p2pb_pointwise_minmax_floats", "p2pb_pointwise_conv_pool_forward",
     "p2pb_minmax_act", "p2pb_linear_attention_forward", "p2pb_linear_attention_backward", "p2pb_softmax_attention_forward", "p2pb_softmax_attention_backward",
     "p2pb_approxmatch_temp_floats", "p2pb_approxmatch_forward_ws", "p2pb_pointwise_conv_pool_gather", "p2pb_chamfer_ws_bytes", "p2pb_chamfer_forward_ws", "p2pb_radius_count", "p2pb_radius_fill", "p2pb_merge_accumulate", "p2pb_merge_finish", "p2pb_gn_affine_params_ex", "p2pb_norm_act_backward", "p2pb_norm_act_backward_ex", "p2pb_grouping_backward_pitched", "p2pb_three_nn_interpolate_backward_pitched", "p2pb_affine_act_train", "p2pb_conv3d_k3_wgrad_ws_floats", "p2pb_conv3d_k3_wgrad", "p2pb_conv3d_k3_wgrad_occ_ws_floats", "p2pb_conv3d_k3_wgrad_occ", "p2pb_pointwise_wgrad_ws_floats", "p2pb_pointwise_wgrad",
-    "p2pb_debug_pointwise_form", "p2pb_linear_rows", "p2pb_gn_finisher_arm", "p2pb_gn_finisher_armed", "p2pb_gn_finisher_disarm", "p2pb_fps_grid_ws_bytes", "p2pb_furthest_point_sampling_grid",
+    "p2pb_debug_pointwise_form", "p2pb_linear_rows", "p2pb_gn_finisher_arm", "p2pb_gn_finisher_armed", "p2pb_gn_finisher_disarm", "p2pb_gn_fold_arm", "p2pb_gn_fold_disarm", "p2pb_debug_fold_counts", "p2pb_fps_grid_ws_bytes", "p2pb_furthest_point_sampling_grid",
     "p2pb_optim_entry_bytes", "p2pb_optim_chunk", "p2pb_optim_clip_adam_step",
     "p2pb_conv3d_k3_pack_weights_split_adjoint", "p2pb_pointwise_pack_weights_adjoint", "p2pb_pointwise_pack_weights_split_adjoint",
     "p2pb_conv3d_k3_pack_weights_split_amax", "p2pb_pointwise_pack_weights_split_amax",
@@ -33,7 +33,7 @@
     "p2pb_occupancy_grid_cells", "p2pb_occupancy_ws_bytes", "p2pb_occupancy_counts",
 ]
 
-ABI_VERSION = 9
+ABI_VERSION = 10
 
 _lib = None
 
diff --git a/p2p_bridge_amd/csrc/abi.hip b/p2p_bridge_amd/csrc/abi.hip
--- a/p2p_bridge_amd/csrc/abi.hip
+++ b/p2p_bridge_amd/csrc/abi.hip
@@ -128,3 +128,27 @@
   tl_fin_armed = false;
   return true;
 }
+
+namespace {
+thread_local bool tl_fold_armed = false;
+thread_local GnFold tl_fold;
+}
+extern "C" int p2pb_gn_fold_arm(int c, int groups, int nslots, double count_per_channel, const float *part, const float *gamma,
+                                const float *beta, const float *style, int style_stride, float eps, float *scale, float *shift) {
+  if (c <= 0 || nslots <= 0 || !part || !scale || !shift || !(count_per_channel > 0.0) || !gn_shape_ok(c, groups, style, style_stride) ||
+      tl_fold_armed)
+    return P2PB_EINVAL;
+  GnFinish &f = tl_fold.f;
+  f.gamma = gamma, f.beta = beta, f.style = style, f.scale = scale, f.shift = shift, f.chmean = nullptr;
+  f.count_per_channel = count_per_channel, f.style_stride = style_stride, f.groups = groups, f.eps = eps;
+  tl_fold.part = part, tl_fold.nslots = nslots, tl_fold.c = c;
+  tl_fold_armed = true;
+  return 0;
+}
+extern "C" void p2pb_gn_fold_disarm(void) { tl_fold_armed = false; }
+bool p2pb_gn_fold_take(GnFold *out) {
+  if (!tl_fold_armed) return false;
+  *out = tl_fold;
+  tl_fold_armed = false;
+  return true;
+}
diff --git a/p2p_bridge_amd/csrc/common.h b/p2p_bridge_amd/csrc/common.h
--- a/p2p_bridge_amd/csrc/common.h
+++ b/p2p_bridge_amd/csrc/common.h
@@ -108,6 +108,70 @@
   return groups > 0 && c % groups == 0 && c / groups <= 256 && !(style && style_stride < 2 * c);
 }
 typedef float gnf_f32x2 __attribute__((ext_vector_type(2)));
+__device__ __forceinline__ void gnf_slot_sums(const float *__restrict__ p0, size_t pitch, int j, int nt, int nslots, double &s, double &q) {
+  int sl = j;
+  for (; sl + 7 * nt < nslots; sl += 8 * nt) {
+    gnf_f32x2 v[8];
+#pragma unroll
+    for (int u = 0; u < 8; ++u) {
+      const float *pp = p0 + (size_t)(sl + u * nt) * pitch;
+      v[u] = *(const gnf_f32x2 *)pp;
+    }
+#pragma unroll
+    for (int u = 0; u < 8; ++u) {
+      s += (double)v[u][0];
+      q += (double)v[u][1];
+    }
+  }
+  for (; sl + 3 * nt < nslots; sl += 4 * nt) {
+    gnf_f32x2 v[4];
+#pragma unroll
+    for (int u = 0; u < 4; ++u) {
+      const float *pp = p0 + (size_t)(sl + u * nt) * pitch;
+      v[u] = *(const gnf_f32x2 *)pp;
+    }
+#pragma unroll
+    for (int u = 0; u < 4; ++u) {
+      s += (double)v[u][0];
+      q += (double)v[u][1];
+    }
+  }
+  for (; sl < nslots; sl += nt) {
+    const float *p = p0 + (size_t)sl * pitch;
+    s += (double)p[0];
+    q += (double)p[1];
+  }
+}
+__device__ __forceinline__ void gnf_channel_sum(const double *rs, const double *rq, int cg, int nt, int t, double &ts, double &tq) {
+  ts = 0.0, tq = 0.0;
+  for (int jj = 0; jj < nt; ++jj) {
+    ts += rs[jj * cg + t];
+    tq += rq[jj * cg + t];
+  }
+}
+struct GnfAffine {
+  double sc, sh, mean, rstd;
+  float cm;
+};
+__device__ __forceinline__ GnfAffine gnf_group_fold(const double *chs, const double *chq, int cg, int t, double count_per_channel, float eps,
+                                                   float p_ga, float p_be, float p_fa, float p_bi) {
+  double gs = 0.0, gq = 0.0;
+  for (int kk = 0; kk < cg; ++kk) {
+    gs += chs[kk];
+    gq += chq[kk];
+  }
+  GnfAffine a;
+  const double n = count_per_channel * cg;
+  a.mean = gs / n;
+  double var = gq / n - a.mean * a.mean;
+  if (var < 0.0) var = 0.0;
+  a.rstd = 1.0 / sqrt(var + (double)eps);
+  const double ga = (double)p_ga, be = (double)p_be, fa = (double)p_fa, bi = (double)p_bi;
+  a.sc = a.rstd * ga * fa;
+  a.sh = (be - a.mean * a.rstd * ga) * fa + bi;
+  a.cm = (float)(a.sc * (chs[t] / count_per_channel) + a.sh);
+  return a;
+}
 __device__ __forceinline__ void gn_finish_group_v(int c, int nslots, const float *__restrict__ part, const GnFinish &f, int b, int g,
                                                   double *lds, int vt, bool live, float *mean_rstd = nullptr,
                                                   float *tab_scale = nullptr, float *tab_shift = nullptr, float *tab_mean = nullptr) {
@@ -127,83 +191,74 @@
     }
   }
   double s = 0.0, q = 0.0;
-  if (live && j < nt) {
-    const float *p0 = part + ((size_t)b * nslots * c + g0 + k) * 2;
-    const size_t pitch = (size_t)c * 2;
-    int sl = j;
-    for (; sl + 7 * nt < nslots; sl += 8 * nt) {
-      gnf_f32x2 v[8];
-#pragma unroll
-      for (int u = 0; u < 8; ++u) {
-        const float *pp = p0 + (size_t)(sl + u * nt) * pitch;
-        v[u] = *(const gnf_f32x2 *)pp;
-      }
-#pragma unroll
-      for (int u = 0; u < 8; ++u) {
-        s += (double)v[u][0];
-        q += (double)v[u][1];
-      }
-    }
-    for (; sl + 3 * nt < nslots; sl += 4 * nt) {
-      gnf_f32x2 v[4];
-#pragma unroll
-      for (int u = 0; u < 4; ++u) {
-        const float *pp = p0 + (size_t)(sl + u * nt) * pitch;
-        v[u] = *(const gnf_f32x2 *)pp;
-      }
-#pragma unroll
-      for (int u = 0; u < 4; ++u) {
-        s += (double)v[u][0];
-        q += (double)v[u][1];
-      }
-    }
-    for (; sl < nslots; sl += nt) {
-      const float *p = p0 + (size_t)sl * pitch;
-      s += (double)p[0];
-      q += (double)p[1];
-    }
-  }
+  if (live && j < nt) gnf_slot_sums(part + ((size_t)b * nslots * c + g0 + k) * 2, (size_t)c * 2, j, nt, nslots, s, q);
   if (live) {
     rs[t] = s;
     rq[t] = q;
   }
   __syncthreads();
   if (live && t < cg) {
-    double ts = 0.0, tq = 0.0;
-    for (int jj = 0; jj < nt; ++jj) {
-      ts += rs[jj * cg + t];
-      tq += rq[jj * cg + t];
-    }
+    double ts, tq;
+    gnf_channel_sum(rs, rq, cg, nt, t, ts, tq);
     chs[t] = ts;
     chq[t] = tq;
   }
   __syncthreads();
   if (live && t < cg) {
-    double gs = 0.0, gq = 0.0;
-    for (int kk = 0; kk < cg; ++kk) {
-      gs += chs[kk];
-      gq += chq[kk];
-    }
     const int ch = g0 + t;
-    const double n = f.count_per_channel * cg;
-    const double mean = gs / n;
-    double var = gq / n - mean * mean;
-    if (var < 0.0) var = 0.0;
-    const double rstd = 1.0 / sqrt(var + (double)f.eps);
-    const double ga = (double)p_ga, be = (double)p_be, fa = (double)p_fa, bi = (double)p_bi;
-    const double sc = rstd * ga * fa;
-    const double sh = (be - mean * rstd * ga) * fa + bi;
-    const float cm = (float)(sc * (chs[t] / f.count_per_channel) + sh);
-    if (f.scale) f.scale[(size_t)b * c + ch] = (float)sc;
-    if (f.shift) f.shift[(size_t)b * c + ch] = (float)sh;
-    if (f.chmean) f.chmean[(size_t)b * c + ch] = cm;
-    if (tab_scale) tab_scale[ch] = (float)sc;
-    if (tab_shift) tab_shift[ch] = (float)sh;
-    if (tab_mean) tab_mean[ch] = cm;
+    const GnfAffine a = gnf_group_fold(chs, chq, cg, t, f.count_per_channel, f.eps, p_ga, p_be, p_fa, p_bi);
+    if (f.scale) f.scale[(size_t)b * c + ch] = (float)a.sc;
+    if (f.shift) f.shift[(size_t)b * c + ch] = (float)a.sh;
+    if (f.chmean) f.chmean[(size_t)b * c + ch] = a.cm;
+    if (tab_scale) tab_scale[ch] = (float)a.sc;
+    if (tab_shift) tab_shift[ch] = (float)a.sh;
+    if (tab_mean) tab_mean[ch] = a.cm;
     if (mean_rstd && t == 0) {
-      mean_rstd[((size_t)b * f.groups + g) * 2] = (float)mean;
-      mean_rstd[((size_t)b * f.groups + g) * 2 + 1] = (float)rstd;
-    }
+      mean_rstd[((size_t)b * f.groups + g) * 2] = (float)a.mean;
+      mean_rstd[((size_t)b * f.groups + g) * 2 + 1] = (float)a.rstd;
+    }
+  }
+  __syncthreads();
+}
+struct GnFold {
+  const float *part;
+  int nslots, c;
+  GnFinish f;
+};
+constexpr __host__ __device__ size_t gn_fold_lds_doubles(int c, int groups) { return (size_t)groups * 512 + 2 * (size_t)c; }
+template <int NT>
+__device__ __forceinline__ void gn_fold_sample(const GnFold &fo, int b, double *lds, float *tab_scale, float *tab_shift) {
+  const GnFinish &f = fo.f;
+  const int c = fo.c, groups = f.groups, cg = c / groups, nt = 256 / cg, tid = (int)threadIdx.x;
+  double *rs = lds, *rq = lds + (size_t)groups * 256, *chs = lds + (size_t)groups * 512, *chq = chs + c;
+  for (int v = tid; v < groups * 256; v += NT) {
+    const int g = v >> 8, t = v & 255, k = t % cg, j = t / cg;
+    double s = 0.0, q = 0.0;
+    if (j < nt) gnf_slot_sums(fo.part + ((size_t)b * fo.nslots * c + g * cg + k) * 2, (size_t)c * 2, j, nt, fo.nslots, s, q);
+    rs[v] = s;
+    rq[v] = q;
+  }
+  __syncthreads();
+  for (int ch = tid; ch < c; ch += NT) {
+    const int g = ch / cg;
+    double ts, tq;
+    gnf_channel_sum(rs + g * 256, rq + g * 256, cg, nt, ch - g * cg, ts, tq);
+    chs[ch] = ts;
+    chq[ch] = tq;
+  }
+  __syncthreads();
+  for (int ch = tid; ch < c; ch += NT) {
+    const int g = ch / cg;
+    float p_ga = 1.0f, p_be = 0.0f, p_fa = 1.0f, p_bi = 0.0f;
+    if (f.gamma) p_ga = f.gamma[ch];
+    if (f.beta) p_be = f.beta[ch];
+    if (f.style) {
+      p_fa = f.style[(size_t)b * f.style_stride + ch];
+      p_bi = f.style[(size_t)b * f.style_stride + c + ch];
+    }
+    const GnfAffine a = gnf_group_fold(chs + g * cg, chq + g * cg, cg, ch - g * cg, f.count_per_channel, f.eps, p_ga, p_be, p_fa, p_bi);
+    tab_scale[ch] = (float)a.sc;
+    tab_shift[ch] = (float)a.sh;
   }
   __syncthreads();
 }
@@ -341,6 +396,7 @@
 void p2pb_note_pointwise_form(int cin, int cout, int npos, int form);
 bool p2pb_gn_finisher_take(GnFinish *out);
 int p2pb_gn_affine_launch(int b, int c, int nslots, const float *part, const GnFinish &f, hipStream_t s);
+bool p2pb_gn_fold_take(GnFold *out);
 
 long p2pb_experiment_long(const char *key, long dflt);
 
diff --git a/p2p_bridge_amd/csrc/pointwise.hip b/p2p_bridge_amd/csrc/pointwise.hip
--- a/p2p_bridge_amd/csrc/pointwise.hip
+++ b/p2p_bridge_amd/csrc/pointwise.hip
@@ -715,7 +715,7 @@
                                                        const float *__restrict__ in_scale,
                                                        const float *__restrict__ in_shift, int in_swish,
                                                        float *__restrict__ out, float *__restrict__ stats_part,
-                                                       float *__restrict__ mm_out, int pool_u, int out_pm) {
+                                                       float *__restrict__ mm_out, int pool_u, int out_pm, GnFold fold) {
   extern __shared__ u32x4 pws_lds[];
   constexpr int NT = 128 * WM;
   constexpr int BS = 128 * NB;
@@ -792,6 +792,9 @@
                                          (__attribute__((address_space(3))) void *)(dst + i * NT + wave * 64), 16, 0, 0);
   };
   load_b(0);
+  float *fold_tab = (float *)(pws_lds + (WM / 2 + NB) * PWS_TILE);
+  const bool folded = XF && fold.part != nullptr;
+  if (folded) gn_fold_sample<NT>(fold, b, (double *)pws_lds, fold_tab, fold_tab + cin);
 
   for (int ci0 = 0; ci0 < cin; ci0 += PWS_CK) {
     __syncthreads();
@@ -802,7 +805,7 @@
 #pragma unroll
         for (int i = 0; i < 8; ++i) {
           const int c = min(ci0 + 8 * bgrp + i, cin - 1);
-          const float sc = in_scale[b * cin + c], sh = in_shift[b * cin + c];
+          const float sc = folded ? fold_tab[c] : in_scale[b * cin + c], sh = folded ? fold_tab[cin + c] : in_shift[b * cin + c];
 #pragma unroll
           for (int q = 0; q < NBW; ++q)
 #pragma unroll
@@ -967,14 +970,54 @@
   return p2pb_gn_affine_launch(b, cout, (P + 255) / 256 * 4, stats_part, tl_pw_fin, s);
 }
 
+static thread_local GnFold tl_pw_fold;
+static thread_local bool tl_pw_fold_have = false;
+static std::atomic<unsigned long long> g_fold_in_kernel{0}, g_fold_launched{0};
+extern "C" void p2pb_debug_fold_counts(unsigned long long *in_kernel, unsigned long long *launched) {
+  if (in_kernel) *in_kernel = g_fold_in_kernel.load();
+  if (launched) *launched = g_fold_launched.load();
+}
+static int pw_fold_resolve(bool has_prologue, size_t scratch_bytes, int b, int cin, const float *&in_scale, const float *&in_shift,
+                           GnFold *kernel_fold, hipStream_t s) {
+  *kernel_fold = GnFold();
+  if (!tl_pw_fold_have) return 0;
+  tl_pw_fold_have = false;
+  const GnFold &fo = tl_pw_fold;
+  if (in_scale || in_shift || fo.c != cin) return P2PB_EINVAL;
+  static const long max_slots = p2pb_experiment_long("norm_prologue", 16);
+  if (has_prologue && fo.nslots <= max_slots && cin <= 512 && gn_fold_lds_doubles(cin, fo.f.groups) * 8 <= scratch_bytes) {
+    *kernel_fold = fo;
+    ++g_fold_in_kernel;
+    return 0;
+  }
+  ++g_fold_launched;
+  in_scale = fo.f.scale, in_shift = fo.f.shift;
+  return p2pb_gn_affine_launch(b, cin, fo.nslots, fo.part, fo.f, s);
+}
+static int pw_fold_done(int rc) {
+  if (tl_pw_fold_have) {
+    tl_pw_fold_have = false;
+    return rc ? rc : P2PB_EINVAL;
+  }
+  return rc;
+}
+
 static int pw_launch_split(int b, int cin, int cout, int P, const float *in, const void *wp, const float *bias,
                            const float *bias_b, const float *in_scale, const float *in_shift, int in_swish,
                            float *out, float *stats_part, float *minmax, int pool_u, int out_pm, hipStream_t s) {
-  const bool xf = in_scale != nullptr;
   const int mode = p2pb_g_split_terms;
   static const int wm_env = (int)p2pb_experiment_long("pw_wm", 0);
   const bool wm4 = !out_pm && (wm_env ? wm_env == 4
                                        : (cout >= 512 && (long)((P + 127) / 128) * ((cout + 255) / 256) * b >= 1024));
+  static const int pp_env = (int)p2pb_experiment_long("pw_pp", 1);
+  const bool pp = pp_env && wm4 && mode == SPLIT_F16X3 && cin % 64 == 0 && cout % 512 == 0 && (!minmax || pool_u == 0) &&
+                  (size_t)cin * P * 4 < (1ull << 31);
+  GnFold fold;
+  const int frc = pw_fold_resolve(!pp && mode != SPLIT_BF16X3, (size_t)((wm4 ? 2 : 1) + 1) * PWS_TILE * 16, b, cin, in_scale, in_shift,
+                                  &fold, s);
+  if (frc) return frc;
+  const bool xf = in_scale != nullptr || fold.part != nullptr;
+  const int fold_lds = fold.part ? 2 * cin * 4 : 0;
   dim3 grid((P + 127) / 128, wm4 ? (cout + 255) / 256 : (cout + 127) / 128, b);
   const int nslots = (P + 255) / 256 * 4;
   const u32x4 *w = (const u32x4 *)wp;
@@ -984,11 +1027,12 @@
     const int lds = (WM / 2 + NB) * PWS_TILE * 16;                                                                   \
     if (!once) {                                                                                                     \
       (void)hipFuncSetAttribute((const void *)pw_split_kernel<XF, PL, WM, NB, TM>,                                   \
-                                hipFuncAttributeMaxDynamicSharedMemorySize, lds);                                    \
+                                hipFuncAttributeMaxDynamicSharedMemorySize, lds + 4096);                             \
       once = true;                                                                                                   \
     }                                                                                                                \
-    hipLaunchKernelGGL((pw_split_kernel<XF, PL, WM, NB, TM>), grid, dim3(128 * WM), lds, s, cin, cout, P, nslots, in, \
-                       w, bias, bias_b, in_scale, in_shift, in_swish, out, stats_part, minmax, pool_u, out_pm);       \
+    hipLaunchKernelGGL((pw_split_kernel<XF, PL, WM, NB, TM>), grid, dim3(128 * WM), lds + fold_lds, s, cin, cout, P, \
+                       nslots, in, w, bias, bias_b, in_scale, in_shift, in_swish, out, stats_part, minmax, pool_u,   \
+                       out_pm, fold);                                                                                \
   } while (0)
 #define LAUNCHF(XF, PL, WM, NB)                                       \
   do {                                                                \
@@ -1007,9 +1051,7 @@
     if (wm4) LAUNCHF(XF, PL, 4, 1);        \
     else LAUNCHF(XF, PL, 2, 1);            \
   } while (0)
-  static const int pp_env = (int)p2pb_experiment_long("pw_pp", 1);
-  if (pp_env && wm4 && mode == SPLIT_F16X3 && cin % 64 == 0 && cout % 512 == 0 && (!minmax || pool_u == 0) &&
-      (size_t)cin * P * 4 < (1ull << 31)) {
+  if (pp) {
     dim3 pgrid((P + 127) / 128, cout / 512, b);
 #define LAUNCHP5(XF, PL)                                                                                              \
   do {                                                                                                                \
@@ -1057,6 +1099,11 @@
 static int pw_launch(int b, int cin, int cout, int P, const float *in, const float *wp, const float *bias,
                      const float *bias_b, const float *in_scale, const float *in_shift, int in_swish, float *out,
                      float *stats_part, float *minmax, int pool_g, int out_pm, hipStream_t s, bool split_pack = false) {
+  {
+    GnFold none;
+    const int rc = pw_fold_resolve(false, 0, b, cin, in_scale, in_shift, &none, s);
+    if (rc) return rc;
+  }
   const bool xf = in_scale != nullptr, st = stats_part != nullptr;
   if (split_pack && (!pw_wide_ok(P, in, out) || p2pb_g_split_terms != SPLIT_F16X3)) return P2PB_EINVAL;
   if (pw_wide_ok(P, in, out)) {
@@ -1137,8 +1184,9 @@
                                            const float *in_shift, int in_swish, int flags, float *out,
                                            float *stats_part, void *stream) {
   tl_pw_fin_pending = p2pb_gn_finisher_take(&tl_pw_fin);
-  const int rc = pw_conv_forward_impl(b, cin, cout, npos, in, wp_any, bias, bias_b, in_scale, in_shift, in_swish, flags, out,
-                                      stats_part, stream);
+  tl_pw_fold_have = p2pb_gn_fold_take(&tl_pw_fold);
+  const int rc = pw_fold_done(pw_conv_forward_impl(b, cin, cout, npos, in, wp_any, bias, bias_b, in_scale, in_shift, in_swish, flags,
+                                                   out, stats_part, stream));
   return pw_finish_behind(rc, b, cout, npos, stats_part, (hipStream_t)stream);
 }
 
@@ -1188,8 +1236,9 @@
                                                 float *out, float *stats_part, int pool_u, float *minmax,
                                                 void *stream) {
   tl_pw_fin_pending = p2pb_gn_finisher_take(&tl_pw_fin);
-  const int rc = pw_conv_pool_forward_impl(b, cin, cout, npos, in, wp_any, bias, bias_b, in_scale, in_shift, in_swish, flags, out,
-                                           stats_part, pool_u, minmax, stream);
+  tl_pw_fold_have = p2pb_gn_fold_take(&tl_pw_fold);
+  const int rc = pw_fold_done(pw_conv_pool_forward_impl(b, cin, cout, npos, in, wp_any, bias, bias_b, in_scale, in_shift, in_swish,
+                                                        flags, out, stats_part, pool_u, minmax, stream));
   return pw_finish_behind(rc, b, cout, npos, stats_part, (hipStream_t)stream);
 }
 
diff --git a/p2p_bridge_amd/fused.py b/p2p_bridge_amd/fused.py
--- a/p2p_bridge_amd/fused.py
+++ b/p2p_bridge_amd/fused.py
@@ -452,6 +452,37 @@
             and npos % 4 == 0)
 
 
+class NormFold:
+
+    def __init__(self, part, fin):
+        self.part, self.fin, self._arrays = part, fin, None
+
+    def arrays(self):
+        if self._arrays is None:
+            count, groups, gamma, beta, style, eps, _ = self.fin
+            self._arrays = gn_affine_params(self.part, count, groups, gamma, beta, style, eps)[:2]
+        return self._arrays
+
+
+def norm_prologue() -> bool:
+    return _experiment.get_int("norm_prologue", 16) > 0
+
+
+def fold_arrays(scale, shift):
+    return scale.arrays() if isinstance(scale, NormFold) else (scale, shift)
+
+
+def _arm_fold(fold, b, c, device):
+    count, groups, gamma, beta, style, eps, _ = fold.fin
+    assert tuple(fold.part.shape[::2]) == (b, c), "fold of another tensor"
+    scale = torch.empty(b, c, dtype=F32, device=device)
+    shift = torch.empty_like(scale)
+    style, stride = _style_arg(style, c)
+    call("p2pb_gn_fold_arm", _i(c), _i(int(groups)), _i(fold.part.shape[1]), _d(float(count)), ptr(fold.part), ptr(gamma), ptr(beta),
+         ptr(style), _i(stride), _f(eps), ptr(scale), ptr(shift))
+    return scale, shift, style
+
+
 def arm_finisher(fin, b, c, device):
     count, groups, gamma, beta, style, eps, want_mean = fin
     scale = torch.empty(b, c, dtype=F32, device=device)
@@ -469,13 +500,13 @@
 
 @_honours_pin(1)
 def pw_conv(x, conv, in_scale=None, in_shift=None, swish=False, stats=True, bias_b=None, ci_lo=0, ci_hi=None,
-            use_bias=True, pool_u=None, store=True, math=None, point_major=False, fin=None):
+            use_bias=True, pool_u=None, store=True, math=None, point_major=False, fin=None, lazy=False):
     check(x, F32, "x")
     b, ci, p = x.shape
     co = conv.out_channels if getattr(conv, "adjoint", False) else conv.weight.shape[0]
     split = use_split_pw(ci, co, p, math)
     if in_scale is not None and (co + (127 if split else 63)) // (128 if split else 64) >= _experiment.get_int("prepass_blocks", 9):
-        x = affine_act(x, in_scale, in_shift, swish)
+        x = affine_act(x, *fold_arrays(in_scale, in_shift), swish)
         in_scale = in_shift = None
         swish = False
     point_major = point_major and not stats and pool_u is None and p % 4 == 0
@@ -493,19 +524,29 @@
         nfl = lib().p2pb_pointwise_stats_floats(_i(b), _i(co), _i(p))
         st = torch.empty(b, nfl // (b * co * 2), co, 2, dtype=F32, device=x.device)
     bias = conv.bias if use_bias else None
-    aff = keep = None
-    if fin is not None:
+    aff = keep = keep_fold = None
+    armed = fin is not None and not (lazy and not fin[6] and norm_prologue())
+    if armed:
         assert st is not None
         aff, keep = arm_finisher(fin, b, co, x.device)
+    elif fin is not None:
+        assert st is not None
+        aff = (NormFold(st, fin), None, None)
+    fold = isinstance(in_scale, NormFold)
     try:
+        if fold:
+            keep_fold = _arm_fold(in_scale, b, ci, x.device)
+            in_scale = in_shift = None
         if pool_u is None:
             call("p2pb_pointwise_conv_forward", _i(b), _i(ci), _i(co), _i(p), ptr(x), ptr(wp), ptr(bias), ptr(bias_b),
                  ptr(in_scale), ptr(in_shift), _i(int(swish)), flags, ptr(y), ptr(st), stream_ptr())
             return (y, st) if fin is None else (y, st, aff)
         return _pw_conv_pool(x, wp, bias, bias_b, in_scale, in_shift, swish, flags, y, st, pool_u, b, ci, co, p, fin, aff)
     finally:
-        if fin is not None:
+        if armed:
             lib().p2pb_gn_finisher_disarm()
+        if fold:
+            lib().p2pb_gn_fold_disarm()
 
 
 def _pw_conv_pool(x, wp, bias, bias_b, in_scale, in_shift, swish, flags, y, st, pool_u, b, ci, co, p, fin, aff):
@@ -532,6 +573,7 @@
 
 
 def minmax_act(mm, scale, shift, swish=True, global_pool=False):
+    scale, shift = fold_arrays(scale, shift)
     if global_pool:
         b, nslots, c, _ = mm.shape
         y = torch.empty(b, c, dtype=F32, device=mm.device)
@@ -611,6 +653,7 @@
 
 
 def affine_act(x, scale, shift, swish=True, residual=None):
+    scale, shift = fold_arrays(scale, shift)
     b, c, p = x.shape
     y = torch.empty_like(x)
     if residual is not None:
@@ -621,6 +664,7 @@
 
 
 def affine_act_max(x, scale, shift, m, u, swish=True):
+    scale, shift = fold_arrays(scale, shift)
     b, c = x.shape[:2]
     y = torch.empty((b, c, m) if u else (b, c), dtype=F32, device=x.device)
     call("p2pb_affine_act_max", _i(b), _i(c), _i(m), _i(u), ptr(x), ptr(scale), ptr(shift), _i(int(swish)), ptr(y),
@@ -634,7 +678,7 @@
     def __enter__(self):
         import sys
         self._pre = os.environ.get("P2PB_EXPERIMENT")
-        os.environ["P2PB_EXPERIMENT"] = _experiment.setting(conv_pre=":")
+        os.environ["P2PB_EXPERIMENT"] = _experiment.setting(conv_pre=":", norm_prologue=0)
         self.rows, self.layers, self._mod = [], [], sys.modules[__name__]
         self._orig = {k: getattr(self._mod, k) for k in ("pw_conv", "conv3d_k3", "conv3d_k3_sparse", "conv3d_k3_compact")}
         names = {"pw_conv": ("in_scale", "in_shift", "swish"), "conv3d_k3": ("in_scale", "in_shift", "swish"),
diff --git a/p2p_bridge_amd/pvcnn_unet.py b/p2p_bridge_amd/pvcnn_unet.py
--- a/p2p_bridge_amd/pvcnn_unet.py
+++ b/p2p_bridge_amd/pvcnn_unet.py
@@ -411,7 +411,7 @@
                 _, st, mm, (sc, sh, _) = fused.pw_conv(h, conv, sc, sh, swish=sc is not None, pool_u=shape[-1], store=False,
                                                        fin=norm_fin(norm, P, cond))
                 return fused.minmax_act(mm, sc, sh).view(B, conv.weight.shape[0], *shape[2:-1])
-            h, st, (sc, sh, _) = fused.pw_conv(h, conv, sc, sh, swish=sc is not None, fin=norm_fin(norm, P, cond))
+            h, st, (sc, sh, _) = fused.pw_conv(h, conv, sc, sh, swish=sc is not None, fin=norm_fin(norm, P, cond), lazy=True)
         C = h.shape[1]
         if reduce_max:
             return fused.affine_act_max(h, sc, sh, int(np.prod(shape[2:-1])), shape[-1]).view(B, C, *shape[2:-1])
@@ -766,22 +766,23 @@
         N = coords.shape[2]
         a0, a1 = self.mlp1.shared_mlp_0.mlp, self.mlp1.shared_mlp_1.mlp
         b0, b1 = self.mlp2.shared_mlp_0.mlp, self.mlp2.shared_mlp_1.mlp
-        h, st, (sc, sh, _) = fused.pw_conv(coords.contiguous(), a0[0], fin=norm_fin(a0[1], N, None))
+        h, st, (sc, sh, _) = fused.pw_conv(coords.contiguous(), a0[0], fin=norm_fin(a0[1], N, None), lazy=True)
         pool = fused.pool_supported(N, 0)
         if pool:
             h, st, mm = fused.pw_conv(h, a1[0], sc, sh, swish=True, pool_u=0)
             g, sc, sh = fused.minmax_act_pool_gn(mm, st, norm_fin(a1[1], N, None))
         else:
-            h, st, (sc, sh, _) = fused.pw_conv(h, a1[0], sc, sh, swish=True, fin=norm_fin(a1[1], N, None))
+            h, st, (sc, sh, _) = fused.pw_conv(h, a1[0], sc, sh, swish=True, fin=norm_fin(a1[1], N, None), lazy=True)
             g = fused.affine_act_max(h, sc, sh, N, 0)
         c1 = h.shape[1]
         w = b0[0].weight.reshape(b0[0].out_channels, -1)
         bias_b = fused.linear_rows(g, w[:, c1:])
-        h, st, (sc, sh, _) = fused.pw_conv(h, b0[0], sc, sh, swish=True, bias_b=bias_b, ci_lo=0, ci_hi=c1, fin=norm_fin(b0[1], N, None))
+        h, st, (sc, sh, _) = fused.pw_conv(h, b0[0], sc, sh, swish=True, bias_b=bias_b, ci_lo=0, ci_hi=c1, fin=norm_fin(b0[1], N, None),
+                                           lazy=True)
         if pool:
             _, st, mm = fused.pw_conv(h, b1[0], sc, sh, swish=True, pool_u=0, store=False)
             return fused.minmax_act_pool_gn(mm, st, norm_fin(b1[1], N, None))[0]
-        h, st, (sc, sh, _) = fused.pw_conv(h, b1[0], sc, sh, swish=True, fin=norm_fin(b1[1], N, None))
+        h, st, (sc, sh, _) = fused.pw_conv(h, b1[0], sc, sh, swish=True, fin=norm_fin(b1[1], N, None), lazy=True)
         return fused.affine_act_max(h, sc, sh, N, 0)
 
 
@@ -1044,7 +1045,7 @@
         if self.embed_feats is not None:
             src = coords if self.extra_feature_channels == 0 else feats
             if use_fused:
-                h, st, (sc, sh, _) = fused.pw_conv(src, self.embed_feats[0], fin=norm_fin(self.embed_feats[1], N, None))
+                h, st, (sc, sh, _) = fused.pw_conv(src, self.embed_feats[0], fin=norm_fin(self.embed_feats[1], N, None), lazy=True)
                 feats, _ = fused.pw_conv(h, self.embed_feats[3], sc, sh, swish=True, stats=False)
             else:
                 from . import dense
@@ -1122,7 +1123,7 @@
         if use_fused:
             c0 = self.classifier[0]
             xin = data.features.contiguous()
-            h, st, (sc, sh, _) = fused.pw_conv(xin, c0.layers[0], fin=norm_fin(c0.layers[1], xin.shape[2], None))
+            h, st, (sc, sh, _) = fused.pw_conv(xin, c0.layers[0], fin=norm_fin(c0.layers[1], xin.shape[2], None), lazy=True)
             return fused.pw_conv(h, self.classifier[2], sc, sh, swish=True, stats=False)[0]
         from . import dense
 
```

After: 1.144 million points/s. About the same (-0.7%).
